# athaddius/RAFT_STIR

Hardware: AMD Instinct MI355X
Metric: train image-pairs/sec (node) + Sintel-res inference FPS, RAFT 12 iters (higher is better)
Workload: dtype bf16; 1 GPU; model=RAFT (raft-things config, 5.26M params), global_batch=8, per_gpu_batch=8, seq_len=12, iters=12, parallelism=dp1, ops=hip-kernels, corr_pyramid=bf16, correlation=all-pairs, train_step=eager, deterministic=True, grad_allreduce=none

## Files before the change

raft_stir_amd/csrc/conv.hip:

```cpp
#include "conv_common.h"

namespace rs {
namespace conv {

template <int CPR>
__device__ __forceinline__ int swz(int r, int c) {
  return CPR == 4 ? r * 4 + (c ^ ((r >> 2) & 3)) : r * 8 + (c ^ ((r >> 1) & 7));
}

template <int BM, int BN, int WAVES_M, int WAVES_N, int BK, bool GEO = false, bool F32 = false, int KG = 1>
__global__ __launch_bounds__(256 * KG) void conv_lds_kernel(Args a) {
  static_assert(WAVES_M * WAVES_N == 4, "4 waves");
  static_assert(KG == 1 || KG == 2 || KG == 4, "KG");
  static_assert(BK == 32 || BK == 64, "BK");
  static_assert(!F32 || BK == 64, "F32: 64-wide staged rows ([hi 32 | lo 32])");
  constexpr int CPR = BK / 8;
  constexpr int WM = BM / WAVES_M / 16, WN = BN / WAVES_N / 16;
  constexpr int NA = BM * CPR / 256, NB = F32 ? BN * 4 / 256 : BN * CPR / 256;
  static_assert(NA >= 1 && NB >= 1, "BM, BN must be multiples of 64");
  __shared__ uint4 lds_[KG * 2][(BM + BN) * CPR];

  const int kg = KG == 1 ? 0 : __builtin_amdgcn_readfirstlane((int)threadIdx.x >> 8);
  uint4 (*lds)[(BM + BN) * CPR] = lds_ + kg * 2;
  const int t = threadIdx.x & 255, lane = t & 63, wave = t >> 6;
// ... 478 lines not shown
#pragma unroll
      for (int nt = 0; nt < WN; ++nt)
        asm volatile("ds_read_b128 %0, %1 offset:%2" : "=v"(fb[kk][nt]) : "v"(bbase[kk] + so), "i"(nt * 16 * RB)
                     : "memory");
    }
    if (step + STAGES - 1 < nst) RS_BISSUE(buf == 0 ? STAGES - 1 : buf - 1);
    asm volatile("s_waitcnt lgkmcnt(0)" ::: "memory");
#pragma unroll
    for (int kk = 0; kk < 2; ++kk) {
#pragma unroll
      for (int mt = 0; mt < WM; ++mt) asm volatile("" : "+v"(fa[kk][mt]));
#pragma unroll
      for (int nt = 0; nt < WN; ++nt) asm volatile("" : "+v"(fb[kk][nt]));
    }
#pragma unroll
    for (int kk = 0; kk < 2; ++kk)
#pragma unroll
      for (int mt = 0; mt < WM; ++mt)
#pragma unroll
        for (int nt = 0; nt < WN; ++nt)
          acc[mt][nt] = __builtin_amdgcn_mfma_f32_16x16x32_bf16(__builtin_bit_cast(bf16x8_t, fa[kk][mt]),
                                                                __builtin_bit_cast(bf16x8_t, fb[kk][nt]),
                                                                acc[mt][nt], 0, 0, 0);
    buf = buf == STAGES - 1 ? 0 : buf + 1;
  }

#undef RS_BISSUE
#undef RS_BADV
  if constexpr (KG > 1) {
    constexpr int NE = WM * WN * 4;
    static_assert((KG - 1) * NE * NT * 4 <= STAGES * KG * GSLOT * 16, "split-K reduction buffer");
    float* red = reinterpret_cast<float*>(&lds[0][0]);
    __syncthreads();
    if (kg > 0) {
#pragma unroll
      for (int mt = 0; mt < WM; ++mt)
#pragma unroll
        for (int nt = 0; nt < WN; ++nt)
#pragma unroll
          for (int j = 0; j < 4; ++j)
            red[((size_t)((kg - 1) * NE + (mt * WN + nt) * 4 + j) * NT) + t] = acc[mt][nt][j];
    }
    __syncthreads();
    if (kg > 0) return;
#pragma unroll
    for (int g = 0; g < KG - 1; ++g)
#pragma unroll
      for (int mt = 0; mt < WM; ++mt)
#pragma unroll
        for (int nt = 0; nt < WN; ++nt)
#pragma unroll
          for (int j = 0; j < 4; ++j) acc[mt][nt][j] += red[((size_t)(g * NE + (mt * WN + nt) * 4 + j) * NT) + t];
  }

  int pb[WN], py[WN], px[WN];
#pragma unroll
  for (int nt = 0; nt < WN; ++nt) {
    const int p = n0 + nt * 16 + lr;
    if (p < a.P) {
      pb[nt] = p / HW;
      const int q = p - pb[nt] * HW;
      py[nt] = q / W;
      px[nt] = q - py[nt] * W;
    } else {
      pb[nt] = -1;
      py[nt] = px[nt] = 0;
    }
  }
  epilogue<WM, WN>(a, acc, m0, n0, lane, pb, py, px);
}

template <int BM, int TH, int HCAP>
__global__ __launch_bounds__(256) void conv_halo_kernel(Args a) {
  constexpr int TW = 16, BN = TH * TW;
  constexpr int WM = BM / 2 / 16, WN = BN / 2 / 16;
  constexpr int NA = BM * 8 / 256, NH = HCAP * 8 / 256;
  constexpr int AST = BM * 8, HST = HCAP * 8;
  constexpr int kFar = 0x7ffffff0;
  __shared__ uint4 lds[2 * AST + 2 * HST];

  const int t = threadIdx.x, lane = t & 63, wave = t >> 6;
  const int wm = wave & 1, wn = wave >> 1;
  const int H = a.H, W = a.W, KW = a.KW, Ktot = a.Ktot;
  const int taps = a.KH * KW;
  const int hw = TW + KW - 1;
  const int hrows = (TH + a.KH - 1) * hw;
  const int ntx = cdiv(W, TW), npb = cdiv(H, TH) * ntx;
  const int nct = cdiv(a.Cout, BM);
  const int lid = a.xcd_remap ? xcd_remap(blockIdx.x, gridDim.x) : (int)blockIdx.x;
  const int bm0 = (lid % nct) * BM;
  const int pt = lid / nct;
  const int img = pt / npb, pq = pt - img * npb;
  const int pty = pq / ntx;
  const int y0 = pty * TH, x0 = (pq - pty * ntx) * TW;
  const int m0 = bm0 + wm * WM * 16;

  const __amdgpu_buffer_rsrc_t rw = __builtin_amdgcn_make_buffer_rsrc((void*)a.w, (short)0, a.w_bytes, 0x00020000);
  const Seg s0 = a.seg[0], s1 = a.seg[1], s2 = a.seg[2];
  const __amdgpu_buffer_rsrc_t rs0 =
      __builtin_amdgcn_make_buffer_rsrc((void*)s0.ptr, (short)0, a.seg_bytes[0], 0x00020000);
  const __amdgpu_buffer_rsrc_t rs1 =
      __builtin_amdgcn_make_buffer_rsrc((void*)s1.ptr, (short)0, a.seg_bytes[1], 0x00020000);
  const __amdgpu_buffer_rsrc_t rs2 =
      __builtin_amdgcn_make_buffer_rsrc((void*)s2.ptr, (short)0, a.seg_bytes[2], 0x00020000);

  int aoff[NA];
#pragma unroll
  for (int i = 0; i < NA; ++i) {
    const int id = t + 256 * i, r = id >> 3;
    aoff[i] = ((bm0 + r) * taps * Ktot + (((id & 7) ^ ((r >> 1) & 7)) * 8)) * 2;
  }
  int hpix[NH], hch[NH];
#pragma unroll
  for (int i = 0; i < NH; ++i) {
    const int id = t + 256 * i, r = id >> 3;
    hch[i] = ((id & 7) ^ ((r >> 1) & 7)) * 8;
    hpix[i] = -1;
    if (r < hrows) {
      const int hy = r / hw, hx = r - hy * hw;
      const int y = y0 + hy - a.PH, x = x0 + hx - a.PW;
      if (y >= 0 && y < H && x >= 0 && x < W) hpix[i] = (img * H + y) * W + x;
    }
  }
  const int wbase = wave * 64;
  const int nsteps =
      taps * ((s0.C >> 6) + (a.nseg > 1 ? (s1.C >> 6) : 0) + (a.nseg > 2 ? (s2.C >> 6) : 0));

  int si = 0, c0 = 0, kseg = 0, itap = 0, ichunk = 0, istep = 0;
#define RS_HISSUE()                                                                                 \
  do {                                                                                              \
    const int sC = si == 0 ? s0.C : (si == 1 ? s1.C : s2.C);                                        \
    if (itap == 0) {                                                                                \
      const int sst = si == 0 ? s0.stride : (si == 1 ? s1.stride : s2.stride);                      \
      const __amdgpu_buffer_rsrc_t rb = si == 0 ? rs0 : (si == 1 ? rs1 : rs2);                      \
      uint4* hd = lds + 2 * AST + (ichunk & 1) * HST;                                               \
      _Pragma("unroll") for (int i = 0; i < NH; ++i) {                                              \
        const int v = hpix[i] >= 0 ? (hpix[i] * sst + c0 + hch[i]) * 2 : kFar;                      \
        bdma16(rb, hd + wbase + 256 * i, v, 0);                                                     \
      }                                                                                             \
    }                                                                                               \
    uint4* ad = lds + (istep & 1) * AST;                                                            \
    const int asoff = (itap * Ktot + kseg + c0) * 2;                                                \
    _Pragma("unroll") for (int i = 0; i < NA; ++i) bdma16(rw, ad + wbase + 256 * i, aoff[i], asoff); \
    ++istep;                                                                                        \
    if (++itap == taps) {                                                                           \
      itap = 0;                                                                                     \
      ++ichunk;                                                                                     \
      c0 += 64;                                                                                     \
      if (c0 == sC) { c0 = 0; kseg += sC; ++si; }                                                   \
    }                                                                                               \
  } while (0)

  f32x4_t acc[WM][WN];
#pragma unroll
  for (int i = 0; i < WM; ++i)
#pragma unroll
    for (int j = 0; j < WN; ++j) acc[i][j] = f32x4_t{0.f, 0.f, 0.f, 0.f};

  const int lr = lane & 15, lc = lane >> 4;
  const uint32_t lds0 = (uint32_t)(size_t)(__attribute__((address_space(3))) uint4*)&lds[0];
  uint32_t abase[2];
#pragma unroll
  for (int kk = 0; kk < 2; ++kk)
    abase[kk] = lds0 + (uint32_t)((wm * WM * 16 + lr) * 128 + (((kk * 4 + lc) ^ ((lr >> 1) & 7)) * 16));
  int rbn[WN];
#pragma unroll
  for (int nt = 0; nt < WN; ++nt) rbn[nt] = (wn * WN + nt) * hw + lr;

  RS_HISSUE();
  int ctap = 0, cty = 0, ctx = 0, cchunk = 0;
  for (int step = 0; step < nsteps; ++step) {
    wait_vmcnt<0>();
    asm volatile("s_barrier" ::: "memory");
    const uint32_t so = (step & 1) * AST * 16;
    const uint32_t hb = lds0 + (uint32_t)((2 * AST + (cchunk & 1) * HST) * 16);
    const int toff = cty * hw + ctx;
    uint32_t brow[WN], bsw[WN];
#pragma unroll
    for (int nt = 0; nt < WN; ++nt) {
      const int row = rbn[nt] + toff;
      brow[nt] = hb + (uint32_t)(row * 128);
      bsw[nt] = (uint32_t)((row >> 1) & 7);
    }
    u32x4_t fa[2][WM], fb[2][WN];
#pragma unroll
    for (int kk = 0; kk < 2; ++kk) {
#pragma unroll
      for (int mt = 0; mt < WM; ++mt)
        asm volatile("ds_read_b128 %0, %1 offset:%2" : "=v"(fa[kk][mt]) : "v"(abase[kk] + so), "i"(mt * 16 * 128)
                     : "memory");
#pragma unroll
      for (int nt = 0; nt < WN; ++nt)
        asm volatile("ds_read_b128 %0, %1" : "=v"(fb[kk][nt])
                     : "v"(brow[nt] + ((((uint32_t)(kk * 4 + lc)) ^ bsw[nt]) << 4)) : "memory");
    }
    if (step + 1 < nsteps) RS_HISSUE();
    asm volatile("s_waitcnt lgkmcnt(0)" ::: "memory");
#pragma unroll
    for (int kk = 0; kk < 2; ++kk) {
#pragma unroll
      for (int mt = 0; mt < WM; ++mt) asm volatile("" : "+v"(fa[kk][mt]));
#pragma unroll
      for (int nt = 0; nt < WN; ++nt) asm volatile("" : "+v"(fb[kk][nt]));
    }
#pragma unroll
    for (int kk = 0; kk < 2; ++kk)
#pragma unroll
      for (int mt = 0; mt < WM; ++mt)
#pragma unroll
        for (int nt = 0; nt < WN; ++nt)
          acc[mt][nt] = __builtin_amdgcn_mfma_f32_16x16x32_bf16(__builtin_bit_cast(bf16x8_t, fa[kk][mt]),
                                                                __builtin_bit_cast(bf16x8_t, fb[kk][nt]),
                                                                acc[mt][nt], 0, 0, 0);
    if (++ctx == KW) { ctx = 0; ++cty; }
    if (++ctap == taps) { ctap = 0; cty = 0; ctx = 0; ++cchunk; }
  }
#undef RS_HISSUE

  int pp[WN], pb[WN], py[WN], px[WN];
#pragma unroll
  for (int nt = 0; nt < WN; ++nt) {
    const int y = y0 + wn * WN + nt, x = x0 + lr;
    if (y < H && x < W) {
      pb[nt] = img;
      py[nt] = y;
      px[nt] = x;
      pp[nt] = (img * H + y) * W + x;
    } else {
      pb[nt] = -1;
      py[nt] = px[nt] = pp[nt] = 0;
    }
  }
  epilogue_pix<WM, WN>(a, acc, m0, lane, pp, pb, py, px);
}

__global__ __launch_bounds__(256) void conv_smalln_kernel(Args a) {
  __shared__ f32x4_t red[4][64];
  const int t = threadIdx.x, lane = t & 63, wave = t >> 6;
  const int n0 = blockIdx.x * 16;
  const int H = a.H, W = a.W, KW = a.KW, PH = a.PH, PW = a.PW, Ktot = a.Ktot;
  const int taps = a.KH * KW;
  const int HW = H * W;
  const int lr = lane & 15, lk = (lane >> 4) * 8;
  int pb[1], py[1], px[1];
  {
    const int p = n0 + lr;
    if (p < a.P) {
      pb[0] = p / HW;
      const int q = p - pb[0] * HW;
      py[0] = q / W;
      px[0] = q - py[0] * W;
    } else {
      pb[0] = -1;
      py[0] = px[0] = 0;
    }
  }
  const bf16_t* wrow = a.w + (size_t)lr * taps * Ktot + lk;
  const Seg s0 = a.seg[0], s1 = a.seg[1], s2 = a.seg[2];
  const int e1 = taps * (s0.C >> 5);
  const int e2 = e1 + (a.nseg > 1 ? taps * (s1.C >> 5) : 0);
  const int nsteps = e2 + (a.nseg > 2 ? taps * (s2.C >> 5) : 0);
  const uint4 zero = make_uint4(0, 0, 0, 0);
  f32x4_t acc[1][1];
  acc[0][0] = f32x4_t{0.f, 0.f, 0.f, 0.f};
  for (int step = wave; step < nsteps; step += 4) {
    const int si = (step >= e1) + (step >= e2);
    const bf16_t* sp = si == 0 ? s0.ptr : (si == 1 ? s1.ptr : s2.ptr);
    const int sC = si == 0 ? s0.C : (si == 1 ? s1.C : s2.C);
    const int sst = si == 0 ? s0.stride : (si == 1 ? s1.stride : s2.stride);
    const int kseg = si == 0 ? 0 : (si == 1 ? s0.C : s0.C + s1.C);
    const int local = step - (si == 0 ? 0 : (si == 1 ? e1 : e2));
    const int chunks = sC >> 5;
    const int tap = local / chunks;
    const int c0 = (local - tap * chunks) * 32;
    const int dy = tap / KW - PH, dx = tap % KW - PW;
    const uint4 fa = ld16(wrow + (size_t)tap * Ktot + kseg + c0);
    const int yy = py[0] + dy, xx = px[0] + dx;
    const bool ok = pb[0] >= 0 && yy >= 0 && yy < H && xx >= 0 && xx < W;
    const uint4 fb = ok ? ld16(sp + ((size_t)(pb[0] * H + yy) * W + xx) * sst + c0 + lk) : zero;
    acc[0][0] = __builtin_amdgcn_mfma_f32_16x16x32_bf16(__builtin_bit_cast(bf16x8_t, fa),
                                                        __builtin_bit_cast(bf16x8_t, fb), acc[0][0], 0, 0, 0);
  }
  red[wave][lane] = acc[0][0];
  __syncthreads();
  if (wave == 0) {
    acc[0][0] = red[0][lane] + red[1][lane] + red[2][lane] + red[3][lane];
    epilogue<1, 1>(a, acc, 0, n0, lane, pb, py, px);
  }
}

template <typename T>
__global__ __launch_bounds__(256) void gru_gate_bwd_kernel(float* __restrict__ dh, int dhstr, const T* __restrict__ z,
                                                           int zstr, const T* __restrict__ q, int qstr,
                                                           const T* __restrict__ h, int hstr, int hoff,
                                                           T* __restrict__ dq, int dqstr,
                                                           T* __restrict__ dzr, int dzrstr, long P, int hd) {
  const long total = P * hd;
  for (long i = (long)blockIdx.x * blockDim.x + threadIdx.x; i < total; i += (long)gridDim.x * blockDim.x) {
    const long p = i / hd;
    const int c = (int)(i - p * hd);
    const float g = dh[p * dhstr + c];
    const float zv = io<T>::ld(z + p * zstr + c), qv = io<T>::ld(q + p * qstr + c);
    const float hv = io<T>::ld(h + p * hstr + hoff + c);
    io<T>::st(dq + p * dqstr + c, g * zv * (1.f - qv * qv));
    io<T>::st(dzr + p * dzrstr + c, g * (qv - hv) * zv * (1.f - zv));
    dh[p * dhstr + c] = g * (1.f - zv);
  }
}

template <typename T>
__global__ __launch_bounds__(256) void relu_take_kernel(float* __restrict__ G, int gstr, int goff, int n, int nz,
                                                        const T* __restrict__ act, int astr, int aoff,
                                                        T* __restrict__ out, int ostr, long P) {
  const long total = P * ostr;
  for (long i = (long)blockIdx.x * blockDim.x + threadIdx.x; i < total; i += (long)gridDim.x * blockDim.x) {
    const long p = i / ostr;
    const int c = (int)(i - p * ostr);
    float v = 0.f;
    if (c < n) {
      const float g = G[p * gstr + goff + c];
      v = io<T>::ld(act + p * astr + aoff + c) > 0.f ? g : 0.f;
    }
    io<T>::st(out + i, v);
    if (c < nz) G[p * gstr + goff + c] = 0.f;
  }
}

}

bool conv_1x1_launch(const conv::Args& a, int tile, hipStream_t stream);

struct ConvLaunch {
  const void* seg_ptr[3];
  int seg_C[3], seg_stride[3];
  int nseg;
  const void* w;
  const float* bias;
  int B, H, W, KH, KW, PH, PW, Cout, Cout_pad, Ktot;
  int epi;
  float scale;
  int hd;
  void* out; int ostr, ooff;
  void* out2; int o2str, o2off;
  void* out3; int o3str, o3off;
  const void* aux1; int a1str, a1off;
  const void* aux2; int a2str, a2off;
  int tile;
  unsigned seg_bytes[3];
  unsigned w_bytes;
  int geo;
  int Hi, Wi, SY, SX, oH, oW, OSY, OSX, OOY, OOX;
  const float* chs;
  int f32;
};

bool conv_launch(const ConvLaunch& L, hipStream_t stream) {
  conv::Args a{};
  for (int s = 0; s < 3; ++s) {
    a.seg[s].ptr = static_cast<const bf16_t*>(L.seg_ptr[s]);
    a.seg[s].C = L.seg_C[s];
    a.seg[s].stride = L.seg_stride[s];
  }
  a.nseg = L.nseg;
  a.w = static_cast<const bf16_t*>(L.w);
  a.bias = L.bias;
  a.B = L.B; a.H = L.H; a.W = L.W; a.P = L.B * L.H * L.W;
  a.KH = L.KH; a.KW = L.KW; a.PH = L.PH; a.PW = L.PW;
  a.Cout = L.Cout; a.Ktot = L.Ktot;
  a.epi = L.epi; a.scale = L.scale; a.hd = L.hd;
  a.out = L.out; a.ostr = L.ostr; a.ooff = L.ooff;
  a.out2 = L.out2; a.o2str = L.o2str; a.o2off = L.o2off;
  a.out3 = L.out3; a.o3str = L.o3str; a.o3off = L.o3off;
  a.aux1 = static_cast<const bf16_t*>(L.aux1); a.a1str = L.a1str; a.a1off = L.a1off;
  a.aux2 = static_cast<const bf16_t*>(L.aux2); a.a2str = L.a2str; a.a2off = L.a2off;
  for (int s = 0; s < 3; ++s) a.seg_bytes[s] = L.seg_bytes[s];
  a.w_bytes = L.w_bytes;
  a.chs = L.chs;
  a.f32 = L.f32;
  a.xcd_remap = 1;
  if (L.geo) {
    a.Hi = L.Hi; a.Wi = L.Wi; a.SY = L.SY; a.SX = L.SX;
    a.oH = L.oH; a.oW = L.oW; a.OSY = L.OSY; a.OSX = L.OSX; a.OOY = L.OOY; a.OOX = L.OOX;
#define RS_GEO(BM_, BN_, WM_, WN_, BK_)                                                             \
  if (L.f32)                                                                                       \
    hipLaunchKernelGGL((conv::conv_lds_kernel<BM_, BN_, WM_, WN_, 64, true, true>),               \
                       dim3(cdiv(a.P, BN_), cdiv(L.Cout, BM_)), dim3(256), 0, stream, a);          \
  else                                                                                             \
    hipLaunchKernelGGL((conv::conv_lds_kernel<BM_, BN_, WM_, WN_, BK_, true>),                    \
                       dim3(cdiv(a.P, BN_), cdiv(L.Cout, BM_)), dim3(256), 0, stream, a)
    switch (L.tile) {
      case 2: RS_GEO(64, 128, 1, 4, 32); break;
      case 3: RS_GEO(64, 64, 2, 2, 32); break;
      case 6: RS_GEO(64, 64, 2, 2, 64); break;
      case 7: RS_GEO(128, 64, 2, 2, 64); break;
      case 8: RS_GEO(128, 128, 2, 2, 64); break;
      default: RS_GEO(128, 64, 2, 2, 32); break;
    }
#undef RS_GEO
    return true;
  }
  if (L.f32 && L.tile >= 81 && L.tile <= 85) {
    return conv_v3f_launch(a, L.tile, stream);
  }
  if (L.f32) {
#define RS_F32(BM_, BN_, KG_)                                                                       \
  hipLaunchKernelGGL((conv::conv_lds_kernel<BM_, BN_, 2, 2, 64, false, true, KG_>),                \
                     dim3(cdiv(a.P, BN_), cdiv(L.Cout, BM_)), dim3(256 * KG_), 0, stream, a)
    if (L.tile == 6) RS_F32(64, 64, 1);
    else if (L.tile == 8) RS_F32(128, 128, 1);
    else if (L.tile == 38) RS_F32(64, 64, 4);
    else if (L.tile == 39) RS_F32(128, 64, 2);
    else if (L.tile == 40) RS_F32(64, 64, 2);
    else RS_F32(128, 64, 1);
#undef RS_F32
    return true;
  }
  if (L.tile == 41) {
    dim3 grid(cdiv(a.P, 64), cdiv(L.Cout, 64));
    hipLaunchKernelGGL((conv::conv_lds_kernel<64, 64, 2, 2, 32, false, false, 4>), grid, dim3(1024), 0, stream, a);
    return true;
  }
  if (L.tile >= 24 && L.tile <= 26) {
    const int TH = L.tile == 26 ? 4 : 8, BM = L.tile == 25 ? 64 : 128;
    const dim3 grid(cdiv(L.Cout, BM) * L.B * cdiv(L.H, TH) * cdiv(L.W, 16));
    if (L.tile == 24) hipLaunchKernelGGL((conv::conv_halo_kernel<128, 8, 192>), grid, dim3(256), 0, stream, a);
    else if (L.tile == 25) hipLaunchKernelGGL((conv::conv_halo_kernel<64, 8, 192>), grid, dim3(256), 0, stream, a);
    else hipLaunchKernelGGL((conv::conv_halo_kernel<128, 4, 128>), grid, dim3(256), 0, stream, a);
    return true;
  }
  if (L.tile >= 42 && L.tile <= 54) {
    return conv_v2_launch(a, L.tile, stream);
  }
  if (L.tile == 70) {
    return conv_1x1_launch(a, L.tile, stream);
  }
  if (L.tile >= 56) {
    return conv_v3_launch(a, L.tile, stream);
  }
  if (L.tile == 5) {
    hipLaunchKernelGGL(conv::conv_smalln_kernel, dim3(cdiv(a.P, 16)), dim3(256), 0, stream, a);
  } else if (L.tile >= 2) {
    if (L.tile == 2) {
      dim3 grid(cdiv(a.P, 128), cdiv(L.Cout, 64));
      hipLaunchKernelGGL((conv::conv_lds_kernel<64, 128, 1, 4, 32>), grid, dim3(256), 0, stream, a);
    } else if (L.tile == 3) {
      dim3 grid(cdiv(a.P, 64), cdiv(L.Cout, 64));
      hipLaunchKernelGGL((conv::conv_lds_kernel<64, 64, 2, 2, 32>), grid, dim3(256), 0, stream, a);
    } else if (L.tile == 4) {
      dim3 grid(cdiv(a.P, 64), cdiv(L.Cout, 128));
      hipLaunchKernelGGL((conv::conv_lds_kernel<128, 64, 2, 2, 32>), grid, dim3(256), 0, stream, a);
    } else if (L.tile == 6) {
      dim3 grid(cdiv(a.P, 64), cdiv(L.Cout, 64));
      hipLaunchKernelGGL((conv::conv_lds_kernel<64, 64, 2, 2, 64>), grid, dim3(256), 0, stream, a);
    } else if (L.tile == 7) {
      dim3 grid(cdiv(a.P, 64), cdiv(L.Cout, 128));
      hipLaunchKernelGGL((conv::conv_lds_kernel<128, 64, 2, 2, 64>), grid, dim3(256), 0, stream, a);
    } else if (L.tile == 8) {
      dim3 grid(cdiv(a.P, 128), cdiv(L.Cout, 128));
      hipLaunchKernelGGL((conv::conv_lds_kernel<128, 128, 2, 2, 64>), grid, dim3(256), 0, stream, a);
    } else {
#define RS_GLDS(BM_, BN_, BK_, ST_)                                                                  \
  hipLaunchKernelGGL((conv::conv_glds_kernel<BM_, BN_, 2, 2, BK_, ST_>),                             \
                     dim3(cdiv(a.P, BN_) * cdiv(L.Cout, BM_)), dim3(256), 0, stream, a)
      switch (L.tile) {
        case 9: RS_GLDS(64, 64, 64, 3); break;
        case 10: RS_GLDS(128, 64, 64, 3); break;
        case 11: RS_GLDS(128, 64, 64, 2); break;
        case 12: RS_GLDS(128, 64, 32, 4); break;
        case 13: RS_GLDS(128, 64, 32, 3); break;
        case 14: RS_GLDS(64, 64, 32, 4); break;
        case 15: RS_GLDS(64, 64, 64, 2); break;
#define RS_BUF(BM_, BN_, ST_)                                                                        \
  hipLaunchKernelGGL((conv::conv_buf_kernel<BM_, BN_, 2, 2, ST_>), dim3(cdiv(a.P, BN_) * cdiv(L.Cout, BM_)), \
                     dim3(256), 0, stream, a)
        case 16: RS_BUF(128, 64, 2); break;
        case 17: RS_BUF(64, 64, 2); break;
        case 18: RS_BUF(128, 64, 3); break;
        case 19: RS_BUF(64, 64, 3); break;
        case 20: RS_BUF(128, 128, 2); break;
        case 21: RS_BUF(64, 128, 2); break;
        case 22: RS_BUF(128, 128, 3); break;
        case 23: RS_BUF(64, 64, 4); break;
#define RS_BUF8(BM_, BN_, ST_)                                                                       \
  hipLaunchKernelGGL((conv::conv_buf_kernel<BM_, BN_, 4, 2, ST_>), dim3(cdiv(a.P, BN_) * cdiv(L.Cout, BM_)), \
                     dim3(512), 0, stream, a)
        case 27: RS_BUF8(256, 96, 3); break;
        case 28: RS_BUF8(128, 96, 3); break;
        case 29: RS_BUF8(192, 96, 3); break;
        case 30: RS_BUF8(256, 96, 2); break;
        case 31: RS_BUF8(128, 96, 2); break;
        case 32: RS_BUF8(256, 192, 2); break;
        case 33: RS_BUF8(128, 192, 2); break;
#define RS_BUFK(BM_, BN_, ST_, KG_)                                                                  \
  hipLaunchKernelGGL((conv::conv_buf_kernel<BM_, BN_, 2, 2, ST_, KG_>),                                \
                     dim3(cdiv(a.P, BN_) * cdiv(L.Cout, BM_)), dim3(256 * KG_), 0, stream, a)
        case 34: RS_BUFK(64, 64, 2, 2); break;
        case 35: RS_BUFK(64, 64, 3, 2); break;
        case 36: RS_BUFK(128, 64, 2, 2); break;
        default: RS_BUFK(64, 64, 2, 4); break;
#undef RS_BUFK
#undef RS_BUF8
#undef RS_BUF
      }
#undef RS_GLDS
    }
  } else if (L.tile == 1) {
    constexpr int WM = 4, WN = 2, WAVES_M = 1, WAVES_N = 4;
    dim3 grid(cdiv(a.P, WN * 16 * WAVES_N), cdiv(L.Cout, WM * 16 * WAVES_M));
    hipLaunchKernelGGL((conv::conv_kernel<WM, WN, WAVES_M, WAVES_N>), grid, dim3(64 * WAVES_M * WAVES_N),
                       0, stream, a);
  } else {
    constexpr int WM = 2, WN = 2, WAVES_M = 1, WAVES_N = 4;
    dim3 grid(cdiv(a.P, WN * 16 * WAVES_N), cdiv(L.Cout, WM * 16 * WAVES_M));
    hipLaunchKernelGGL((conv::conv_kernel<WM, WN, WAVES_M, WAVES_N>), grid, dim3(64 * WAVES_M * WAVES_N),
                       0, stream, a);
  }
  return true;
}

static int egrid(long total) {
  const long g = (total + 255) / 256;
  return (int)(g < 16384 ? g : 16384);
}

void gru_gate_bwd_launch(float* dh, int dhstr, const void* z, int zstr, const void* q, int qstr, const void* h,
                         int hstr, int hoff, void* dq, int dqstr, void* dzr, int dzrstr, long P, int hd, bool f32,
                         hipStream_t stream) {
  if (f32)
    hipLaunchKernelGGL(conv::gru_gate_bwd_kernel<float>, dim3(egrid(P * hd)), dim3(256), 0, stream, dh, dhstr,
                       static_cast<const float*>(z), zstr, static_cast<const float*>(q), qstr,
                       static_cast<const float*>(h), hstr, hoff, static_cast<float*>(dq), dqstr,
                       static_cast<float*>(dzr), dzrstr, P, hd);
  else
    hipLaunchKernelGGL(conv::gru_gate_bwd_kernel<bf16_t>, dim3(egrid(P * hd)), dim3(256), 0, stream, dh, dhstr,
                       static_cast<const bf16_t*>(z), zstr, static_cast<const bf16_t*>(q), qstr,
                       static_cast<const bf16_t*>(h), hstr, hoff, static_cast<bf16_t*>(dq), dqstr,
                       static_cast<bf16_t*>(dzr), dzrstr, P, hd);
}

void relu_take_launch(float* G, int gstr, int goff, int n, int nz, const void* act, int astr, int aoff, void* out,
                      int ostr, long P, bool f32, hipStream_t stream) {
  if (f32)
    hipLaunchKernelGGL(conv::relu_take_kernel<float>, dim3(egrid(P * ostr)), dim3(256), 0, stream, G, gstr, goff, n,
                       nz, static_cast<const float*>(act), astr, aoff, static_cast<float*>(out), ostr, P);
  else
    hipLaunchKernelGGL(conv::relu_take_kernel<bf16_t>, dim3(egrid(P * ostr)), dim3(256), 0, stream, G, gstr, goff, n,
                       nz, static_cast<const bf16_t*>(act), astr, aoff, static_cast<bf16_t*>(out), ostr, P);
}


}
```

raft_stir_amd/csrc/conv_common.h:

```cpp
#pragma once
#include "common.h"

#include <stdlib.h>

namespace rs {
namespace conv {

enum Epi : int {
  EPI_BIAS = 0,
  EPI_RELU = 1,
  EPI_SCALE = 2,
  EPI_GRU_ZR = 3,
  EPI_GRU_Q = 4,
  EPI_FLOW = 5,
  EPI_RELU_BWD = 6,
  EPI_ACC_F32 = 7,
  EPI_GRU_QBWD = 8,
  EPI_NORM = 9,
};

struct Seg {
  const bf16_t* ptr;
  int C;
  int stride;
};

struct Args {
  Seg seg[3];
  int nseg;
  const bf16_t* w;
  const float* bias;
  int B, H, W, P;
  int KH, KW, PH, PW;
  int Cout, Ktot;
  int epi;
  float scale;
  int hd;
  void* out;
  int ostr, ooff;
  void* out2;
  int o2str, o2off;
  void* out3;
  int o3str, o3off;
  const bf16_t* aux1;
  int a1str, a1off;
  const bf16_t* aux2;
  int a2str, a2off;
  int xcd_remap;
  unsigned seg_bytes[3];
  unsigned w_bytes;
  int Hi, Wi, SY, SX;
  int oH, oW, OSY, OSX, OOY, OOX;
  const float* chs;
  int f32;
};

typedef float f32x2v_t __attribute__((ext_vector_type(2)));
typedef __bf16 bf16x2v_t __attribute__((ext_vector_type(2)));
__device__ __forceinline__ void split8(const float4& a, const float4& b, uint4& hi, uint4& lo) {
  const float x[8] = {a.x, a.y, a.z, a.w, b.x, b.y, b.z, b.w};
  uint32_t h[4], l[4];
#pragma unroll
  for (int i = 0; i < 4; ++i) {
    const f32x2v_t v = {x[2 * i], x[2 * i + 1]};
    const uint32_t hu = __builtin_bit_cast(uint32_t, __builtin_convertvector(v, bf16x2v_t));
    const f32x2v_t hf = {__uint_as_float(hu << 16), __uint_as_float(hu & 0xffff0000u)};
    h[i] = hu;
    l[i] = __builtin_bit_cast(uint32_t, __builtin_convertvector(v - hf, bf16x2v_t));
  }
  hi = make_uint4(h[0], h[1], h[2], h[3]);
  lo = make_uint4(l[0], l[1], l[2], l[3]);
}

__device__ __forceinline__ uint4 ld16(const bf16_t* p) { return *reinterpret_cast<const uint4*>(p); }

__device__ __forceinline__ void ld4(const bf16_t* p, float (&f)[4]) {
  const uint2 u = *reinterpret_cast<const uint2*>(p);
  f[0] = bf2f((bf16_t)(u.x & 0xffffu));
  f[1] = bf2f((bf16_t)(u.x >> 16));
  f[2] = bf2f((bf16_t)(u.y & 0xffffu));
  f[3] = bf2f((bf16_t)(u.y >> 16));
}
__device__ __forceinline__ void st4(bf16_t* p, const float (&f)[4]) {
  typedef float f2_t __attribute__((ext_vector_type(2)));
  typedef __bf16 b2_t __attribute__((ext_vector_type(2)));
  uint2 pk;
  pk.x = __builtin_bit_cast(uint32_t, __builtin_convertvector((f2_t{f[0], f[1]}), b2_t));
  pk.y = __builtin_bit_cast(uint32_t, __builtin_convertvector((f2_t{f[2], f[3]}), b2_t));
  *reinterpret_cast<uint2*>(p) = pk;
}
__device__ __forceinline__ void acc4(float* p, const float (&f)[4]) {
  float4 o = *reinterpret_cast<float4*>(p);
  o.x += f[0];
  o.y += f[1];
  o.z += f[2];
  o.w += f[3];
  *reinterpret_cast<float4*>(p) = o;
}

template <int E>
__device__ __forceinline__ void epi_frag(const Args& a, float (&v)[4], int cb, int p, int pb, int py, int px,
                                         int HW, bool vec) {
  const bool full = cb + 3 < a.Cout;
  if constexpr (E == EPI_FLOW) {
    float* crd = static_cast<float*>(a.out);
    const float* src = a.out2 ? static_cast<const float*>(a.out2) : crd;
#pragma unroll
    for (int j = 0; j < 4; ++j) {
      const int co = cb + j;
      if (co < a.Cout && co < 2) {
        const size_t o = ((size_t)pb * 2 + co) * HW + (size_t)py * a.W + px;
        crd[o] = src[o] + v[j];
      }
    }
  } else if constexpr (E == EPI_GRU_ZR) {
    if (cb < a.hd) {
      bf16_t* z = static_cast<bf16_t*>(a.out) + (size_t)p * a.ostr + a.ooff + cb;
      float zv[4];
#pragma unroll
      for (int j = 0; j < 4; ++j) zv[j] = sigmoidf_(v[j]);
      if (vec) {
        st4(z, zv);
      } else {
#pragma unroll
        for (int j = 0; j < 4; ++j) z[j] = f2bf(zv[j]);
      }
    } else {
      const int c = cb - a.hd;
      const bf16_t* h = a.aux1 + (size_t)p * a.a1str + a.a1off + c;
      bf16_t* rh = static_cast<bf16_t*>(a.out2) + (size_t)p * a.o2str + a.o2off + c;
      bf16_t* rs_ = a.out3 ? static_cast<bf16_t*>(a.out3) + (size_t)p * a.o3str + a.o3off + c : nullptr;
      float hv[4], rv[4], rhv[4];
      if (vec) {
        ld4(h, hv);
      } else {
#pragma unroll
        for (int j = 0; j < 4; ++j) hv[j] = bf2f(h[j]);
      }
#pragma unroll
      for (int j = 0; j < 4; ++j) {
        rv[j] = sigmoidf_(v[j]);
        rhv[j] = rv[j] * hv[j];
      }
      if (vec) {
        st4(rh, rhv);
        if (rs_) st4(rs_, rv);
      } else {
#pragma unroll
        for (int j = 0; j < 4; ++j) {
          rh[j] = f2bf(rhv[j]);
          if (rs_) rs_[j] = f2bf(rv[j]);
        }
      }
    }
  } else if constexpr (E == EPI_GRU_Q) {
    const bf16_t* h = a.aux1 + (size_t)p * a.a1str + a.a1off + cb;
    const bf16_t* z = a.aux2 + (size_t)p * a.a2str + a.a2off + cb;
    bf16_t* hn = static_cast<bf16_t*>(a.out) + (size_t)p * a.ostr + a.ooff + cb;
    bf16_t* qs = a.out2 ? static_cast<bf16_t*>(a.out2) + (size_t)p * a.o2str + a.o2off + cb : nullptr;
    float hv[4], zv[4], qv[4], nv[4];
    if (vec) {
      ld4(h, hv);
      ld4(z, zv);
    } else {
#pragma unroll
      for (int j = 0; j < 4; ++j) {
        hv[j] = bf2f(h[j]);
        zv[j] = bf2f(z[j]);
      }
    }
#pragma unroll
    for (int j = 0; j < 4; ++j) {
      qv[j] = tanhf_(v[j]);
      nv[j] = (1.f - zv[j]) * hv[j] + zv[j] * qv[j];
    }
    if (vec) {
      st4(hn, nv);
      if (qs) st4(qs, qv);
    } else {
#pragma unroll
      for (int j = 0; j < 4; ++j) {
        hn[j] = f2bf(nv[j]);
        if (qs) qs[j] = f2bf(qv[j]);
      }
    }
  } else if constexpr (E == EPI_RELU_BWD) {
    const bf16_t* act = a.aux1 + (size_t)p * a.a1str + a.a1off + cb;
    bf16_t* o = static_cast<bf16_t*>(a.out) + (size_t)p * a.ostr + a.ooff + cb;
    if (vec && full) {
      float av[4], ov[4];
      ld4(act, av);
#pragma unroll
      for (int j = 0; j < 4; ++j) ov[j] = av[j] > 0.f ? v[j] : 0.f;
      st4(o, ov);
    } else {
#pragma unroll
      for (int j = 0; j < 4; ++j)
        if (cb + j < a.Cout) o[j] = f2bf(bf2f(act[j]) > 0.f ? v[j] : 0.f);
    }
  } else if constexpr (E == EPI_ACC_F32) {
    float* o = static_cast<float*>(a.out) + (size_t)p * a.ostr + a.ooff + cb;
    if (vec && full) {
      acc4(o, v);
    } else {
#pragma unroll
      for (int j = 0; j < 4; ++j)
        if (cb + j < a.Cout) o[j] += v[j];
    }
  } else if constexpr (E == EPI_GRU_QBWD) {
    float* o = static_cast<float*>(a.out) + (size_t)p * a.ostr + a.ooff + cb;
    if (cb < a.hd) {
      const bf16_t* h = a.aux1 + (size_t)p * a.a1str + a.a1off + cb;
      const bf16_t* r = a.aux2 + (size_t)p * a.a2str + a.a2off + cb;
      bf16_t* drp = static_cast<bf16_t*>(a.out2) + (size_t)p * a.o2str + a.o2off + cb;
      float hv[4], rv[4], dv[4], gv[4];
      if (vec) {
        ld4(h, hv);
        ld4(r, rv);
      } else {
#pragma unroll
        for (int j = 0; j < 4; ++j) {
          hv[j] = bf2f(h[j]);
          rv[j] = bf2f(r[j]);
        }
      }
#pragma unroll
      for (int j = 0; j < 4; ++j) {
        dv[j] = v[j] * hv[j] * rv[j] * (1.f - rv[j]);
        gv[j] = v[j] * rv[j];
      }
      if (vec) {
        st4(drp, dv);
        acc4(o, gv);
      } else {
#pragma unroll
        for (int j = 0; j < 4; ++j) {
          drp[j] = f2bf(dv[j]);
          o[j] += gv[j];
        }
      }
    } else {
      if (vec && full) {
        acc4(o, v);
      } else {
#pragma unroll
        for (int j = 0; j < 4; ++j)
          if (cb + j < a.Cout) o[j] += v[j];
      }
    }
  } else if constexpr (E == EPI_NORM) {
    if (a.hd) {
#pragma unroll
      for (int j = 0; j < 4; ++j) v[j] = fmaxf(v[j], 0.f);
    }
    bf16_t* o = static_cast<bf16_t*>(a.out) + (size_t)p * a.ostr + a.ooff + cb;
    const bf16_t* r = a.aux1 ? a.aux1 + (size_t)p * a.a1str + a.a1off + cb : nullptr;
    if (vec && full) {
      if (r) {
        float rv[4];
        ld4(r, rv);
#pragma unroll
        for (int j = 0; j < 4; ++j) v[j] = fmaxf(v[j] + rv[j], 0.f);
      }
      st4(o, v);
    } else {
#pragma unroll
      for (int j = 0; j < 4; ++j)
        if (cb + j < a.Cout) o[j] = f2bf(r ? fmaxf(v[j] + bf2f(r[j]), 0.f) : v[j]);
    }
  } else {
#pragma unroll
    for (int j = 0; j < 4; ++j) {
      if constexpr (E == EPI_RELU) v[j] = fmaxf(v[j], 0.f);
      if constexpr (E == EPI_SCALE) v[j] *= a.scale;
    }
    bf16_t* o = static_cast<bf16_t*>(a.out) + (size_t)p * a.ostr + a.ooff + cb;
    if (vec && full) {
      st4(o, v);
    } else {
#pragma unroll
      for (int j = 0; j < 4; ++j)
        if (cb + j < a.Cout) o[j] = f2bf(v[j]);
    }
  }
}

template <int WM, int WN, int E>
__device__ __forceinline__ void epi_loop(const Args& a, const f32x4_t (&acc)[WM][WN], int m0, int lane,
                                         const int (&pp)[WN], const int (&pb)[WN], const int (&py)[WN],
                                         const int (&px)[WN]) {
  const int HW = a.H * a.W;
  const int cq = (lane >> 4) * 4;
  const bool vec =
      ((a.ooff | a.ostr | a.o2off | a.o2str | a.o3off | a.o3str | a.a1off | a.a1str | a.a2off | a.a2str) & 3) == 0 &&
      (((uintptr_t)a.out | (uintptr_t)a.out2 | (uintptr_t)a.out3 | (uintptr_t)a.aux1 | (uintptr_t)a.aux2) & 15) == 0;
  const bool bvec = a.bias && (((uintptr_t)a.bias) & 15) == 0;
#pragma unroll
  for (int nt = 0; nt < WN; ++nt) {
    if (pb[nt] < 0) continue;
#pragma unroll
    for (int mt = 0; mt < WM; ++mt) {
      const int cb = m0 + mt * 16 + cq;
      if (cb >= a.Cout) continue;
      float v[4];
      if constexpr (E == EPI_NORM) {
        const float4 sv = *reinterpret_cast<const float4*>(a.chs + cb);
        const float4 bv = *reinterpret_cast<const float4*>(a.bias + cb);
        v[0] = acc[mt][nt][0] * sv.x + bv.x;
        v[1] = acc[mt][nt][1] * sv.y + bv.y;
        v[2] = acc[mt][nt][2] * sv.z + bv.z;
        v[3] = acc[mt][nt][3] * sv.w + bv.w;
      } else if (bvec && cb + 3 < a.Cout) {
        const float4 bv = *reinterpret_cast<const float4*>(a.bias + cb);
        v[0] = acc[mt][nt][0] + bv.x;
        v[1] = acc[mt][nt][1] + bv.y;
        v[2] = acc[mt][nt][2] + bv.z;
        v[3] = acc[mt][nt][3] + bv.w;
      } else {
#pragma unroll
        for (int j = 0; j < 4; ++j) v[j] = acc[mt][nt][j] + (cb + j < a.Cout && a.bias ? a.bias[cb + j] : 0.f);
      }
      epi_frag<E>(a, v, cb, pp[nt], pb[nt], py[nt], px[nt], HW, vec);
    }
  }
}

template <int WM, int WN>
__device__ __forceinline__ void epilogue_pix(const Args& a, const f32x4_t (&acc)[WM][WN], int m0, int lane,
                                             const int (&pp)[WN], const int (&pb)[WN], const int (&py)[WN],
                                             const int (&px)[WN]) {
  switch (a.epi) {
#define RS_EPI(E) \
  case E: epi_loop<WM, WN, E>(a, acc, m0, lane, pp, pb, py, px); break
    RS_EPI(EPI_FLOW);
    RS_EPI(EPI_GRU_ZR);
    RS_EPI(EPI_GRU_Q);
    RS_EPI(EPI_RELU_BWD);
    RS_EPI(EPI_ACC_F32);
    RS_EPI(EPI_GRU_QBWD);
    RS_EPI(EPI_RELU);
    RS_EPI(EPI_SCALE);
    RS_EPI(EPI_NORM);
#undef RS_EPI
    default: epi_loop<WM, WN, EPI_BIAS>(a, acc, m0, lane, pp, pb, py, px); break;
  }
}

__device__ __forceinline__ void ld4f(const bf16_t* p, float (&f)[4]) {
  const float4 v = *reinterpret_cast<const float4*>(p);
  f[0] = v.x; f[1] = v.y; f[2] = v.z; f[3] = v.w;
}
__device__ __forceinline__ void st4f(void* p, const float (&f)[4]) {
  *reinterpret_cast<float4*>(p) = make_float4(f[0], f[1], f[2], f[3]);
}

template <int E>
__device__ __forceinline__ void epi_frag_f32(const Args& a, float (&v)[4], int cb, int p, bool vec) {
  const bool full = cb + 3 < a.Cout;
  auto fo = [](void* b, int str, int off, int p_, int c) { return static_cast<float*>(b) + (size_t)p_ * str + off + c; };
  auto fi = [](const bf16_t* b, int str, int off, int p_, int c) {
    return reinterpret_cast<const float*>(b) + (size_t)p_ * str + off + c;
  };
  if constexpr (E == EPI_GRU_ZR) {
    if (cb < a.hd) {
      float* z = fo(a.out, a.ostr, a.ooff, p, cb);
#pragma unroll
      for (int j = 0; j < 4; ++j) z[j] = sigmoidf_(v[j]);
    } else {
      const int c = cb - a.hd;
      const float* h = fi(a.aux1, a.a1str, a.a1off, p, c);
      float* rh = fo(a.out2, a.o2str, a.o2off, p, c);
      float* r = a.out3 ? fo(a.out3, a.o3str, a.o3off, p, c) : nullptr;
#pragma unroll
      for (int j = 0; j < 4; ++j) {
        const float rv = sigmoidf_(v[j]);
        rh[j] = rv * h[j];
        if (r) r[j] = rv;
      }
    }
  } else if constexpr (E == EPI_GRU_Q) {
    const float* h = fi(a.aux1, a.a1str, a.a1off, p, cb);
    const float* z = fi(a.aux2, a.a2str, a.a2off, p, cb);
    float* hn = fo(a.out, a.ostr, a.ooff, p, cb);
    float* qs = a.out2 ? fo(a.out2, a.o2str, a.o2off, p, cb) : nullptr;
#pragma unroll
    for (int j = 0; j < 4; ++j) {
      const float q = tanhf(v[j]);
      hn[j] = (1.f - z[j]) * h[j] + z[j] * q;
      if (qs) qs[j] = q;
    }
  } else if constexpr (E == EPI_RELU_BWD) {
    const float* act = fi(a.aux1, a.a1str, a.a1off, p, cb);
    float* o = fo(a.out, a.ostr, a.ooff, p, cb);
    if (vec && full) {
      const float4 av = *reinterpret_cast<const float4*>(act);
      *reinterpret_cast<float4*>(o) = make_float4(av.x > 0.f ? v[0] : 0.f, av.y > 0.f ? v[1] : 0.f,
                                                  av.z > 0.f ? v[2] : 0.f, av.w > 0.f ? v[3] : 0.f);
    } else {
#pragma unroll
      for (int j = 0; j < 4; ++j)
        if (cb + j < a.Cout) o[j] = act[j] > 0.f ? v[j] : 0.f;
    }
  } else if constexpr (E == EPI_ACC_F32) {
    float* o = fo(a.out, a.ostr, a.ooff, p, cb);
    if (vec && full) {
      acc4(o, v);
    } else {
#pragma unroll
      for (int j = 0; j < 4; ++j)
        if (cb + j < a.Cout) o[j] += v[j];
    }
  } else if constexpr (E == EPI_GRU_QBWD) {
    float* o = fo(a.out, a.ostr, a.ooff, p, cb);
    if (cb < a.hd) {
      const float* h = fi(a.aux1, a.a1str, a.a1off, p, cb);
      const float* r = fi(a.aux2, a.a2str, a.a2off, p, cb);
      float* drp = fo(a.out2, a.o2str, a.o2off, p, cb);
      float gv[4];
#pragma unroll
      for (int j = 0; j < 4; ++j) {
        drp[j] = v[j] * h[j] * r[j] * (1.f - r[j]);
        gv[j] = v[j] * r[j];
      }
      if (vec) {
        acc4(o, gv);
      } else {
#pragma unroll
        for (int j = 0; j < 4; ++j) o[j] += gv[j];
      }
    } else if (vec && full) {
      acc4(o, v);
    } else {
#pragma unroll
      for (int j = 0; j < 4; ++j)
        if (cb + j < a.Cout) o[j] += v[j];
    }
  } else {
#pragma unroll
    for (int j = 0; j < 4; ++j) {
      if constexpr (E == EPI_RELU) v[j] = fmaxf(v[j], 0.f);
      if constexpr (E == EPI_SCALE) v[j] *= a.scale;
      if constexpr (E == EPI_NORM)
        if (a.hd) v[j] = fmaxf(v[j], 0.f);
    }
    float* o = fo(a.out, a.ostr, a.ooff, p, cb);
    const float* r = (E == EPI_NORM && a.aux1) ? fi(a.aux1, a.a1str, a.a1off, p, cb) : nullptr;
    if (vec && full) {
      if (r) {
        float rv[4];
        ld4f(reinterpret_cast<const bf16_t*>(r), rv);
#pragma unroll
        for (int j = 0; j < 4; ++j) v[j] = fmaxf(v[j] + rv[j], 0.f);
      }
      st4f(o, v);
    } else {
#pragma unroll
      for (int j = 0; j < 4; ++j)
        if (cb + j < a.Cout) o[j] = r ? fmaxf(v[j] + r[j], 0.f) : v[j];
    }
  }
}

template <int WM, int WN, int E>
__device__ __forceinline__ void epi_loop_f32(const Args& a, const f32x4_t (&acc)[WM][WN], int m0, int lane,
                                             const int (&pp)[WN], const int (&pb)[WN]) {
  const int cq = (lane >> 4) * 4;
  const bool vec =
      ((a.ooff | a.ostr | a.o2off | a.o2str | a.o3off | a.o3str | a.a1off | a.a1str | a.a2off | a.a2str) & 3) == 0 &&
      (((uintptr_t)a.out | (uintptr_t)a.out2 | (uintptr_t)a.out3 | (uintptr_t)a.aux1 | (uintptr_t)a.aux2) & 15) == 0;
#pragma unroll
  for (int nt = 0; nt < WN; ++nt) {
    if (pb[nt] < 0) continue;
#pragma unroll
    for (int mt = 0; mt < WM; ++mt) {
      const int cb = m0 + mt * 16 + cq;
      if (cb >= a.Cout) continue;
      float v[4];
#pragma unroll
      for (int j = 0; j < 4; ++j) {
        const int c = cb + j;
        const bool in = c < a.Cout;
        const float sc = (E == EPI_NORM && in) ? a.chs[c] : 1.f;
        v[j] = acc[mt][nt][j] * sc + (in && a.bias ? a.bias[c] : 0.f);
      }
      epi_frag_f32<E>(a, v, cb, pp[nt], vec);
    }
  }
}

template <int WM, int WN>
__device__ __forceinline__ void epilogue_pix_f32(const Args& a, const f32x4_t (&acc)[WM][WN], int m0, int lane,
                                                 const int (&pp)[WN], const int (&pb)[WN]) {
  switch (a.epi) {
#define RS_EPI32(E) \
  case E: epi_loop_f32<WM, WN, E>(a, acc, m0, lane, pp, pb); break
    RS_EPI32(EPI_GRU_ZR);
    RS_EPI32(EPI_GRU_Q);
    RS_EPI32(EPI_RELU_BWD);
    RS_EPI32(EPI_ACC_F32);
    RS_EPI32(EPI_GRU_QBWD);
    RS_EPI32(EPI_RELU);
    RS_EPI32(EPI_SCALE);
    RS_EPI32(EPI_NORM);
#undef RS_EPI32
    default: epi_loop_f32<WM, WN, EPI_BIAS>(a, acc, m0, lane, pp, pb); break;
  }
}

template <int WM, int WN>
__device__ __forceinline__ void epilogue(const Args& a, const f32x4_t (&acc)[WM][WN], int m0, int n0,
                                         int lane, const int (&pb)[WN], const int (&py)[WN],
                                         const int (&px)[WN]) {
  int pp[WN];
#pragma unroll
  for (int nt = 0; nt < WN; ++nt) pp[nt] = n0 + nt * 16 + (lane & 15);
  epilogue_pix<WM, WN>(a, acc, m0, lane, pp, pb, py, px);
}

template <int WM, int WN, int WAVES_M, int WAVES_N>
__global__ __launch_bounds__(64 * WAVES_M * WAVES_N) void conv_kernel(Args a) {
  const int lane = threadIdx.x & 63;
  const int wave = threadIdx.x >> 6;
  const int wm = wave % WAVES_M, wn = wave / WAVES_M;
  const int m0 = (blockIdx.y * WAVES_M + wm) * WM * 16;
  const int n0 = (blockIdx.x * WAVES_N + wn) * WN * 16;
  const int lr = lane & 15, lk = (lane >> 4) * 8;
  const int taps = a.KH * a.KW;
  const int HW = a.H * a.W;

  int pb[WN], py[WN], px[WN];
#pragma unroll
  for (int nt = 0; nt < WN; ++nt) {
    const int p = n0 + nt * 16 + lr;
    if (p < a.P) {
      pb[nt] = p / HW;
      const int q = p - pb[nt] * HW;
      py[nt] = q / a.W;
      px[nt] = q - py[nt] * a.W;
    } else {
      pb[nt] = -1;
      py[nt] = px[nt] = 0;
    }
  }
  const bf16_t* wrow[WM];
#pragma unroll
  for (int mt = 0; mt < WM; ++mt)
    wrow[mt] = a.w + (size_t)(m0 + mt * 16 + lr) * taps * a.Ktot + lk;

  f32x4_t acc[WM][WN];
#pragma unroll
  for (int i = 0; i < WM; ++i)
#pragma unroll
    for (int j = 0; j < WN; ++j) acc[i][j] = f32x4_t{0.f, 0.f, 0.f, 0.f};

  const Seg s0 = a.seg[0], s1 = a.seg[1], s2 = a.seg[2];
  const int e1 = taps * (s0.C >> 5);
  const int e2 = e1 + (a.nseg > 1 ? taps * (s1.C >> 5) : 0);
  const int nsteps = e2 + (a.nseg > 2 ? taps * (s2.C >> 5) : 0);

  const int H = a.H, W = a.W, KW = a.KW, PH = a.PH, PW = a.PW, Ktot = a.Ktot;
  const uint4 zero = make_uint4(0, 0, 0, 0);
#define RS_CONV_LOAD(STEP, FA, FB)                                                           \
  do {                                                                                       \
    const int step_ = (STEP);                                                                \
    const int si = (step_ >= e1) + (step_ >= e2);                                            \
    const bf16_t* sp = si == 0 ? s0.ptr : (si == 1 ? s1.ptr : s2.ptr);                       \
    const int sC = si == 0 ? s0.C : (si == 1 ? s1.C : s2.C);                                 \
    const int sst = si == 0 ? s0.stride : (si == 1 ? s1.stride : s2.stride);                 \
    const int kseg = si == 0 ? 0 : (si == 1 ? s0.C : s0.C + s1.C);                           \
    const int local = step_ - (si == 0 ? 0 : (si == 1 ? e1 : e2));                          \
    const int chunks = sC >> 5;                                                              \
    const int tap = local / chunks;                                                          \
    const int c0 = (local - tap * chunks) * 32;                                              \
    const int dy = tap / KW - PH, dx = tap % KW - PW;                                        \
    _Pragma("unroll") for (int mt = 0; mt < WM; ++mt)                                        \
      FA[mt] = ld16(wrow[mt] + (size_t)tap * Ktot + kseg + c0);                              \
    _Pragma("unroll") for (int nt = 0; nt < WN; ++nt) {                                      \
      const int yy = py[nt] + dy, xx = px[nt] + dx;                                          \
      const bool ok = pb[nt] >= 0 && yy >= 0 && yy < H && xx >= 0 && xx < W;                 \
      FB[nt] = ok ? ld16(sp + ((size_t)(pb[nt] * H + yy) * W + xx) * sst + c0 + lk) : zero;  \
    }                                                                                        \
  } while (0)

#define RS_CONV_MMA(FA, FB)                                                                       \
  _Pragma("unroll") for (int mt = 0; mt < WM; ++mt)                                               \
    _Pragma("unroll") for (int nt = 0; nt < WN; ++nt)                                             \
      acc[mt][nt] = __builtin_amdgcn_mfma_f32_16x16x32_bf16(                                      \
          __builtin_bit_cast(bf16x8_t, FA[mt]), __builtin_bit_cast(bf16x8_t, FB[nt]), acc[mt][nt], \
          0, 0, 0)

  uint4 fa0[WM], fb0[WN], fa1[WM], fb1[WN];
  RS_CONV_LOAD(0, fa0, fb0);
  int step = 0;
  for (; step + 2 <= nsteps; step += 2) {
    RS_CONV_LOAD(step + 1, fa1, fb1);
    RS_CONV_MMA(fa0, fb0);
    if (step + 2 < nsteps) RS_CONV_LOAD(step + 2, fa0, fb0);
    RS_CONV_MMA(fa1, fb1);
  }
  if (step < nsteps) {
    RS_CONV_MMA(fa0, fb0);
  }
#undef RS_CONV_LOAD
#undef RS_CONV_MMA

  epilogue<WM, WN>(a, acc, m0, n0, lane, pb, py, px);
}

typedef unsigned int u32x4_t __attribute__((ext_vector_type(4)));

__device__ __forceinline__ int xcd_remap(int bid, int nwg) {
  const int q = nwg >> 3, r = nwg & 7, x = bid & 7;
  return (x < r ? x * (q + 1) : r * (q + 1) + (x - r) * q) + (bid >> 3);
}

__device__ __forceinline__ void glds16(const void* src, uint4* lds_base) {
  __builtin_amdgcn_global_load_lds(
      (const __attribute__((address_space(1))) void*)src, (__attribute__((address_space(3))) void*)lds_base, 16,
      0, 0);
}

template <int N>
__device__ __forceinline__ void wait_vmcnt() {
  asm volatile("s_waitcnt vmcnt(%0)" ::"n"(N) : "memory");
}

__device__ __forceinline__ void bdma16(__amdgpu_buffer_rsrc_t r, uint4* lds_base, int voff, int soff) {
  __builtin_amdgcn_raw_ptr_buffer_load_lds(r, (__attribute__((address_space(3))) void*)lds_base, 16, voff, soff,
                                           0, 0);
}

template <int N>
__device__ __forceinline__ void wait_lgkm() {
  asm volatile("s_waitcnt lgkmcnt(%0)" ::"n"(N) : "memory");
}

template <int E>
__device__ __forceinline__ void epi32(const Args& a, const f32x16_t& acc, int m0, int lane, int p, int pb, int py,
                                      int px, bool vec) {
  if (pb < 0) return;
  const int HW = a.H * a.W;
#pragma unroll
  for (int g = 0; g < 4; ++g) {
    const int cb = m0 + 8 * g + 4 * (lane >> 5);
    if (cb >= a.Cout) continue;
    float v[4];
#pragma unroll
    for (int j = 0; j < 4; ++j) v[j] = acc[4 * g + j] + (cb + j < a.Cout && a.bias ? a.bias[cb + j] : 0.f);
    epi_frag<E>(a, v, cb, p, pb, py, px, HW, vec);
  }
}

template <int NB, int E>
__device__ __forceinline__ void epi32_batch(const Args& a, const f32x16_t (&acc)[NB], int m0, int lane,
                                            const int (&pp)[NB], const int (&pb)[NB]) {
  const int h4 = 4 * (lane >> 5);
  float bz[16];
#pragma unroll
  for (int i = 0; i < 16; ++i) bz[i] = a.bias ? a.bias[m0 + 8 * (i >> 2) + h4 + (i & 3)] : 0.f;
  const bool lo = m0 < a.hd;
  constexpr int NBC = NB > 3 ? 3 : NB;
#pragma unroll
  for (int n0 = 0; n0 < NB; n0 += NBC) {
    uint2 l1[NBC][4], l2[NBC][4];
    float4 lf[NBC][4];
#pragma unroll
    for (int k = 0; k < NBC; ++k) {
      if (n0 + k >= NB) break;
      const size_t p = (size_t)(pb[n0 + k] >= 0 ? pp[n0 + k] : 0);
#pragma unroll
      for (int g = 0; g < 4; ++g) {
        const int cb = m0 + 8 * g + h4;
        if constexpr (E == EPI_GRU_ZR) {
          if (!lo) l1[k][g] = *reinterpret_cast<const uint2*>(a.aux1 + p * a.a1str + a.a1off + cb - a.hd);
        } else if constexpr (E == EPI_GRU_Q) {
          l1[k][g] = *reinterpret_cast<const uint2*>(a.aux1 + p * a.a1str + a.a1off + cb);
          l2[k][g] = *reinterpret_cast<const uint2*>(a.aux2 + p * a.a2str + a.a2off + cb);
        } else if constexpr (E == EPI_RELU_BWD) {
          l1[k][g] = *reinterpret_cast<const uint2*>(a.aux1 + p * a.a1str + a.a1off + cb);
        } else if constexpr (E == EPI_ACC_F32) {
          lf[k][g] = *reinterpret_cast<const float4*>(static_cast<const float*>(a.out) + p * a.ostr + a.ooff + cb);
        } else if constexpr (E == EPI_GRU_QBWD) {
          lf[k][g] = *reinterpret_cast<const float4*>(static_cast<const float*>(a.out) + p * a.ostr + a.ooff + cb);
          if (lo) {
            l1[k][g] = *reinterpret_cast<const uint2*>(a.aux1 + p * a.a1str + a.a1off + cb);
            l2[k][g] = *reinterpret_cast<const uint2*>(a.aux2 + p * a.a2str + a.a2off + cb);
          }
        }
      }
    }
#pragma unroll
    for (int k = 0; k < NBC; ++k) {
      if (n0 + k >= NB) break;
      if (pb[n0 + k] < 0) continue;
      const size_t p = (size_t)pp[n0 + k];
#pragma unroll
      for (int g = 0; g < 4; ++g) {
        const int cb = m0 + 8 * g + h4;
        float v[4];
#pragma unroll
        for (int j = 0; j < 4; ++j) v[j] = acc[n0 + k][4 * g + j] + bz[4 * g + j];
        auto unpack = [](uint2 u, float (&f)[4]) {
          f[0] = bf2f((bf16_t)(u.x & 0xffffu));
          f[1] = bf2f((bf16_t)(u.x >> 16));
          f[2] = bf2f((bf16_t)(u.y & 0xffffu));
          f[3] = bf2f((bf16_t)(u.y >> 16));
        };
        if constexpr (E == EPI_GRU_ZR) {
          float r[4];
#pragma unroll
          for (int j = 0; j < 4; ++j) r[j] = sigmoidf_(v[j]);
          if (lo) {
            st4(static_cast<bf16_t*>(a.out) + p * a.ostr + a.ooff + cb, r);
          } else {
            const int c = cb - a.hd;
            float hv[4], rh[4];
            unpack(l1[k][g], hv);
#pragma unroll
            for (int j = 0; j < 4; ++j) rh[j] = r[j] * hv[j];
            st4(static_cast<bf16_t*>(a.out2) + p * a.o2str + a.o2off + c, rh);
            if (a.out3) st4(static_cast<bf16_t*>(a.out3) + p * a.o3str + a.o3off + c, r);
          }
        } else if constexpr (E == EPI_GRU_Q) {
          float hv[4], zv[4], q[4], nv[4];
          unpack(l1[k][g], hv);
          unpack(l2[k][g], zv);
#pragma unroll
          for (int j = 0; j < 4; ++j) {
            q[j] = tanhf_(v[j]);
            nv[j] = (1.f - zv[j]) * hv[j] + zv[j] * q[j];
          }
          st4(static_cast<bf16_t*>(a.out) + p * a.ostr + a.ooff + cb, nv);
          if (a.out2) st4(static_cast<bf16_t*>(a.out2) + p * a.o2str + a.o2off + cb, q);
        } else if constexpr (E == EPI_RELU_BWD) {
          float av[4];
          unpack(l1[k][g], av);
#pragma unroll
          for (int j = 0; j < 4; ++j) v[j] = av[j] > 0.f ? v[j] : 0.f;
          st4(static_cast<bf16_t*>(a.out) + p * a.ostr + a.ooff + cb, v);
        } else if constexpr (E == EPI_ACC_F32) {
          const float4 o = lf[k][g];
          *reinterpret_cast<float4*>(static_cast<float*>(a.out) + p * a.ostr + a.ooff + cb) =
              make_float4(o.x + v[0], o.y + v[1], o.z + v[2], o.w + v[3]);
        } else if constexpr (E == EPI_GRU_QBWD) {
          const float4 o = lf[k][g];
          float* op = static_cast<float*>(a.out) + p * a.ostr + a.ooff + cb;
          if (lo) {
            float hv[4], rv[4], dv[4];
            unpack(l1[k][g], hv);
            unpack(l2[k][g], rv);
#pragma unroll
            for (int j = 0; j < 4; ++j) dv[j] = v[j] * hv[j] * rv[j] * (1.f - rv[j]);
            st4(static_cast<bf16_t*>(a.out2) + p * a.o2str + a.o2off + cb, dv);
            *reinterpret_cast<float4*>(op) =
                make_float4(o.x + v[0] * rv[0], o.y + v[1] * rv[1], o.z + v[2] * rv[2], o.w + v[3] * rv[3]);
          } else {
            *reinterpret_cast<float4*>(op) = make_float4(o.x + v[0], o.y + v[1], o.z + v[2], o.w + v[3]);
          }
        } else {
#pragma unroll
          for (int j = 0; j < 4; ++j) {
            if constexpr (E == EPI_RELU) v[j] = fmaxf(v[j], 0.f);
            if constexpr (E == EPI_SCALE) v[j] *= a.scale;
          }
          st4(static_cast<bf16_t*>(a.out) + p * a.ostr + a.ooff + cb, v);
        }
      }
    }
  }
}

template <int NB>
__device__ __forceinline__ void epilogue32(const Args& a, const f32x16_t (&acc)[NB], int m0, int lane,
                                           const int (&pp)[NB], const int (&pb)[NB], const int (&py)[NB],
                                           const int (&px)[NB]) {
  const bool vec =
      ((a.ooff | a.ostr | a.o2off | a.o2str | a.o3off | a.o3str | a.a1off | a.a1str | a.a2off | a.a2str) & 3) == 0 &&
      (((uintptr_t)a.out | (uintptr_t)a.out2 | (uintptr_t)a.out3 | (uintptr_t)a.aux1 | (uintptr_t)a.aux2) & 15) == 0;
  const bool fast = vec && m0 + 32 <= a.Cout && (a.hd & 31) == 0;
  if (fast) {
    switch (a.epi) {
#define RS_EB(E) \
  case E: epi32_batch<NB, E>(a, acc, m0, lane, pp, pb); return
      RS_EB(EPI_GRU_ZR);
      RS_EB(EPI_GRU_Q);
      RS_EB(EPI_RELU_BWD);
      RS_EB(EPI_ACC_F32);
      RS_EB(EPI_GRU_QBWD);
      RS_EB(EPI_RELU);
      RS_EB(EPI_SCALE);
      RS_EB(EPI_BIAS);
#undef RS_EB
      default: break;
    }
  }
  switch (a.epi) {
#define RS_E2(E)                                                                      \
  case E:                                                                             \
    _Pragma("unroll") for (int nb = 0; nb < NB; ++nb)                                 \
      epi32<E>(a, acc[nb], m0, lane, pp[nb], pb[nb], py[nb], px[nb], vec);            \
    break
    RS_E2(EPI_FLOW);
    RS_E2(EPI_GRU_ZR);
    RS_E2(EPI_GRU_Q);
    RS_E2(EPI_RELU_BWD);
    RS_E2(EPI_ACC_F32);
    RS_E2(EPI_GRU_QBWD);
    RS_E2(EPI_RELU);
    RS_E2(EPI_SCALE);
#undef RS_E2
    default:
#pragma unroll
      for (int nb = 0; nb < NB; ++nb) epi32<EPI_BIAS>(a, acc[nb], m0, lane, pp[nb], pb[nb], py[nb], px[nb], vec);
      break;
  }
}

}

bool conv_v2_launch(const conv::Args& a, int tile, hipStream_t stream);
bool conv_v3_launch(const conv::Args& a, int tile, hipStream_t stream);
bool conv_v3f_launch(const conv::Args& a, int tile, hipStream_t stream);
}
```

raft_stir_amd/csrc/ops_conv.cpp:

```cpp
#include <ATen/ATen.h>
#include "host_common.h"
#include "enc_epi.h"
#include <c10/core/DeviceGuard.h>
#include <torch/library.h>

#include <hip/hip_runtime.h>
#include <stdlib.h>

#include <algorithm>
#include <initializer_list>

namespace rs {
struct ConvLaunch {
  const void* seg_ptr[3];
  int seg_C[3], seg_stride[3];
  int nseg;
  const void* w;
  const float* bias;
  int B, H, W, KH, KW, PH, PW, Cout, Cout_pad, Ktot;
  int epi;
  float scale;
  int hd;
  void* out; int ostr, ooff;
  void* out2; int o2str, o2off;
  void* out3; int o3str, o3off;
  const void* aux1; int a1str, a1off;
  const void* aux2; int a2str, a2off;
  int tile;
  unsigned seg_bytes[3];
  unsigned w_bytes;
  int geo;
  int Hi, Wi, SY, SX, oH, oW, OSY, OSX, OOY, OOX;
  const float* chs;
  int f32;
};
bool conv_launch(const ConvLaunch& L, hipStream_t stream);
struct SconvLaunch {
  const void* x;
  int xstr, Cin, B, Hi, Wi;
  const float* w;
  const float* bias;
  void* y;
  int ystr, yoff, Cout, Ho, Wo, KH, KW, S, P, relu;
  const void* res;
  int rstr;
  bool f32;
};
int sconv_max_weights();
struct SconvWgradLaunch {
  const void* x;
  const void* dy;
  int xstr, ystr, Cin, Cout, B, Hi, Wi, Ho, Wo, KH, KW, S, P;
  bool f32;
  float* dw;
  float* part;
};
int sconv_wgrad_blocks(int B, int Ho, int OUT, int* rows_per_block);
void sconv_wgrad_launch(const SconvWgradLaunch& L, int nblk, int rows_per_block, hipStream_t stream);
void sconv_launch(const SconvLaunch& L, hipStream_t stream);
struct EncWgradLaunch {
  const void* x;
  const void* dy;
  int xstr, ystr;
  long x_bytes, dy_bytes;
  int B, H, W, Cin, Cout;
  float* part;
  float* dw;
  int nsplit, tpb;
};
int enc_wgrad_splits(int B, int H, int W, int Cin, int Cout, int* tpb);
void enc_wgrad_launch(const EncWgradLaunch& L, hipStream_t stream);
void flow_enc_launch(const float* coords, int B, int H, int W, const float* w, const float* bias,
                     int Cout, void* out, int ostr, int ooff, void* fout, int fstr, int foff, bool f32,
                     hipStream_t stream);
void flowhead_fwd_launch(const void* x, int xstr, int xoff, int cin, const float* w, const float* bias, int B,
                         int H, int W, float* crd, const float* src, bool x_f32, hipStream_t s);
void flowhead_dgrad_launch(const float* dflow, const float* w, int cin, int B, int H, int W, const void* act,
                           int astr, int aoff, void* out, int ostr, int ooff, bool f32, hipStream_t s);
void gru_gate_bwd_launch(float* dh, int dhstr, const void* z, int zstr, const void* q, int qstr, const void* h,
                         int hstr, int hoff, void* dq, int dqstr, void* dzr, int dzrstr, long P, int hd, bool f32,
                         hipStream_t stream);
void relu_take_launch(float* G, int gstr, int goff, int n, int nz, const void* act, int astr, int aoff, void* out,
                      int ostr, long P, bool f32, hipStream_t stream);
struct WgradLaunch {
  const void* dy;
  int ystr, yoff, Cout;
  const void* seg_ptr[3];
  int seg_C[3], seg_stride[3], seg_period[3];
  int nseg;
  int Bp, H, W, KH, KW, Ktot;
  float* dw;
  float* db;
  int bn128;  unsigned dy_bytes, seg_bytes[3];
  int dma;
  float* part;
  int Hi, Wi, SY, SX;
};
void wgrad_launch(const WgradLaunch& L, hipStream_t stream);
int wgrad_splits(const WgradLaunch& L);
int colsum_blocks(int P);
void colsum_launch(const void* dy, int ystr, int yoff, int C, int P, float* db, float* part, hipStream_t stream);
int flow_wgrad_blocks(int Bp, int H);
size_t flow_wgrad_lds(int W);
void flow_wgrad_launch(const float* coords, int Bp, int H, int W, const void* df, int fstr, int Cout, float* dw,
                       float* db, float* part, bool f32, hipStream_t stream);
bool deterministic();
bool enc_halo_launch(const uint16_t* x, int xstr, const uint16_t* w, int Ktot, uint16_t* y, int ystr, int B, int H,
                     int W, int cin, int cout, int num_cus, const EncEpi& e, hipStream_t stream);
bool enc_halo_supported(int cin, int cout);
struct StemLaunch {
  const void* x;
  int x_bf16, B, Hi, Wi, Ho, Wo;
  const void* w;
  const float* bias;
  int Cout, epi, relu;
  void* out;
  int ostr, ooff;
  const void* res;
  int rstr;
  const float* chs;
  int f32;
};
void stem_launch(const StemLaunch& L, hipStream_t stream);
int stem_wgrad_blocks(int B, int Ho, int Wo, int* chunks_per_block);
void stem_wgrad_launch(const void* x, bool x_bf16, int B, int Hi, int Wi, int Ho, int Wo, const uint16_t* dy, int ystr,
                       int Cout, float* part, int nblk, int px_per_block, float* dw, hipStream_t stream);
}

namespace {
using at::Tensor;

constexpr int EPI_GRU_ZR = 3, EPI_GRU_Q = 4, EPI_FLOW = 5, EPI_RELU_BWD = 6, EPI_ACC_F32 = 7, EPI_GRU_QBWD = 8,
              EPI_NORM = 9;

hipStream_t stream() { return rs::current_stream(); }

void check_nhwc(const Tensor& t, int B, int H, int W, const char* n, at::ScalarType dt = at::kBFloat16) {
  TORCH_CHECK(t.is_cuda() && t.is_contiguous() && t.dim() == 4, n, ": contiguous NHWC GPU tensor required");
  TORCH_CHECK(t.size(0) == B && t.size(1) == H && t.size(2) == W, n, ": spatial shape mismatch");
  TORCH_CHECK(t.scalar_type() == dt, n, ": ", dt, " required");
}

void check_one_device(const char* op, const Tensor& first, std::initializer_list<const Tensor*> rest) {
  for (const Tensor* t : rest)
    TORCH_CHECK(t == nullptr || !t->defined() || t->device() == first.device(), op,
                ": all tensors must be on one device, got ", first.device(), " and ", t->device());
}
const Tensor* opt_ptr(const c10::optional<Tensor>& t) { return t ? &*t : nullptr; }

struct NormX {
  const float* chs = nullptr;
};
void check_vec4(const c10::optional<Tensor>& t, int Cout, const char* op, const char* n) {
  TORCH_CHECK(t && t->is_cuda() && t->is_contiguous() && t->scalar_type() == at::kFloat &&
                  t->numel() >= (Cout + 3) / 4 * 4 && (uintptr_t)t->data_ptr() % 16 == 0,
              op, ": ", n, " must be 16-B aligned fp32 with round_up(Cout, 4) values");
}
NormX norm_extras(const c10::optional<Tensor>& nscale, const c10::optional<Tensor>& bias, int epi, int Cout,
                  const char* op) {
  NormX x;
  TORCH_CHECK(bool(nscale) == (epi == EPI_NORM), op, ": nscale is the EPI_NORM scale (and only that)");
  if (nscale) {
    check_vec4(nscale, Cout, op, "nscale");
    check_vec4(bias, Cout, op, "bias (the EPI_NORM shift)");
    x.chs = nscale->data_ptr<float>();
  }
  return x;
}

void conv_impl(const std::vector<Tensor>& segs, at::IntArrayRef seg_off, at::IntArrayRef seg_C,
               const Tensor& w, const c10::optional<Tensor>& bias, int64_t KH, int64_t KW, int64_t Cout,
               int64_t epi, double scale, int64_t hd, const Tensor& out, int64_t ooff,
               const c10::optional<Tensor>& out2, int64_t o2off, const c10::optional<Tensor>& out3,
               int64_t o3off, const c10::optional<Tensor>& aux1, int64_t a1off,
               const c10::optional<Tensor>& aux2, int64_t a2off, int64_t tile,
               const NormX& nx = NormX()) {
  TORCH_CHECK(!segs.empty() && segs.size() <= 3, "conv_fused: 1..3 input segments");
  TORCH_CHECK(seg_off.size() == segs.size() && seg_C.size() == segs.size(), "conv_fused: segment spec");
  const int B = segs[0].size(0), H = segs[0].size(1), W = segs[0].size(2);
  const c10::DeviceGuard guard(segs[0].device());
  rs::ConvLaunch L{};
  const bool f32 = segs[0].scalar_type() == at::kFloat;
  const at::ScalarType adt = f32 ? at::kFloat : at::kBFloat16;
  const bool v3f = f32 && tile >= 81 && tile <= 85;
  if (f32) {
    TORCH_CHECK(tile == 6 || tile == 7 || tile == 8 || (tile >= 38 && tile <= 40) || v3f,
                "conv_fused: fp32 activations run on tiles 6, 7, 8, 38-40, 81-85 only");
    TORCH_CHECK(epi != EPI_FLOW, "conv_fused: fp32 activations: no flow epilogue (csrc/flowhead.hip serves it)");
  }
  L.f32 = f32 ? 1 : 0;
  int Ktot = 0;
  for (size_t s = 0; s < 3; ++s) {
    if (s < segs.size()) {
      check_nhwc(segs[s], B, H, W, "segment", adt);
      const int C = seg_C[s], off = seg_off[s], Cb = segs[s].size(3);
      TORCH_CHECK(C > 0 && C % 32 == 0, "conv_fused: segment channels must be a positive multiple of 32");
      TORCH_CHECK(off >= 0 && off % 8 == 0 && Cb % 8 == 0 && off + C <= Cb,
                  "conv_fused: segment window out of bounds or misaligned");
      L.seg_ptr[s] = static_cast<const char*>(segs[s].data_ptr()) + (size_t)off * segs[s].element_size();
      L.seg_C[s] = C;
      L.seg_stride[s] = Cb;
      TORCH_CHECK(segs[s].numel() * segs[s].element_size() < (int64_t(1) << 31),
                  "conv_fused: segment tensor must be < 2 GiB");
      L.seg_bytes[s] = (unsigned)((segs[s].numel() - off) * segs[s].element_size());
      Ktot += C;
    } else {
      L.seg_ptr[s] = L.seg_ptr[0];
      L.seg_C[s] = 32;
      L.seg_stride[s] = L.seg_stride[0];
      L.seg_bytes[s] = L.seg_bytes[0];
    }
  }
  L.nseg = segs.size();
  TORCH_CHECK(KH >= 1 && KW >= 1 && KH % 2 == 1 && KW % 2 == 1, "conv_fused: odd kernel sizes only");
  TORCH_CHECK((tile >= 0 && tile <= 54) || tile == 56 || tile == 57 || tile == 61 || tile == 65 || tile == 66 ||
                  tile == 68 || tile == 70 || v3f,
              "conv_fused: tile must be in [0,54], 56, 57, 61, 65, 66, 68 or 70");
  if (tile == 70) {
    TORCH_CHECK(KH == 1 && KW == 1 && !f32, "conv_fused: tile 70 is the bf16 1x1 GEMM");
    for (size_t s = 0; s < segs.size(); ++s)
      TORCH_CHECK(seg_C[s] % 64 == 0, "conv_fused: tile 70 needs segment channels % 64 == 0");
  }
  const bool v3 = tile >= 56 && tile <= 68;
  if (v3f) {
    for (size_t s = 0; s < segs.size(); ++s)
      TORCH_CHECK(seg_C[s] % 64 == 0, "conv_fused: tiles 81-85 need segment channels % 64 == 0");
    TORCH_CHECK(tile != 85 || Ktot == 64, "conv_fused: tile 85 (one halo buffer) needs exactly one 64-channel K chunk");
  }
  if ((tile >= 42 && tile <= 54) || v3 || v3f)
    TORCH_CHECK((KH == 3 && KW == 3) || (KH == 1 && KW == 5) || (KH == 5 && KW == 1),
                "conv_fused: tiles 42-68 are instantiated for 3x3, 1x5 and 5x1 kernels only");
  TORCH_CHECK(tile < 16 || KH * KW <= 32, "conv_fused: buffer-DMA tiles (16-37) support at most 32 taps");
  TORCH_CHECK(!(tile >= 38 && tile <= 40) || f32, "conv_fused: tiles 38-40 are the fp32 split-K tiles");
  TORCH_CHECK(tile != 5 || Cout <= 16, "conv_fused: tile 5 (small-N) needs Cout <= 16");
  if (tile >= 24 && tile <= 26) {
    const int TH = tile == 26 ? 4 : 8, HCAP = tile == 26 ? 128 : 192;
    TORCH_CHECK((TH + KH - 1) * (16 + KW - 1) <= HCAP, "conv_fused: kernel too large for halo tile ", tile);
  }
  const bool bm128 = tile == 4 || tile == 7 || tile == 8 || (tile >= 10 && tile <= 13) || tile == 16 ||
                     tile == 18 || tile == 20 || tile == 22 || tile == 24 || tile == 26 || tile == 36 ||
                     tile == 39;
  const bool bm128w = tile == 28 || tile == 31 || tile == 33;
  const int tileM = (tile == 48 || tile == 49 || tile == 53 || tile == 70) ? 128
                    : (tile == 50 || tile == 51 || tile == 52) ? 256
                    : tile == 54 ? 192
                    : (tile == 42 || tile >= 45) ? 64 : tile == 43 ? 32 : tile == 44 ? 128
                    : tile == 0 ? 32
                    : (tile == 27 || tile == 30 || tile == 32) ? 256
                    : tile == 29 ? 192
                    : (bm128 || bm128w) ? 128 : (tile == 5 ? 16 : 64);
  if (tile >= 6 && tile != 12 && tile != 13 && tile != 14 && tile != 41 && !f32)
    for (size_t s = 0; s < segs.size(); ++s)
      TORCH_CHECK(seg_C[s] % 64 == 0, "conv_fused: 64-deep-K tiles need segment channels % 64 == 0");
  TORCH_CHECK(w.is_cuda() && w.is_contiguous() && w.scalar_type() == at::kBFloat16 && w.dim() == 3,
              "conv_fused: packed weight must be contiguous bf16 (Cout_pad, taps, Ktot)");
  TORCH_CHECK(w.size(1) == KH * KW && w.size(2) == (f32 && !v3f ? 2 : 1) * Ktot,
              "conv_fused: packed weight K mismatch", f32 && !v3f ? " (fp32: split [wh | wl] weights, 2 x Ktot)" : "");
  if (v3f) {
    TORCH_CHECK(w.size(0) % 64 == 0 && w.size(0) / 2 >= (Cout + 31) / 32 * 32 && w.numel() * 2 < (int64_t(1) << 31),
                "conv_fused: tiles 81-85 need split fragment-major weights [frag(wh); frag(wl)] (ops/conv.py "
                "frag_weight_split)");
  } else if (v3) {
    TORCH_CHECK(w.size(0) % 32 == 0 && w.size(0) >= (Cout + 31) / 32 * 32 && w.numel() * 2 < (int64_t(1) << 31),
                "conv_fused: tiles 56-68 need fragment-major weights with round_up(Cout, 32) rows (< 2 GiB)");
  } else {
    TORCH_CHECK(w.size(0) >= (Cout + tileM - 1) / tileM * tileM,
                "conv_fused: packed weight needs >= round_up(Cout, ", tileM, ") rows");
  }
  if (bias) {
    TORCH_CHECK(bias->is_cuda() && bias->scalar_type() == at::kFloat && bias->numel() >= Cout &&
                    bias->is_contiguous(),
                "conv_fused: bias must be fp32 (Cout,)");
  }
  L.w = w.data_ptr();
  L.w_bytes = (unsigned)(w.numel() * 2);
  L.bias = bias ? bias->data_ptr<float>() : nullptr;
  L.B = B; L.H = H; L.W = W; L.KH = KH; L.KW = KW; L.PH = KH / 2; L.PW = KW / 2;
  L.Cout = Cout; L.Cout_pad = w.size(0); L.Ktot = w.size(2);
  L.epi = epi; L.scale = scale; L.hd = hd; L.tile = tile;
  if (epi == EPI_FLOW) {
    TORCH_CHECK(out.is_cuda() && out.is_contiguous() && out.scalar_type() == at::kFloat && out.dim() == 4 &&
                    out.size(0) == B && out.size(1) == 2 && out.size(2) == H && out.size(3) == W,
                "conv_fused(flow): out must be fp32 coords (B,2,H,W)");
    TORCH_CHECK(Cout == 2, "conv_fused(flow): Cout must be 2");
    L.out = out.data_ptr(); L.ostr = 0; L.ooff = 0;
    if (out2) {
      TORCH_CHECK(out2->is_cuda() && out2->is_contiguous() && out2->scalar_type() == at::kFloat &&
                      out2->sizes() == out.sizes(),
                  "conv_fused(flow): out2 (source coords) must match out");
      L.out2 = out2->data_ptr();
    }
  } else {
    const bool f32out = f32 || epi == EPI_ACC_F32 || epi == EPI_GRU_QBWD;
    check_nhwc(out, B, H, W, "out", f32out ? at::kFloat : at::kBFloat16);
    const int cw = epi == EPI_GRU_ZR ? hd : Cout;
    TORCH_CHECK(ooff >= 0 && ooff + cw <= out.size(3), "conv_fused: output window out of bounds");
    L.out = out.data_ptr(); L.ostr = out.size(3); L.ooff = ooff;
  }
  auto opt_nhwc = [&](const c10::optional<Tensor>& t, int64_t off, int width, const char* n, void** p,
                      int* str, int* o) {
    if (!t) { *p = nullptr; *str = 0; *o = 0; return; }
    check_nhwc(*t, B, H, W, n, adt);
    TORCH_CHECK(off >= 0 && off + width <= t->size(3), "conv_fused: ", n, " window out of bounds");
    *p = t->data_ptr(); *str = t->size(3); *o = off;
  };
  void* p;
  if (epi == EPI_GRU_ZR) {
    TORCH_CHECK(Cout == 2 * hd && hd % 4 == 0 && out2 && aux1, "conv_fused(gru_zr): needs Cout=2*hd, out2 (r*h), aux1 (h)");
    opt_nhwc(out2, o2off, hd, "out2", &L.out2, &L.o2str, &L.o2off);
    opt_nhwc(out3, o3off, hd, "out3", &L.out3, &L.o3str, &L.o3off);
    opt_nhwc(aux1, a1off, hd, "aux1", &p, &L.a1str, &L.a1off); L.aux1 = p;
  } else if (epi == EPI_GRU_Q) {
    TORCH_CHECK(Cout % 4 == 0 && aux1 && aux2, "conv_fused(gru_q): needs aux1 (h) and aux2 (z)");
    opt_nhwc(out2, o2off, Cout, "out2", &L.out2, &L.o2str, &L.o2off);
    opt_nhwc(aux1, a1off, Cout, "aux1", &p, &L.a1str, &L.a1off); L.aux1 = p;
    opt_nhwc(aux2, a2off, Cout, "aux2", &p, &L.a2str, &L.a2off); L.aux2 = p;
  } else if (epi == EPI_RELU_BWD) {
    TORCH_CHECK(aux1, "conv_fused(relu_bwd): needs aux1 (the ReLU output)");
    opt_nhwc(aux1, a1off, Cout, "aux1", &p, &L.a1str, &L.a1off); L.aux1 = p;
  } else if (epi == EPI_NORM) {
    if (aux1) { opt_nhwc(aux1, a1off, Cout, "aux1", &p, &L.a1str, &L.a1off); L.aux1 = p; }
  } else if (epi == EPI_GRU_QBWD) {
    TORCH_CHECK(hd % 4 == 0 && hd <= Cout && out2 && aux1 && aux2,
                "conv_fused(gru_qbwd): needs out2 (dr_pre), aux1 (h), aux2 (r)");
    opt_nhwc(out2, o2off, hd, "out2", &L.out2, &L.o2str, &L.o2off);
    opt_nhwc(aux1, a1off, hd, "aux1", &p, &L.a1str, &L.a1off); L.aux1 = p;
    opt_nhwc(aux2, a2off, hd, "aux2", &p, &L.a2str, &L.a2off); L.aux2 = p;
  }
  TORCH_CHECK(epi >= 0 && epi <= EPI_NORM, "conv_fused: unknown epilogue kind");
  if (nx.chs)
    TORCH_CHECK(!(tile >= 42 && tile <= 54) && !v3 && tile != 70 && (!(tile >= 81 && tile <= 85) || f32),
                "conv_fused: EPI_NORM needs a tile with the shared epilogue (not 42-70)");
  L.chs = nx.chs;
  TORCH_CHECK(rs::conv_launch(L, stream()), "conv_fused: tile ", L.tile, " is not instantiated for a ", KH, "x", KW,
              " kernel");
  RS_CHECK_LAUNCH();
}

void conv_fused(const std::vector<Tensor>& segs, at::IntArrayRef seg_off, at::IntArrayRef seg_C,
                const Tensor& w, const c10::optional<Tensor>& bias, int64_t KH, int64_t KW, int64_t Cout,
                int64_t epi, double scale, int64_t hd, const Tensor& out, int64_t ooff,
                const c10::optional<Tensor>& out2, int64_t o2off, const c10::optional<Tensor>& out3,
                int64_t o3off, const c10::optional<Tensor>& aux1, int64_t a1off,
                const c10::optional<Tensor>& aux2, int64_t a2off, int64_t tile, const c10::optional<Tensor>& nscale) {
  const NormX nx = norm_extras(nscale, bias, epi, Cout, "conv_fused");
  conv_impl(segs, seg_off, seg_C, w, bias, KH, KW, Cout, epi, scale, hd, out, ooff, out2, o2off, out3, o3off,
            aux1, a1off, aux2, a2off, tile, nx);
}

void conv_geo(const std::vector<Tensor>& segs, at::IntArrayRef seg_off, at::IntArrayRef seg_C, const Tensor& w,
              const c10::optional<Tensor>& bias, int64_t KH, int64_t KW, int64_t PH, int64_t PW, int64_t SY,
              int64_t SX, int64_t Ho, int64_t Wo, int64_t Cout, const Tensor& out, int64_t ooff, int64_t OSY,
              int64_t OSX, int64_t OOY, int64_t OOX, int64_t tile, const c10::optional<Tensor>& nscale, bool relu) {
  TORCH_CHECK(!segs.empty() && segs.size() <= 3 && seg_off.size() == segs.size() && seg_C.size() == segs.size(),
              "conv_geo: 1..3 input segments");
  TORCH_CHECK(tile == 2 || tile == 3 || tile == 4 || tile == 6 || tile == 7 || tile == 8,
              "conv_geo: tile must be one of the register-staged variants 2, 3, 4, 6, 7, 8");
  const bool f32 = segs[0].scalar_type() == at::kFloat;
  const at::ScalarType adt = f32 ? at::kFloat : at::kBFloat16;
  const int bk = (tile >= 6 && !f32) ? 64 : 32;
  const int tileM = (tile == 2 || tile == 3 || tile == 6) ? 64 : 128;
  const int B = segs[0].size(0), Hi = segs[0].size(1), Wi = segs[0].size(2);
  const c10::DeviceGuard guard(segs[0].device());
  rs::ConvLaunch L{};
  int Ktot = 0;
  for (size_t s = 0; s < 3; ++s) {
    if (s < segs.size()) {
      check_nhwc(segs[s], B, Hi, Wi, "conv_geo segment", adt);
      const int C = seg_C[s], off = seg_off[s], Cb = segs[s].size(3);
      TORCH_CHECK(C > 0 && C % bk == 0, "conv_geo: segment channels must be a multiple of ", bk, " for tile ", tile);
      TORCH_CHECK(off >= 0 && off % 8 == 0 && Cb % 8 == 0 && off + C <= Cb, "conv_geo: segment window");
      L.seg_ptr[s] = static_cast<const char*>(segs[s].data_ptr()) + (size_t)off * segs[s].element_size();
      L.seg_C[s] = C;
      L.seg_stride[s] = Cb;
      Ktot += C;
    } else {
      L.seg_ptr[s] = L.seg_ptr[0];
      L.seg_C[s] = bk;
      L.seg_stride[s] = L.seg_stride[0];
    }
  }
  L.nseg = segs.size();
  TORCH_CHECK(KH >= 1 && KW >= 1 && SY >= 1 && SX >= 1 && Ho >= 1 && Wo >= 1 && Cout >= 1, "conv_geo: geometry");
  TORCH_CHECK(w.is_cuda() && w.is_contiguous() && w.scalar_type() == at::kBFloat16 && w.dim() == 3 &&
                  w.size(1) == KH * KW && w.size(2) == (f32 ? 2 : 1) * Ktot &&
                  w.size(0) >= (Cout + tileM - 1) / tileM * tileM,
              "conv_geo: packed weight must be bf16 [>= round_up(Cout, ", tileM, ")][KH*KW][Ktot]");
  if (bias)
    TORCH_CHECK(bias->is_cuda() && bias->scalar_type() == at::kFloat && bias->is_contiguous() &&
                    bias->numel() >= Cout,
                "conv_geo: bias fp32 (Cout,)");
  TORCH_CHECK(out.is_cuda() && out.is_contiguous() && out.dim() == 4 && out.scalar_type() == adt &&
                  out.size(0) == B && ooff >= 0 && ooff + Cout <= out.size(3),
              "conv_geo: out must be contiguous NHWC (the input dtype) with room for the channel window");
  const int oH = out.size(1), oW = out.size(2);
  TORCH_CHECK(OSY >= 1 && OSX >= 1 && OOY >= 0 && OOX >= 0 && (Ho - 1) * OSY + OOY < oH &&
                  (Wo - 1) * OSX + OOX < oW,
              "conv_geo: output pixel map out of bounds");
  TORCH_CHECK(int64_t(B) * Ho * Wo < (int64_t(1) << 31) && out.numel() < (int64_t(1) << 31), "conv_geo: size");
  L.w = w.data_ptr();
  L.bias = bias ? bias->data_ptr<float>() : nullptr;
  L.B = B; L.H = Ho; L.W = Wo; L.KH = KH; L.KW = KW; L.PH = PH; L.PW = PW;
  L.Cout = Cout; L.Cout_pad = w.size(0); L.Ktot = w.size(2);
  L.f32 = f32 ? 1 : 0;
  const int epi = nscale ? EPI_NORM : 0;
  const NormX nx = norm_extras(nscale, bias, epi, Cout, "conv_geo");
  TORCH_CHECK(!relu || nscale, "conv_geo: relu goes with the EPI_NORM epilogue");
  L.epi = epi; L.scale = 1.f; L.hd = relu ? 1 : 0;
  L.chs = nx.chs;
  L.out = out.data_ptr(); L.ostr = out.size(3); L.ooff = ooff;
  L.tile = tile;
  L.geo = 1;
  L.Hi = Hi; L.Wi = Wi; L.SY = SY; L.SX = SX;
  L.oH = oH; L.oW = oW; L.OSY = OSY; L.OSX = OSX; L.OOY = OOY; L.OOX = OOX;
  TORCH_CHECK(rs::conv_launch(L, stream()), "conv_fused: tile ", L.tile, " is not instantiated for a ", KH, "x", KW,
              " kernel");
  RS_CHECK_LAUNCH();
}

void flow_encode(const Tensor& coords, const Tensor& w, const Tensor& bias, const Tensor& out, int64_t ooff,
                 const c10::optional<Tensor>& fout, int64_t foff) {
  TORCH_CHECK(coords.is_cuda() && coords.is_contiguous() && coords.scalar_type() == at::kFloat &&
                  coords.dim() == 4 && coords.size(1) == 2,
              "flow_encode: coords must be fp32 (B,2,H,W)");
  const int B = coords.size(0), H = coords.size(2), W = coords.size(3);
  const int Cout = bias.numel();
  TORCH_CHECK(Cout % 16 == 0, "flow_encode: Cout must be a multiple of 16");
  TORCH_CHECK(w.is_cuda() && w.is_contiguous() && w.scalar_type() == at::kFloat && w.numel() == 98 * Cout,
              "flow_encode: w must be fp32 [49][2][Cout]");
  TORCH_CHECK(bias.is_cuda() && bias.scalar_type() == at::kFloat && bias.is_contiguous(), "flow_encode: bias fp32");
  const bool f32 = out.scalar_type() == at::kFloat;
  check_nhwc(out, B, H, W, "out", f32 ? at::kFloat : at::kBFloat16);
  TORCH_CHECK(ooff % 8 == 0 && out.size(3) % 8 == 0 && ooff + Cout <= out.size(3), "flow_encode: out window");
  void* fp = nullptr;
  int fstr = 0;
  if (fout) {
    check_nhwc(*fout, B, H, W, "fout", f32 ? at::kFloat : at::kBFloat16);
    TORCH_CHECK(foff >= 0 && foff + 2 <= fout->size(3), "flow_encode: fout window");
    fp = fout->data_ptr();
    fstr = fout->size(3);
  }
  const c10::DeviceGuard guard(coords.device());
  rs::flow_enc_launch(coords.data_ptr<float>(), B, H, W, w.data_ptr<float>(), bias.data_ptr<float>(), Cout,
                      out.data_ptr(), out.size(3), ooff, fp, fstr, foff, f32, stream());
  RS_CHECK_LAUNCH();
}

void flow_head(const Tensor& x, int64_t xoff, int64_t cin, const Tensor& w, const Tensor& bias, const Tensor& crd,
               const c10::optional<Tensor>& src) {
  TORCH_CHECK(cin == 128 || cin == 256, "flow_head: Cin must be 128 or 256");
  TORCH_CHECK(crd.is_cuda() && crd.is_contiguous() && crd.scalar_type() == at::kFloat && crd.dim() == 4 &&
                  crd.size(1) == 2,
              "flow_head: coords must be contiguous fp32 (B,2,H,W)");
  const int B = crd.size(0), H = crd.size(2), W = crd.size(3);
  const bool xf = x.scalar_type() == at::kFloat;
  check_nhwc(x, B, H, W, "x", xf ? at::kFloat : at::kBFloat16);
  const int vn = cin == 256 ? 4 : 2;
  TORCH_CHECK(xoff >= 0 && xoff + cin <= x.size(3) && xoff % vn == 0 && x.size(3) % vn == 0,
              "flow_head: x channel window");
  TORCH_CHECK(w.is_cuda() && w.is_contiguous() && w.scalar_type() == at::kFloat && w.numel() == 18 * cin,
              "flow_head: w must be fp32 [2][3][3][Cin]");
  TORCH_CHECK(bias.is_cuda() && bias.scalar_type() == at::kFloat && bias.numel() == 2, "flow_head: bias fp32 (2,)");
  if (src) TORCH_CHECK(src->sizes() == crd.sizes() && src->is_contiguous() && src->scalar_type() == at::kFloat,
                       "flow_head: src must match coords");
  const c10::DeviceGuard guard(crd.device());
  rs::flowhead_fwd_launch(x.data_ptr(), x.size(3), xoff, cin, w.data_ptr<float>(), bias.data_ptr<float>(), B, H, W,
                          crd.data_ptr<float>(), src ? src->data_ptr<float>() : crd.data_ptr<float>(), xf, stream());
  RS_CHECK_LAUNCH();
}

void flow_head_dgrad(const Tensor& dflow, const Tensor& w, int64_t cin, const Tensor& act, int64_t aoff,
                     const Tensor& out, int64_t ooff) {
  TORCH_CHECK(cin == 128 || cin == 256, "flow_head_dgrad: Cin must be 128 or 256");
  TORCH_CHECK(dflow.is_cuda() && dflow.is_contiguous() && dflow.scalar_type() == at::kFloat && dflow.dim() == 4 &&
                  dflow.size(1) == 2,
              "flow_head_dgrad: dflow must be contiguous fp32 (B,2,H,W)");
  const int B = dflow.size(0), H = dflow.size(2), W = dflow.size(3);
  const bool f32 = out.scalar_type() == at::kFloat;
  check_nhwc(act, B, H, W, "act", f32 ? at::kFloat : at::kBFloat16);
  check_nhwc(out, B, H, W, "out", f32 ? at::kFloat : at::kBFloat16);
  const int vn = cin == 256 ? 4 : 2;
  TORCH_CHECK(aoff >= 0 && aoff + cin <= act.size(3) && aoff % vn == 0 && act.size(3) % vn == 0,
              "flow_head_dgrad: act channel window");
  TORCH_CHECK(ooff >= 0 && ooff + cin <= out.size(3) && ooff % vn == 0 && out.size(3) % vn == 0,
              "flow_head_dgrad: out channel window");
  TORCH_CHECK(w.is_cuda() && w.is_contiguous() && w.scalar_type() == at::kFloat && w.numel() == 18 * cin,
              "flow_head_dgrad: w must be fp32 [2][3][3][Cin]");
  const c10::DeviceGuard guard(dflow.device());
  rs::flowhead_dgrad_launch(dflow.data_ptr<float>(), w.data_ptr<float>(), cin, B, H, W, act.data_ptr(), act.size(3),
                            aoff, out.data_ptr(), out.size(3), ooff, f32, stream());
  RS_CHECK_LAUNCH();
}

void conv_wgrad_impl(const Tensor& dy, int64_t yoff, int64_t Cout, const std::vector<Tensor>& segs,
                     at::IntArrayRef seg_off, at::IntArrayRef seg_C, at::IntArrayRef seg_period, int64_t KH,
                     int64_t KW, const Tensor& dw, const c10::optional<Tensor>& db, int64_t bn128, int64_t SY,
                     int64_t SX) {
  check_one_device("conv_wgrad", dy, {&dw, opt_ptr(db)});
  for (const auto& t : segs) check_one_device("conv_wgrad", dy, {&t});
  TORCH_CHECK(dy.is_cuda() && dy.is_contiguous() && dy.dim() == 4 && dy.scalar_type() == at::kBFloat16,
              "conv_wgrad: dy must be contiguous bf16 NHWC");
  const int Bp = dy.size(0), H = dy.size(1), W = dy.size(2);
  const bool strided = SY != 1 || SX != 1;
  TORCH_CHECK(SY >= 1 && SX >= 1, "conv_wgrad: stride >= 1");
  const int Hi = strided ? segs.at(0).size(1) : H, Wi = strided ? segs.at(0).size(2) : W;
  static const int dma_env = [] {
    const char* e = getenv("RS_WGRAD_DMA");
    return e ? atoi(e) : 1;
  }();
  const int bm = Cout > 64 ? 128 : 64;
  TORCH_CHECK(yoff >= 0 && yoff % 8 == 0 && yoff + (dma_env ? Cout : (Cout + bm - 1) / bm * bm) <= dy.size(3),
              "conv_wgrad: dy channel window out of bounds");
  TORCH_CHECK(bn128 >= 0 && bn128 <= 5, "conv_wgrad: tile variant 0..5");
  if (db) TORCH_CHECK(db->is_cuda() && db->scalar_type() == at::kFloat && db->numel() >= Cout, "conv_wgrad: db fp32");
  TORCH_CHECK(!segs.empty() && segs.size() <= 3 && seg_off.size() == segs.size() && seg_C.size() == segs.size() &&
                  seg_period.size() == segs.size(),
              "conv_wgrad: segment spec");
  rs::WgradLaunch L{};
  int Ktot = 0;
  for (size_t s = 0; s < 3; ++s) {
    if (s < segs.size()) {
      const Tensor& t = segs[s];
      TORCH_CHECK(t.is_cuda() && t.is_contiguous() && t.dim() == 4 && t.scalar_type() == at::kBFloat16 &&
                      t.size(1) == Hi && t.size(2) == Wi,
                  "conv_wgrad: segment must be contiguous bf16 NHWC with dy's spatial size (the input grid "
                  "when strided)");
      const int per = seg_period[s];
      TORCH_CHECK(per == t.size(0) * Hi * Wi && Bp % t.size(0) == 0,
                  "conv_wgrad: segment period must be its pixel count and its images divide dy's");
      const int C = seg_C[s], off = seg_off[s];
      TORCH_CHECK(C % 64 == 0 && off % 8 == 0 && off + C <= t.size(3), "conv_wgrad: segment window (C % 64)");
      L.seg_ptr[s] = static_cast<const at::BFloat16*>(t.data_ptr()) + off;
      L.seg_C[s] = C;
      L.seg_stride[s] = t.size(3);
      L.seg_period[s] = per;
      TORCH_CHECK(t.numel() * 2 < (int64_t(1) << 31), "conv_wgrad: segment tensor must be < 2 GiB");
      L.seg_bytes[s] = (unsigned)((t.numel() - off) * 2);
      Ktot += C;
    } else {
      L.seg_ptr[s] = L.seg_ptr[0];
      L.seg_C[s] = 64;
      L.seg_stride[s] = L.seg_stride[0];
      L.seg_period[s] = L.seg_period[0];
      L.seg_bytes[s] = L.seg_bytes[0];
    }
  }
  TORCH_CHECK(dw.is_cuda() && dw.is_contiguous() && dw.scalar_type() == at::kFloat && dw.dim() == 3 &&
                  dw.size(0) >= Cout && dw.size(1) == KH * KW && dw.size(2) == Ktot,
              "conv_wgrad: dw must be fp32 (>=Cout, taps, Ktot)");
  const c10::DeviceGuard guard(dy.device());
  L.dy = dy.data_ptr(); L.ystr = dy.size(3); L.yoff = yoff; L.Cout = Cout;
  TORCH_CHECK(dy.numel() * 2 < (int64_t(1) << 31), "conv_wgrad: dY tensor must be < 2 GiB");
  L.dy_bytes = (unsigned)(dy.numel() * 2);
  L.dma = dma_env;
  TORCH_CHECK(!strided || L.dma, "conv_wgrad: strided weight gradients need the buffer-DMA kernels");
  L.Hi = Hi; L.Wi = Wi; L.SY = SY; L.SX = SX;
  L.nseg = segs.size();
  L.Bp = Bp; L.H = H; L.W = W; L.KH = KH; L.KW = KW; L.Ktot = Ktot;
  L.dw = dw.data_ptr<float>();
  L.db = db ? db->data_ptr<float>() : nullptr;
  L.bn128 = bn128;
  L.part = nullptr;
  Tensor part;
  if (rs::deterministic()) {
    TORCH_CHECK(L.dma, "conv_wgrad: deterministic mode needs the buffer-DMA kernels (RS_WGRAD_DMA=1)");
    const int64_t n = int64_t(rs::wgrad_splits(L)) * (int64_t(Cout) * KH * KW * Ktot + Cout);
    part = at::empty({n}, dy.options().dtype(at::kFloat));
    L.part = part.data_ptr<float>();
  }
  rs::wgrad_launch(L, stream());
  RS_CHECK_LAUNCH();
}

void conv_wgrad(const Tensor& dy, int64_t yoff, int64_t Cout, const std::vector<Tensor>& segs,
                at::IntArrayRef seg_off, at::IntArrayRef seg_C, at::IntArrayRef seg_period, int64_t KH, int64_t KW,
                const Tensor& dw, const c10::optional<Tensor>& db, int64_t bn128) {
  conv_wgrad_impl(dy, yoff, Cout, segs, seg_off, seg_C, seg_period, KH, KW, dw, db, bn128, 1, 1);
}

void conv_wgrad_strided(const Tensor& dy, int64_t Cout, const std::vector<Tensor>& segs, at::IntArrayRef seg_off,
                        at::IntArrayRef seg_C, int64_t KH, int64_t KW, int64_t SY, int64_t SX, const Tensor& dw,
                        const c10::optional<Tensor>& db) {
  TORCH_CHECK(dy.dim() == 4 && !segs.empty() && segs[0].dim() == 4 && KH >= 1 && KW >= 1 && SY >= 1 && SX >= 1,
              "conv_wgrad_strided: dy and the segments must be NHWC");
  const int64_t Hi = segs[0].size(1), Wi = segs[0].size(2);
  TORCH_CHECK(dy.size(1) == (Hi + 2 * (KH / 2) - KH) / SY + 1 && dy.size(2) == (Wi + 2 * (KW / 2) - KW) / SX + 1,
              "conv_wgrad_strided: dy grid ", dy.size(1), "x", dy.size(2), " does not match the conv geometry (input ",
              Hi, "x", Wi, ", kernel ", KH, "x", KW, ", stride ", SY, "x", SX, ")");
  std::vector<int64_t> per;
  for (const auto& t : segs) per.push_back(t.size(0) * t.size(1) * t.size(2));
  conv_wgrad_impl(dy, 0, Cout, segs, seg_off, seg_C, per, KH, KW, dw, db, 0, SY, SX);
}

static void check_nhwc_view(const Tensor& t, const char* n) {
  TORCH_CHECK(t.is_cuda() && t.dim() == 4 && t.scalar_type() == at::kBFloat16, n, ": bf16 NHWC GPU tensor");
  TORCH_CHECK(t.stride(3) == 1 && t.stride(2) >= t.size(3) && t.stride(2) % 8 == 0 &&
                  t.stride(1) == t.size(2) * t.stride(2) && t.stride(0) == t.size(1) * t.stride(1),
              n, ": dense NHWC pixels with a channel stride % 8 == 0");
  TORCH_CHECK(reinterpret_cast<uintptr_t>(t.data_ptr()) % 16 == 0, n, ": 16-B aligned base");
  TORCH_CHECK(t.numel() / t.size(3) * t.stride(2) * 2 < (int64_t(1) << 31), n, ": too large for 32-bit offsets");
}

void sconv(const Tensor& x, const Tensor& w, const c10::optional<Tensor>& bias, int64_t stride, int64_t pad,
           bool relu, const Tensor& out, int64_t yoff, const c10::optional<Tensor>& res) {
  check_one_device("sconv", x, {&w, opt_ptr(bias), &out, opt_ptr(res)});
  TORCH_CHECK(x.is_cuda() && x.dim() == 4 && (x.scalar_type() == at::kBFloat16 || x.scalar_type() == at::kFloat),
              "sconv: x bf16 / fp32 NHWC");
  const int B = x.size(0), Hi = x.size(1), Wi = x.size(2), Cin = x.size(3);
  TORCH_CHECK(x.stride(3) == 1 && x.stride(2) % 8 == 0 && x.stride(1) == Wi * x.stride(2) &&
                  x.stride(0) == Hi * x.stride(1) && reinterpret_cast<uintptr_t>(x.data_ptr()) % 16 == 0,
              "sconv: x must be dense NHWC pixels with a channel stride % 8 == 0, 16-B aligned");
  TORCH_CHECK(w.is_cuda() && w.is_contiguous() && w.scalar_type() == at::kFloat && w.dim() == 4 && w.size(3) == Cin,
              "sconv: w fp32 [Cout, KH, KW, Cin]");
  const int Cout = w.size(0), KH = w.size(1), KW = w.size(2);
  TORCH_CHECK(Cin % 8 == 0 && Cout % 8 == 0, "sconv: channel counts must be multiples of 8");
  TORCH_CHECK(std::min(4, Cout / 8) * 8 * KH * KW * Cin <= rs::sconv_max_weights(), "sconv: weight tile too large");
  TORCH_CHECK(stride >= 1 && pad >= 0, "sconv: geometry");
  const int Ho = (Hi + 2 * pad - KH) / stride + 1, Wo = (Wi + 2 * pad - KW) / stride + 1;
  TORCH_CHECK(out.is_cuda() && out.is_contiguous() && out.dim() == 4 && out.scalar_type() == x.scalar_type() &&
                  out.size(0) == B && out.size(1) == Ho && out.size(2) == Wo && yoff >= 0 && yoff % 8 == 0 &&
                  yoff + Cout <= out.size(3) && out.size(3) % 8 == 0,
              "sconv: out must be contiguous [B, Ho, Wo, C] with the window [yoff, yoff + Cout)");
  if (bias) TORCH_CHECK(bias->is_cuda() && bias->scalar_type() == at::kFloat && bias->numel() == Cout, "sconv: bias");
  if (res)
    TORCH_CHECK(res->is_cuda() && res->is_contiguous() && res->scalar_type() == x.scalar_type() && res->dim() == 4 &&
                    res->size(0) == B && res->size(1) == Ho && res->size(2) == Wo && res->size(3) == Cout,
                "sconv: residual must be contiguous [B, Ho, Wo, Cout]");
  const c10::DeviceGuard guard(x.device());
  rs::SconvLaunch L{};
  L.x = x.data_ptr(); L.xstr = x.stride(2); L.Cin = Cin; L.B = B; L.Hi = Hi; L.Wi = Wi;
  L.w = w.data_ptr<float>(); L.bias = bias ? bias->data_ptr<float>() : nullptr;
  L.y = out.data_ptr(); L.ystr = out.size(3); L.yoff = yoff; L.Cout = Cout;
  L.Ho = Ho; L.Wo = Wo; L.KH = KH; L.KW = KW; L.S = stride; L.P = pad; L.relu = relu ? 1 : 0;
  L.res = res ? res->data_ptr() : nullptr; L.rstr = Cout;
  L.f32 = x.scalar_type() == at::kFloat;
  rs::sconv_launch(L, stream());
  RS_CHECK_LAUNCH();
}

void sconv_wgrad(const Tensor& dy, const Tensor& x, int64_t KH, int64_t KW, int64_t stride, int64_t pad,
                 const Tensor& dw) {
  check_one_device("sconv_wgrad", x, {&dy, &dw});
  TORCH_CHECK(x.is_cuda() && x.dim() == 4 && (x.scalar_type() == at::kBFloat16 || x.scalar_type() == at::kFloat),
              "sconv_wgrad: x bf16 / fp32 NHWC");
  TORCH_CHECK(dy.is_cuda() && dy.dim() == 4 && dy.scalar_type() == x.scalar_type(), "sconv_wgrad: dy dtype");
  const int B = x.size(0), Hi = x.size(1), Wi = x.size(2), Cin = x.size(3);
  const int Ho = dy.size(1), Wo = dy.size(2), Cout = dy.size(3);
  TORCH_CHECK(x.stride(3) == 1 && x.stride(2) % 8 == 0 && x.stride(1) == Wi * x.stride(2) &&
                  x.stride(0) == Hi * x.stride(1) && reinterpret_cast<uintptr_t>(x.data_ptr()) % 16 == 0,
              "sconv_wgrad: x must be dense NHWC pixels with a channel stride % 8 == 0, 16-B aligned");
  TORCH_CHECK(dy.stride(3) == 1 && dy.stride(1) == Wo * dy.stride(2) && dy.stride(0) == Ho * dy.stride(1) &&
                  dy.stride(2) % 4 == 0 && reinterpret_cast<uintptr_t>(dy.data_ptr()) % 16 == 0 && Cout % 4 == 0,
              "sconv_wgrad: dy must be dense 16-B aligned NHWC pixels, channel stride % 4 == 0, Cout % 4 == 0");
  TORCH_CHECK(Cin % 8 == 0 && dy.size(0) == B && stride >= 1 && pad >= 0 && KH >= 1 && KW >= 1,
              "sconv_wgrad: shapes");
  TORCH_CHECK(Ho == (Hi + 2 * pad - KH) / stride + 1 && Wo == (Wi + 2 * pad - KW) / stride + 1,
              "sconv_wgrad: dy grid does not match the conv geometry");
  TORCH_CHECK(dw.is_cuda() && dw.is_contiguous() && dw.scalar_type() == at::kFloat &&
                  dw.numel() == (int64_t)Cout * KH * KW * Cin,
              "sconv_wgrad: dw fp32 [Cout, KH, KW, Cin]");
  const int OUT = Cout * KH * KW * Cin;
  int rows = 0;
  const int nblk = rs::sconv_wgrad_blocks(B, Ho, OUT, &rows);
  const c10::DeviceGuard guard(x.device());
  Tensor part = at::empty({(int64_t)nblk * OUT}, dw.options());
  rs::SconvWgradLaunch L{};
  L.x = x.data_ptr(); L.dy = dy.data_ptr(); L.xstr = x.stride(2); L.ystr = dy.stride(2);
  L.Cin = Cin; L.Cout = Cout; L.B = B; L.Hi = Hi; L.Wi = Wi; L.Ho = Ho; L.Wo = Wo;
  L.KH = KH; L.KW = KW; L.S = stride; L.P = pad; L.f32 = x.scalar_type() == at::kFloat;
  L.dw = dw.data_ptr<float>(); L.part = part.data_ptr<float>();
  rs::sconv_wgrad_launch(L, nblk, rows, stream());
  RS_CHECK_LAUNCH();
}

Tensor enc_wgrad(const Tensor& dy, const Tensor& x) {
  check_one_device("enc_wgrad", x, {&dy});
  check_nhwc_view(dy, "enc_wgrad dy");
  check_nhwc_view(x, "enc_wgrad x");
  const int B = x.size(0), H = x.size(1), W = x.size(2), Cin = x.size(3), Cout = dy.size(3);
  TORCH_CHECK(dy.size(0) == B && dy.size(1) == H && dy.size(2) == W, "enc_wgrad: dy / x shapes");
  TORCH_CHECK(Cin % 32 == 0 && Cout % 32 == 0 && Cin >= 64 && Cout >= 64 && Cin <= 512 && Cout <= 512,
              "enc_wgrad: channel counts must be multiples of 32, >= 64");
  const c10::DeviceGuard guard(x.device());
  rs::EncWgradLaunch L{};
  L.x = x.data_ptr();
  L.dy = dy.data_ptr();
  L.xstr = x.stride(2);
  L.ystr = dy.stride(2);
  L.x_bytes = (long)B * H * W * L.xstr * 2;
  L.dy_bytes = (long)B * H * W * L.ystr * 2;
  L.B = B; L.H = H; L.W = W; L.Cin = Cin; L.Cout = Cout;
  L.nsplit = rs::enc_wgrad_splits(B, H, W, Cin, Cout, &L.tpb);
  const int64_t nblk = int64_t(L.nsplit) * ((Cout + 63) / 64) * ((Cin + 63) / 64);
  Tensor part = at::empty({nblk * 64 * 9 * 64}, x.options().dtype(at::kFloat));
  Tensor dw = at::empty({Cout, Cin, 3, 3}, x.options().dtype(at::kFloat).memory_format(at::MemoryFormat::ChannelsLast));
  L.part = part.data_ptr<float>();
  L.dw = dw.data_ptr<float>();
  rs::enc_wgrad_launch(L, stream());
  RS_CHECK_LAUNCH();
  return dw;
}

void colsum(const Tensor& dy, int64_t yoff, int64_t C, const Tensor& db) {
  TORCH_CHECK(dy.is_cuda() && dy.is_contiguous() && dy.scalar_type() == at::kBFloat16, "colsum: bf16 dy");
  TORCH_CHECK(yoff >= 0 && yoff + C <= dy.size(-1), "colsum: channel window");
  TORCH_CHECK(db.is_cuda() && db.scalar_type() == at::kFloat && db.numel() >= C, "colsum: fp32 db");
  const c10::DeviceGuard guard(dy.device());
  const int P = dy.numel() / dy.size(-1);
  Tensor part;
  if (rs::deterministic()) part = at::empty({int64_t(rs::colsum_blocks(P)) * C}, dy.options().dtype(at::kFloat));
  rs::colsum_launch(dy.data_ptr(), dy.size(-1), yoff, C, P, db.data_ptr<float>(),
                    part.defined() ? part.data_ptr<float>() : nullptr, stream());
  RS_CHECK_LAUNCH();
}

void flow_wgrad(const Tensor& coords, const Tensor& df, const Tensor& dw, const Tensor& db) {
  TORCH_CHECK(coords.is_cuda() && coords.is_contiguous() && coords.scalar_type() == at::kFloat && coords.dim() == 4 &&
                  coords.size(1) == 2,
              "flow_wgrad: coords fp32 (B',2,H,W)");
  const int Bp = coords.size(0), H = coords.size(2), W = coords.size(3);
  const bool f32 = df.scalar_type() == at::kFloat;
  TORCH_CHECK(df.is_cuda() && df.is_contiguous() && (f32 || df.scalar_type() == at::kBFloat16) && df.dim() == 4 &&
                  df.size(0) == Bp && df.size(1) == H && df.size(2) == W,
              "flow_wgrad: df bf16 / fp32 (B',H,W,C)");
  const int Cout = db.numel();
  TORCH_CHECK(Cout <= df.size(3) && Cout <= 128 && dw.numel() == 98 * Cout && dw.scalar_type() == at::kFloat &&
                  db.scalar_type() == at::kFloat,
              "flow_wgrad: dw fp32 [49][2][Cout], db fp32 [Cout]");
  TORCH_CHECK(rs::flow_wgrad_lds(W) <= 65536, "flow_wgrad: row width ", W, " exceeds the LDS staging (",
              rs::flow_wgrad_lds(W), " > 65536 bytes)");
  TORCH_CHECK(dw.is_contiguous() && db.is_contiguous(), "flow_wgrad: dw, db contiguous");
  const c10::DeviceGuard guard(coords.device());
  Tensor part;
  if (rs::deterministic())
    part = at::empty({int64_t(rs::flow_wgrad_blocks(Bp, H)) * 99 * Cout}, coords.options());
  rs::flow_wgrad_launch(coords.data_ptr<float>(), Bp, H, W, df.data_ptr(), df.size(3), Cout, dw.data_ptr<float>(),
                        db.data_ptr<float>(), part.defined() ? part.data_ptr<float>() : nullptr, f32, stream());
  RS_CHECK_LAUNCH();
}

void gru_gate_bwd(const Tensor& dh, const Tensor& z, const Tensor& q, const Tensor& h, int64_t hoff, const Tensor& dq,
                  const Tensor& dzr) {
  const int hd = z.size(-1);
  const int64_t P = z.numel() / hd;
  auto chk = [&](const Tensor& t, at::ScalarType dt, int minc, const char* n) {
    TORCH_CHECK(t.is_cuda() && t.is_contiguous() && t.scalar_type() == dt && t.numel() / t.size(-1) == P &&
                    t.size(-1) >= minc,
                "gru_gate_bwd: ", n);
  };
  const bool f32 = z.scalar_type() == at::kFloat;
  const at::ScalarType adt = f32 ? at::kFloat : at::kBFloat16;
  chk(dh, at::kFloat, hd, "dh (fp32)");
  chk(z, adt, hd, "z");
  chk(q, adt, hd, "q");
  chk(h, adt, hoff + hd, "h");
  chk(dq, adt, hd, "dq");
  chk(dzr, adt, hd, "dzr");
  const c10::DeviceGuard guard(z.device());
  rs::gru_gate_bwd_launch(dh.data_ptr<float>(), dh.size(-1), z.data_ptr(), hd, q.data_ptr(), q.size(-1), h.data_ptr(),
                          h.size(-1), hoff, dq.data_ptr(), dq.size(-1), dzr.data_ptr(), dzr.size(-1), P, hd, f32,
                          stream());
  RS_CHECK_LAUNCH();
}

void relu_take(const Tensor& G, int64_t goff, int64_t n, int64_t nz, const Tensor& act, int64_t aoff, const Tensor& out) {
  const int64_t P = out.numel() / out.size(-1);
  TORCH_CHECK(G.is_cuda() && G.is_contiguous() && G.scalar_type() == at::kFloat && G.numel() / G.size(-1) == P &&
                  goff + std::max(n, nz) <= G.size(-1),
              "relu_take: G");
  const bool f32 = out.scalar_type() == at::kFloat;
  const at::ScalarType adt = f32 ? at::kFloat : at::kBFloat16;
  TORCH_CHECK(act.is_contiguous() && act.scalar_type() == adt && act.numel() / act.size(-1) == P &&
                  aoff + n <= act.size(-1),
              "relu_take: act (the out dtype)");
  TORCH_CHECK(out.is_contiguous() && out.scalar_type() == adt && n <= out.size(-1), "relu_take: out");
  const c10::DeviceGuard guard(out.device());
  rs::relu_take_launch(G.data_ptr<float>(), G.size(-1), goff, n, nz, act.data_ptr(), act.size(-1), aoff, out.data_ptr(),
                       out.size(-1), P, f32, stream());
  RS_CHECK_LAUNCH();
}

int num_cus(int dev) {
  static int n[64] = {0};
  if (dev < 0 || dev >= 64) return 256;
  if (n[dev] == 0) {
    int v = 0;
    if (hipDeviceGetAttribute(&v, hipDeviceAttributeMultiprocessorCount, dev) != hipSuccess || v <= 0) v = 256;
    n[dev] = v;
  }
  return n[dev];
}

void conv3x3_halo(const Tensor& x, const Tensor& w, const Tensor& y, int64_t cin, int64_t cout,
                  const c10::optional<Tensor>& nscale,
                  const c10::optional<Tensor>& nshift, const c10::optional<Tensor>& res, bool relu,
                  bool accumulate) {
  check_one_device("conv3x3_halo", x, {&w, &y, opt_ptr(nscale), opt_ptr(nshift), opt_ptr(res)});
  TORCH_CHECK(x.dim() == 4, "conv3x3_halo: x must be NHWC");
  const int B = x.size(0), H = x.size(1), W = x.size(2);
  check_nhwc(x, B, H, W, "conv3x3_halo: x");
  check_nhwc(y, B, H, W, "conv3x3_halo: y");
  TORCH_CHECK(rs::enc_halo_supported(cin, cout), "conv3x3_halo: unsupported channels ", cin, "->", cout);
  TORCH_CHECK(cin <= x.size(3) && x.size(3) % 8 == 0, "conv3x3_halo: x channels");
  TORCH_CHECK(cout <= y.size(3) && y.size(3) % 4 == 0, "conv3x3_halo: y channels");
  TORCH_CHECK(w.is_cuda() && w.is_contiguous() && w.scalar_type() == at::kBFloat16 && w.dim() == 3 &&
                  w.size(0) >= cout && w.size(1) == 9 && w.size(2) >= cin && w.size(2) % 8 == 0,
              "conv3x3_halo: w must be packed [Cout_pad>=cout][9][Ktot>=cin] bf16");
  TORCH_CHECK(((uintptr_t)x.data_ptr() | (uintptr_t)w.data_ptr()) % 16 == 0 && (uintptr_t)y.data_ptr() % 8 == 0,
              "conv3x3_halo: alignment");
  TORCH_CHECK(x.numel() < (int64_t(1) << 31) && y.numel() < (int64_t(1) << 31), "conv3x3_halo: tensor too large");
  rs::EncEpi e;
  const NormX nx = norm_extras(nscale, nshift, nscale ? EPI_NORM : 0, cout, "conv3x3_halo");
  e.chs = nx.chs;
  e.shift = nscale ? nshift->data_ptr<float>() : nullptr;
  TORCH_CHECK(!relu || nscale, "conv3x3_halo: relu goes with nscale / nshift");
  TORCH_CHECK(!res || nscale, "conv3x3_halo: the residual goes with nscale / nshift");
  e.relu = relu ? 1 : 0;
  if (res) {
    check_nhwc(*res, B, H, W, "conv3x3_halo: res");
    TORCH_CHECK(cout <= res->size(3) && res->size(3) % 4 == 0 && (uintptr_t)res->data_ptr() % 8 == 0,
                "conv3x3_halo: res channels / alignment");
    e.res = static_cast<const uint16_t*>(res->data_ptr());
    e.rstr = res->size(3);
  }
  if (accumulate) {
    TORCH_CHECK(!res && !nscale, "conv3x3_halo: accumulate excludes res / nscale");
    e.res = static_cast<const uint16_t*>(y.data_ptr());
    e.rstr = y.size(3);
    e.res_relu = 0;
  }
  const c10::DeviceGuard guard(x.device());
  rs::enc_halo_launch(static_cast<const uint16_t*>(x.data_ptr()), x.size(3), static_cast<const uint16_t*>(w.data_ptr()),
                      w.size(2), static_cast<uint16_t*>(y.data_ptr()), y.size(3), B, H, W, cin, cout,
                      num_cus(x.get_device()), e, stream());
  RS_CHECK_LAUNCH();
}

void stem_conv(const Tensor& x, const Tensor& w, const c10::optional<Tensor>& bias, const Tensor& out, int64_t Cout,
               int64_t epi, const c10::optional<Tensor>& nscale, bool relu) {
  check_one_device("stem_conv", x, {&w, opt_ptr(bias), &out, opt_ptr(nscale)});
  TORCH_CHECK(x.is_cuda() && x.is_contiguous() && x.dim() == 4 && x.size(3) == 3 &&
                  (x.scalar_type() == at::kFloat || x.scalar_type() == at::kBFloat16),
              "stem_conv: x must be a contiguous NHWC [B,H,W,3] fp32 / bf16 image");
  const int B = x.size(0), Hi = x.size(1), Wi = x.size(2);
  const int Ho = (Hi + 6 - 7) / 2 + 1, Wo = (Wi + 6 - 7) / 2 + 1;
  const bool f32 = out.scalar_type() == at::kFloat;
  check_nhwc(out, B, Ho, Wo, "stem_conv: out", f32 ? at::kFloat : at::kBFloat16);
  TORCH_CHECK(Cout >= 1 && Cout <= 64 && Cout % 4 == 0 && out.size(3) >= Cout && out.size(3) % 4 == 0,
              "stem_conv: Cout must be a multiple of 4 in [4, 64]");
  TORCH_CHECK(w.is_cuda() && w.is_contiguous() && w.scalar_type() == at::kBFloat16 && w.dim() == 3 &&
                  w.size(0) == 64 && w.size(1) == 7 && w.size(2) == (f32 ? 64 : 32),
              "stem_conv: packed weight must be bf16 [64][7][", f32 ? 64 : 32, "]");
  TORCH_CHECK(epi == 0 || epi == EPI_NORM, "stem_conv: epilogue 0 (bias) or EPI_NORM");
  if (bias)
    TORCH_CHECK(bias->is_cuda() && bias->scalar_type() == at::kFloat && bias->is_contiguous() &&
                    bias->numel() >= Cout, "stem_conv: bias fp32 (Cout,)");
  const NormX nx = norm_extras(nscale, bias, epi, Cout, "stem_conv");
  TORCH_CHECK(!relu || epi == EPI_NORM, "stem_conv: relu goes with EPI_NORM");
  TORCH_CHECK((uintptr_t)out.data_ptr() % 16 == 0, "stem_conv: out alignment");
  TORCH_CHECK(out.numel() < (int64_t(1) << 31) && x.numel() < (int64_t(1) << 31), "stem_conv: size");
  rs::StemLaunch L{};
  L.x = x.data_ptr(); L.x_bf16 = x.scalar_type() == at::kBFloat16;
  L.B = B; L.Hi = Hi; L.Wi = Wi; L.Ho = Ho; L.Wo = Wo;
  L.w = w.data_ptr(); L.bias = bias ? bias->data_ptr<float>() : nullptr;
  L.Cout = Cout; L.epi = epi; L.relu = relu ? 1 : 0;
  L.out = out.data_ptr(); L.ostr = out.size(3); L.ooff = 0;
  L.chs = nx.chs; L.f32 = f32 ? 1 : 0;
  const c10::DeviceGuard guard(x.device());
  rs::stem_launch(L, stream());
  RS_CHECK_LAUNCH();
}

void stem_wgrad(const Tensor& x, const Tensor& dy, int64_t Cout, const Tensor& dw) {
  check_one_device("stem_wgrad", x, {&dy, &dw});
  TORCH_CHECK(x.is_cuda() && x.is_contiguous() && x.dim() == 4 && x.size(3) == 3 &&
                  (x.scalar_type() == at::kFloat || x.scalar_type() == at::kBFloat16),
              "stem_wgrad: x must be a contiguous NHWC [B,H,W,3] image");
  const int B = x.size(0), Hi = x.size(1), Wi = x.size(2);
  const int Ho = (Hi + 6 - 7) / 2 + 1, Wo = (Wi + 6 - 7) / 2 + 1;
  check_nhwc(dy, B, Ho, Wo, "stem_wgrad: dy");
  TORCH_CHECK(Cout >= 1 && Cout <= 64 && dy.size(3) >= Cout && dy.size(3) % 8 == 0 &&
                  (uintptr_t)dy.data_ptr() % 16 == 0, "stem_wgrad: dy channels / alignment");
  TORCH_CHECK(dw.is_cuda() && dw.is_contiguous() && dw.scalar_type() == at::kFloat && dw.numel() == Cout * 147,
              "stem_wgrad: dw must be fp32 [Cout][3][7][7]");
  int per = 0;
  const int nblk = rs::stem_wgrad_blocks(B, Ho, Wo, &per);
  const c10::DeviceGuard guard(x.device());
  Tensor part = at::empty({(int64_t)nblk * 64 * 224}, dw.options());
  rs::stem_wgrad_launch(x.data_ptr(), x.scalar_type() == at::kBFloat16, B, Hi, Wi, Ho, Wo,
                        static_cast<const uint16_t*>(dy.data_ptr()), dy.size(3), Cout, part.data_ptr<float>(), nblk,
                        per, dw.data_ptr<float>(), stream());
  RS_CHECK_LAUNCH();
}

}

TORCH_LIBRARY_FRAGMENT(raft_stir, m) {
  m.def("stem_conv(Tensor x, Tensor w, Tensor? bias, Tensor(a!) out, int Cout, int epi, Tensor? nscale=None, "
        "bool relu=False) -> ()");
  m.def("stem_wgrad(Tensor x, Tensor dy, int Cout, Tensor(a!) dw) -> ()");
  m.def("conv3x3_halo(Tensor x, Tensor w, Tensor(a!) y, int cin, int cout, "
        "Tensor? nscale=None, Tensor? nshift=None, Tensor? res=None, "
        "bool relu=False, bool accumulate=False) -> ()");
  m.def("conv_wgrad(Tensor dy, int yoff, int Cout, Tensor[] segs, int[] seg_off, int[] seg_C, int[] seg_period, "
        "int KH, int KW, Tensor(a!) dw, Tensor(b!)? db=None, int bn128=0) -> ()");
  m.def("flow_head(Tensor x, int xoff, int cin, Tensor w, Tensor bias, Tensor(a!) crd, Tensor? src) -> ()");
  m.def("flow_head_dgrad(Tensor dflow, Tensor w, int cin, Tensor act, int aoff, Tensor(a!) out, int ooff) -> ()");
  m.def("colsum(Tensor dy, int yoff, int C, Tensor(a!) db) -> ()");
  m.def("flow_wgrad(Tensor coords, Tensor df, Tensor(a!) dw, Tensor(b!) db) -> ()");
  m.def("conv_wgrad_strided(Tensor dy, int Cout, Tensor[] segs, int[] seg_off, int[] seg_C, int KH, int KW, "
        "int SY, int SX, Tensor(a!) dw, Tensor(b!)? db) -> ()");
  m.def("gru_gate_bwd(Tensor(a!) dh, Tensor z, Tensor q, Tensor h, int hoff, Tensor(b!) dq, Tensor(c!) dzr) -> ()");
  m.def("relu_take(Tensor(a!) G, int goff, int n, int nz, Tensor act, int aoff, Tensor(b!) out) -> ()");
  m.def("conv_fused(Tensor[] segs, int[] seg_off, int[] seg_C, Tensor w, Tensor? bias, int KH, int KW, "
        "int Cout, int epi, float scale, int hd, Tensor(a!) out, int ooff, Tensor(b!)? out2, int o2off, "
        "Tensor(c!)? out3, int o3off, Tensor? aux1, int a1off, Tensor? aux2, int a2off, int tile, "
        "Tensor? nscale=None) -> ()");
  m.def("enc_wgrad(Tensor dy, Tensor x) -> Tensor");
  m.def("sconv_wgrad(Tensor dy, Tensor x, int KH, int KW, int stride, int pad, Tensor(a!) dw) -> ()");
  m.def("sconv(Tensor x, Tensor w, Tensor? bias, int stride, int pad, bool relu, Tensor(a!) out, int yoff, "
        "Tensor? res) -> ()");
  m.def("conv_geo(Tensor[] segs, int[] seg_off, int[] seg_C, Tensor w, Tensor? bias, int KH, int KW, int PH, "
        "int PW, int SY, int SX, int Ho, int Wo, int Cout, Tensor(a!) out, int ooff, int OSY, int OSX, int OOY, "
        "int OOX, int tile, Tensor? nscale=None, bool relu=False) -> ()");
  m.def("flow_encode(Tensor coords, Tensor w, Tensor bias, Tensor(a!) out, int ooff, Tensor(b!)? fout, "
        "int foff) -> ()");
}

TORCH_LIBRARY_IMPL(raft_stir, CUDA, m) {
  m.impl("conv_fused", &conv_fused);
  m.impl("conv3x3_halo", &conv3x3_halo);
  m.impl("enc_wgrad", &enc_wgrad);
  m.impl("sconv_wgrad", &sconv_wgrad);
  m.impl("sconv", &sconv);
  m.impl("stem_conv", &stem_conv);
  m.impl("stem_wgrad", &stem_wgrad);
  m.impl("conv_geo", &conv_geo);
  m.impl("flow_encode", &flow_encode);
  m.impl("flow_head", &flow_head);
  m.impl("flow_head_dgrad", &flow_head_dgrad);
  m.impl("conv_wgrad", &conv_wgrad);
  m.impl("colsum", &colsum);
  m.impl("flow_wgrad", &flow_wgrad);
  m.impl("conv_wgrad_strided", &conv_wgrad_strided);
  m.impl("gru_gate_bwd", &gru_gate_bwd);
  m.impl("relu_take", &relu_take);
}
```

raft_stir_amd/models/fused_train.py:

```python
from __future__ import annotations

import contextlib
import os


import torch

from ..ops import _ext
from ..ops.conv import (EPI_ACC_F32, EPI_BIAS, EPI_FLOW, EPI_GRU_Q, EPI_GRU_QBWD, EPI_GRU_ZR, EPI_RELU,
                        EPI_RELU_BWD, EPI_SCALE, conv_fused, frag32_eligible, frag_eligible, frag_weight,
                        frag_weight_split, pack_bias, pack_weight, pad_to)

R = torch.ops.raft_stir
HD = 128
CORR_C = 324
CORR_PAD = 384
SHD = 96
SCORR_C = 196
SCORR_PAD = 256
_SMALL_KPAD = os.environ.get("RS_SMALL_KPAD", "1") != "0"
_EARLY_CORR_BWD = os.environ.get("RS_EARLY_CORR_BWD", "1") != "0"
_V3F_TRAIN = True


class _PConv:

    def __init__(self, convs, segs, scale=1.0, wsegs=None, fsegs=None, dk=None):
        self.convs = convs if isinstance(convs, (list, tuple)) else [convs]
        self.segs = segs
        self.fsegs = fsegs if fsegs is not None else segs
        self.dk = dk
        self.wsegs = wsegs if wsegs is not None else segs
        self.scale = scale
        w0 = self.convs[0].weight
        self.kh, self.kw = w0.shape[2], w0.shape[3]
        self.cout = sum(c.weight.shape[0] for c in self.convs)
        self.cin = w0.shape[1]
        self.ktot = sum(c for c, _ in segs)
        self.wktot = sum(c for c, _ in self.wsegs)

    def index_maps(self, pidx, fill, frag=False):
        weight = torch.cat([pidx[id(c.weight)] for c in self.convs], 0)
        bias = torch.cat([pidx[id(c.bias)] for c in self.convs], 0)
        cout, cin, kh, kw = weight.shape
        taps = kh * kw
        wt = weight.permute(0, 2, 3, 1).reshape(cout, taps, cin)

        def packed(segs):
            w = torch.full((pad_to(cout, 128), taps, sum(c for c, _ in segs)), fill, dtype=torch.long)
            kb = 0
            for c, pieces in segs:
                for w0, n, s0 in pieces:
                    w[:cout, :, kb + s0:kb + s0 + n] = wt[:, :, w0:w0 + n]
                kb += c
            return w
        ws = packed(self.segs)
        w = ws if self.fsegs is self.segs else packed(self.fsegs)
        cy = self.dk or pad_to(cout, 32)
        wd = torch.full((pad_to(self.ktot, 128), taps, cy), fill, dtype=torch.long)
        wd[:self.ktot] = ws[:cy].flip(1).permute(2, 1, 0)
        self.cy = cy
        wf = frag_weight(w) if frag and frag_eligible(w, kh, kw) else None
        wdf = frag_weight(wd) if frag and frag_eligible(wd, kh, kw) else None
        return w, bias, wd, wf, wdf

    def grad_maps(self, gidx):
        dwi, dbi = gidx
        taps = self.kh * self.kw
        gw = torch.empty(self.cout, taps, self.cin, dtype=torch.long)
        kb = 0
        for c, pieces in self.wsegs:
            for w0, n, s0 in pieces:
                gw[:, :, w0:w0 + n] = dwi[:self.cout, :, kb + s0:kb + s0 + n]
            kb += c
        gw = gw.reshape(self.cout, self.kh, self.kw, self.cin).permute(0, 3, 1, 2)
        out, r0 = [], 0
        for c in self.convs:
            n = c.weight.shape[0]
            out.append((gw[r0:r0 + n].contiguous(), dbi[r0:r0 + n].contiguous()))
            r0 += n
        return out


class FusedTrainEngine:
    def __init__(self, model):
        self.model = model
        ub = model.update_block
        enc, g = ub.encoder, ub.gru
        full = lambda c: [(c, [(0, c, 0)])]
        self.small = bool(model.cfg.small)
        self.f32 = not bool(model.cfg.mixed_precision)
        self.spad = self.small and not self.f32 and _SMALL_KPAD
        if self.small:
            self.hd, self.hx_c, self.corr_c, self.corr_pad = SHD, 256, SCORR_C, SCORR_PAD
            dk = 128 if self.spad else None
            self.c1 = _PConv(enc.convc1, [(SCORR_PAD, [(0, SCORR_C, 0)])], dk=dk)
            self.f2 = _PConv(enc.convf2, full(64))
            self.cv = _PConv(enc.conv, full(128), dk=dk)
            self.zr = [_PConv([g.convz, g.convr], [(256, [(0, SHD + 146, 0)])])]
            qw = [(128, [(0, SHD, 0)]), (192, [(SHD, 146, 32)])]
            self.q = [_PConv(g.convq, [(SHD, [(0, SHD, 0)]), (160, [(SHD, 146, 0)])], wsegs=qw,
                             fsegs=qw if self.spad else None, dk=dk)]
            hw = [(128, [(0, SHD, 0)])]
            self.head = _PConv(ub.flow_head.conv1, full(SHD), wsegs=hw, fsegs=hw if self.spad else None)
            self.flow = _PConv(ub.flow_head.conv2, full(128))
            self.mask2 = None
            self.c2 = None
            self.convs = [self.c1, self.f2, self.cv, *self.zr, *self.q, self.head, self.flow]
        else:
            self.hd, self.hx_c, self.corr_c, self.corr_pad = HD, 256, CORR_C, CORR_PAD
            gru_segs = [(HD, [(0, HD, 0)]), (128, [(HD, 128, 0)]), (128, [(HD + 128, 128, 0)])]
            self.c1 = _PConv(enc.convc1, [(CORR_PAD, [(0, CORR_C, 0)])])
            self.c2 = _PConv(enc.convc2, full(256))
            self.f2 = _PConv(enc.convf2, full(128))
            self.cv = _PConv(enc.conv, full(256))
            self.zr = [_PConv([g.convz1, g.convr1], gru_segs), _PConv([g.convz2, g.convr2], gru_segs)]
            self.q = [_PConv(g.convq1, gru_segs), _PConv(g.convq2, gru_segs)]
            self.head = _PConv([ub.flow_head.conv1, ub.mask[0]], full(HD))
            self.flow = _PConv(ub.flow_head.conv2, full(256))
            self.mask2 = _PConv(ub.mask[2], full(256), scale=0.25)
            self.convs = [self.c1, self.c2, self.f2, self.cv, *self.zr, *self.q, self.head, self.flow, self.mask2]
        self.f1 = enc.convf1
        self.f1c = self.f1.weight.shape[0]
        self.adt = torch.float32 if self.f32 else torch.bfloat16
        self.params = []
        for pc in self.convs:
            for c in pc.convs:
                self.params += [c.weight, c.bias]
        self.params += [self.f1.weight, self.f1.bias]
        self._bufs = {}
        self._maps = None
        self.grad_group = None
        self.trace = None

    def attach_grad_group(self, group, world_size: int):
        self.grad_group = (group, int(world_size))

    def reduce_packed(self, gbuf):
        import torch.distributed as dist
        group, ws = self.grad_group
        if ws > 1:
            gbuf.mul_(1.0 / ws)
        work = dist.all_reduce(gbuf, group=group, async_op=True)
        if self.trace is not None:
            self.trace.append(("packed_allreduce", gbuf.numel()))
        work.wait()

    def _build_maps(self, dev):
        sizes = [p.numel() for p in self.params]
        nsrc = sum(sizes)
        fill = nsrc
        ids = torch.arange(nsrc)
        pidx, off = {}, 0
        for p in self.params:
            pidx[id(p)] = ids[off:off + p.numel()].view(p.shape)
            off += p.numel()
        bf_maps, f32_maps, layout = [], [], []
        nbf = 0
        for pc in self.convs:
            w, b, wd, wf, wdf = pc.index_maps(pidx, fill, frag=not self.f32)
            layout.append((pc, w.shape, wd.shape, b.shape, wf is not None, wdf is not None))
            bf_maps += [w.reshape(-1), wd.reshape(-1)]
            bf_maps += [x.reshape(-1) for x in (wf, wdf) if x is not None]
            f32_maps.append(b.reshape(-1))
        f1w = pidx[id(self.f1.weight)].permute(2, 3, 1, 0).contiguous()
        f32_maps += [f1w.reshape(-1), pidx[id(self.f1.bias)].reshape(-1)]
        fcw = self.model.update_block.flow_head.conv2.weight
        f32_maps.append(pidx[id(fcw)].permute(0, 2, 3, 1).reshape(-1))
        nbf = sum(m.numel() for m in bf_maps)
        gather = torch.cat(bf_maps + f32_maps)
        o, scaled = 0, []
        for pc, ws, wds, bs, hf, hdf in layout:
            o += ws.numel()
            if pc.scale != 1.0:
                scaled.append((o, o + wds.numel(), pc.scale))
            o += wds.numel()
            o += ws.numel() if hf else 0
            if hdf and pc.scale != 1.0:
                scaled.append((o, o + wds.numel(), pc.scale))
            o += wds.numel() if hdf else 0
        glayout, go = [], 0
        for pc in self.convs:
            dws = (pad_to(pc.cout, 128), pc.kh * pc.kw, pc.wktot)
            n = dws[0] * dws[1] * dws[2]
            glayout.append((go, dws, go + n, pc.cout))
            go += n + pc.cout
        fc = self.f1c
        gf1 = (go, go + 49 * 2 * fc)
        gtotal = gf1[1] + fc
        gids = torch.arange(gtotal)
        gmaps, gscaled, o = [], [], 0
        for pc, (dwo, dws, dbo, nb) in zip(self.convs, glayout):
            dwi = gids[dwo:dwo + dws[0] * dws[1] * dws[2]].view(dws)
            dbi = gids[dbo:dbo + nb]
            for gw, gb in pc.grad_maps((dwi, dbi)):
                gmaps += [gw.reshape(-1), gb.reshape(-1)]
                if pc.scale != 1.0:
                    scaled_range = (o, o + gw.numel() + gb.numel(), pc.scale)
                    gscaled.append(scaled_range)
                o += gw.numel() + gb.numel()
        f1g = gids[gf1[0]:gf1[1]].view(7, 7, 2, fc).permute(3, 2, 0, 1).contiguous()
        gmaps += [f1g.reshape(-1), gids[gf1[1]:gf1[1] + fc]]
        starts = torch.tensor([0] + sizes[:-1]).cumsum(0)
        row = torch.searchsorted(starts, gather, right=True) - 1
        code = torch.where(gather == fill, torch.full_like(gather, -1),
                           ((row.clamp_min(0) << 24) | (gather - starts[row.clamp_min(0)])))
        assert len(self.params) <= 63 and max(sizes) < (1 << 24)
        code = code.to(torch.int32).to(dev)
        self._maps = dict(dev=dev, gather=gather.to(dev), nbf=nbf, layout=layout, scaled=scaled,
                          code_bf=code[:nbf], code_f32=code[nbf:], tab=None, tab_key=None,
                          out_bf=torch.empty(nbf, dtype=torch.float32 if self.f32 else torch.bfloat16, device=dev),
                          out_f32=torch.empty(gather.numel() - nbf, dtype=torch.float32, device=dev),
                          glayout=glayout, gf1=gf1, gtotal=gtotal, ggather=torch.cat(gmaps).to(dev),
                          gscaled=gscaled, zero=torch.zeros(1, device=dev))

    def _src_table(self):
        M = self._maps
        key = tuple((p.data_ptr(), p.dtype, p.stride()) for p in self.params)
        if key != M["tab_key"]:
            rows = []
            for p in self.params:
                pad = 4 - p.dim()
                rows.append([p.data_ptr(), int(p.dtype == torch.bfloat16)] + [1] * pad + list(p.shape)
                            + [0] * pad + list(p.stride()))
            M["tab"] = torch.tensor(rows, dtype=torch.int64).to(M["dev"])
            M["tab_key"] = key
        return M["tab"]

    @torch.no_grad()
    def pack(self, dev):
        if self._maps is None or self._maps["dev"] != dev:
            self._build_maps(dev)
        M = self._maps
        nbf = M["nbf"]
        if all(p.dtype in (torch.float32, torch.bfloat16) and p.dim() <= 4 for p in self.params):
            tab = self._src_table()
            sc = M["scaled"]
            R.wpack_gather(M["code_bf"], tab, M["out_bf"], [a for a, _, _ in sc], [b for _, b, _ in sc],
                           [float(x) for _, _, x in sc])
            R.wpack_gather(M["code_f32"], tab, M["out_f32"], [], [], [])
            bf = M["out_bf"]
            vals = _Offset(M["out_f32"], nbf)
        else:
            src = torch.cat([p.detach().reshape(-1).float() for p in self.params] + [M["zero"]])
            v = src.index_select(0, M["gather"])
            for a, b, s in M["scaled"]:
                v[a:b].mul_(s)
            bf = v[:nbf] if self.f32 else v[:nbf].to(torch.bfloat16)
            vals = _Offset(v[nbf:], nbf)
        k = 1
        if self.f32:
            v32 = bf.view(-1, 1, 32)
            hi = v32.to(torch.bfloat16)
            bf = torch.cat([hi, (v32 - hi.float()).to(torch.bfloat16)], 1).view(-1)
            k = 2
        ob, of = 0, nbf
        for pc, ws, wds, bs, hf, hdf in M["layout"]:
            n = ws.numel()
            pc.w = bf[k * ob:k * (ob + n)].view(ws[0], ws[1], k * ws[2])
            ob += n
            n = wds.numel()
            pc.wd = bf[k * ob:k * (ob + n)].view(wds[0], wds[1], k * wds[2])
            ob += n
            if self.f32 and _V3F_TRAIN:
                for t in (pc.w, pc.wd):
                    if frag32_eligible(t, pc.kh, pc.kw):
                        t._rs_frag32 = frag_weight_split(t)
            pc.wf = pc.wdf = None
            if hf:
                pc.wf = bf[ob:ob + ws.numel()].view(ws)
                ob += ws.numel()
                pc.w._rs_frag = pc.wf
            if hdf:
                pc.wdf = bf[ob:ob + wds.numel()].view(wds)
                ob += wds.numel()
                pc.wd._rs_frag = pc.wdf
            pc.b = vals[of:of + bs.numel()]
            of += bs.numel()
        fc = self.f1c
        self.f1w = vals[of:of + 49 * 2 * fc].view(7, 7, 2, fc)
        of += 49 * 2 * fc
        self.f1b = vals[of:of + fc]
        of += fc
        fcw = self.model.update_block.flow_head.conv2.weight
        self.flow_w32 = vals[of:of + fcw.numel()].view(fcw.shape[0], fcw.shape[2], fcw.shape[3], fcw.shape[1])

    def side_stream(self, dev, slot: int = 0, flow: bool = False):
        from .raft import OVERLAP
        if not self.model.cfg.overlap_encoders or (flow and not OVERLAP["flow"]):
            return None
        return self.model._side_stream(dev, slot)

    def grad_buffers(self, dev):
        M = self._maps
        g = torch.zeros(M["gtotal"], device=dev)
        for pc, (dwo, dws, dbo, nb) in zip(self.convs, M["glayout"]):
            pc.dw = g[dwo:dwo + dws[0] * dws[1] * dws[2]].view(dws)
            pc.db = g[dbo:dbo + nb]
        a, b = M["gf1"]
        return g, g[a:b].view(49, 2, self.f1c), g[b:b + self.f1c]

    def unpack_grads(self, g):
        M = self._maps
        flat = g.index_select(0, M["ggather"])
        for a, b, s in M["gscaled"]:
            flat[a:b].mul_(s)
        out, o = [], 0
        for p in self.params:
            out.append(flat[o:o + p.numel()].view(p.shape))
            o += p.numel()
        return out

    @staticmethod
    def config_capable(cfg) -> bool:
        return bool(cfg.fused_gru) and getattr(cfg, "fused_train", True)

    @staticmethod
    def eligible(model, image, corr_fn) -> bool:
        corr_ok = getattr(corr_fn, "state", None) is not None or (
            getattr(corr_fn, "f2s", None) is not None and corr_fn.radius == (3 if model.cfg.small else 4)
            and len(corr_fn.f2s) == 4 and corr_fn.f1.dtype == torch.bfloat16 and model.cfg.mixed_precision)
        return (image.device.type == "cuda" and torch.is_grad_enabled() and model.training
                and FusedTrainEngine.config_capable(model.cfg)
                and getattr(corr_fn, "hip", False) and corr_ok
                and _ext.use_hip(image))

    @staticmethod
    def corr_inputs(corr_fn):
        if getattr(corr_fn, "state", None) is not None:
            return corr_fn.state, corr_fn.token, ()
        return None, None, (corr_fn.f1, *corr_fn.f2s)

    def buffers(self, B, H, W, iters, dev):
        key = (B, H, W, iters, dev)
        S = self._bufs.get(key)
        adt = self.adt
        if S is None and self.small:
            n = iters * B
            e = lambda b, c: torch.empty(b, H, W, c, device=dev, dtype=adt)
            z = lambda b, c: torch.zeros(b, H, W, c, device=dev, dtype=adt)
            S = dict(
                corr=e(n, SCORR_PAD), f1=e(n, 64), mot=e(n, 128),
                hx=z(n + B, 256),
                z=[e(n, SHD)], r=[e(n, SHD)], q=[e(n, SHD)],
                rh=[z(n, 128)],
                head=e(n, 128), inp=e(B, 64),
                C=torch.empty(n + B, 2, H, W, device=dev),
                d_flow=torch.zeros(n, H, W, 64, device=dev, dtype=adt),
                d_head=e(n, 128), d_zr=[e(n, 2 * SHD)], d_q=[z(n, 128) if self.spad else e(n, SHD)],
                d_conv=e(n, 128 if self.spad else 96), d_mot=e(n, 128),
                d_f1=e(n, 64), d_corr=e(n, SCORR_PAD),
                G=torch.empty(B, H, W, 256, device=dev),
            )
            self._bufs = {key: S}
        elif S is None:
            n = iters * B
            e = lambda b, c: torch.empty(b, H, W, c, device=dev, dtype=adt)
            S = dict(
                corr=e(n, CORR_PAD), c1=e(n, 256), f1=e(n, 128), mot=e(n, 256), hx=e(n + B, 256), h1=e(n, HD),
                z=[e(n, HD), e(n, HD)], r=[e(n, HD), e(n, HD)], q=[e(n, HD), e(n, HD)], rh=[e(n, HD), e(n, HD)],
                head=e(n, 512), mask=e(n, 576), inp=e(B, 128),
                C=torch.empty(n + B, 2, H, W, device=dev),
                d_mask=torch.zeros(n, H, W, 640, device=dev, dtype=adt),
                d_flow=torch.zeros(n, H, W, 64, device=dev, dtype=adt),
                d_head=e(n, 512), d_zr=[e(n, 256), e(n, 256)], d_q=[e(n, HD), e(n, HD)], d_conv=e(n, 128),
                d_c2f2=e(n, 256), d_c1=e(n, 256), d_f1=e(n, 128), d_corr=e(n, CORR_PAD),
                G=torch.empty(B, H, W, 384, device=dev),
            )
            self._bufs = {key: S}
        return S


def _split_bf16(t: torch.Tensor):
    if t.is_cuda and t.is_contiguous() and t.data_ptr() % 16 == 0:
        hi, lo = R.split_bf16(t)
        return hi, lo
    hi = t.to(torch.bfloat16)
    return hi, (t - hi.float()).to(torch.bfloat16)


_WG3 = True


def _wgrad_fn(pc, segs, bn128):
    if (_WG3 and pc.kh * pc.kw in (5, 9) and pc.cout > 64 and all(int(s[2]) % 64 == 0 for s in segs)):
        bm = 128 if pc.cout >= 512 else 64
        return lambda *a: R.wgrad_v3(*a, bm)
    return lambda *a: R.conv_wgrad(*a, bn128)


def _conv_wgrad(eng, pc, dy, yoff, segs, H, W, bn128=0):
    per = [s[0].shape[0] * H * W for s in segs]
    wg = _wgrad_fn(pc, segs, bn128)
    if not eng.f32:
        wg(dy, yoff, pc.cout, [s[0] for s in segs], [s[1] for s in segs], [s[2] for s in segs],
           per, pc.kh, pc.kw, pc.dw, pc.db)
        return
    cache = eng.__dict__.setdefault("_split_cache", {})
    def split(t):
        key = (t.data_ptr(), tuple(t.shape))
        v = cache.get(key)
        if v is None:
            v = cache[key] = _split_bf16(t)
        return v
    dyh, dyl = split(dy)
    xs = [split(s[0]) for s in segs]
    offs, chans = [s[1] for s in segs], [s[2] for s in segs]
    wg(dyh, yoff, pc.cout, [x[0] for x in xs], offs, chans, per, pc.kh, pc.kw, pc.dw, pc.db)
    wg(dyl, yoff, pc.cout, [x[0] for x in xs], offs, chans, per, pc.kh, pc.kw, pc.dw, pc.db)
    wg(dyh, yoff, pc.cout, [x[1] for x in xs], offs, chans, per, pc.kh, pc.kw, pc.dw, None)


class DeferGrads(torch.autograd.Function):

    @staticmethod
    def forward(ctx, stream, *params):
        ctx.stream = stream
        return tuple(p.view_as(p) for p in params)

    @staticmethod
    def backward(ctx, *grads):
        dev = next(g.device for g in grads if g is not None)
        torch.cuda.current_stream(dev).wait_stream(ctx.stream)
        return (None, *grads)


class _Offset:
    __slots__ = ("t", "o")

    def __init__(self, t, o):
        self.t, self.o = t, o

    def __getitem__(self, s):
        return self.t[s.start - self.o:s.stop - self.o]


class FusedTrainLoop(torch.autograd.Function):

    @staticmethod
    def forward(ctx, eng, corr_state, token, net, inp, coords0, coords1, iters, defer, otf, *tensors):
        nt = 0 if otf is None else otf[2] + 1
        otf_t, params = tensors[:nt], tensors[nt:]
        if eng.small:
            return _small_forward(ctx, eng, corr_state, net, inp, coords0, coords1, iters, defer, otf, otf_t)
        B, _, H, W = coords1.shape
        dev = coords1.device
        eng.pack(dev)
        f1w, f1b = eng.f1w, eng.f1b
        S = eng.buffers(B, H, W, iters, dev)
        sl = lambda t, i: t[i * B:(i + 1) * B]
        if inp is None:
            cn = net.permute(0, 2, 3, 1).to(S["inp"].dtype).contiguous()
            R.context_act(cn, S["hx"][:B], S["inp"], HD)
        else:
            S["hx"][:B, ..., :HD].copy_(net.permute(0, 2, 3, 1))
            S["inp"].copy_(inp.permute(0, 2, 3, 1))
        C = S["C"]
        sl(C, 0).copy_(coords1.detach())
        c0 = coords0.detach().float().contiguous()
        inpb = S["inp"]
        if otf is not None:
            S["corr"][..., otf[2] * 81:].zero_()
        main, side = torch.cuda.current_stream(dev), eng.side_stream(dev, flow=True)
        for i in range(iters):
            hx, hx1 = sl(S["hx"], i), sl(S["hx"], i + 1)
            coords = sl(C, i)
            if side is not None:
                side.wait_stream(main)
            with torch.cuda.stream(side) if side is not None else contextlib.nullcontext():
                R.flow_encode(coords, f1w, f1b, sl(S["f1"], i), 0, hx, 254)
                conv_fused([(sl(S["f1"], i), 0, 128)], eng.f2.w, eng.f2.b, 3, 3, 64, EPI_RELU, sl(S["mot"], i), 192)
            if otf is None:
                R.corr_lookup_into(corr_state.pyr, coords, corr_state.radius, sl(S["corr"], i))
            else:
                cf = R.corr_otf(otf_t[0], list(otf_t[1:]), coords, otf[0], otf[1], True)
                sl(S["corr"], i)[..., :cf.shape[-1]].copy_(cf)
            conv_fused([(sl(S["corr"], i), 0, CORR_PAD)], eng.c1.w, eng.c1.b, 1, 1, 256, EPI_RELU, sl(S["c1"], i))
            conv_fused([(sl(S["c1"], i), 0, 256)], eng.c2.w, eng.c2.b, 3, 3, 192, EPI_RELU, sl(S["mot"], i), 0)
            if side is not None:
                main.wait_stream(side)
            conv_fused([(sl(S["mot"], i), 0, 256)], eng.cv.w, eng.cv.b, 3, 3, 126, EPI_RELU, hx, HD)
            h_in = [(hx, 0), (sl(S["h1"], i), 0)]
            h_out = [(sl(S["h1"], i), 0), (hx1, 0)]
            for p in range(2):
                hb, ho = h_in[p]
                z, r, q, rh = (sl(S[k][p], i) for k in ("z", "r", "q", "rh"))
                conv_fused([(hb, ho, HD), (inpb, 0, 128), (hx, HD, 128)], eng.zr[p].w, eng.zr[p].b, eng.zr[p].kh,
                           eng.zr[p].kw, 2 * HD, EPI_GRU_ZR, z, 0, hd=HD, out2=rh, out3=r, aux1=hb, a1off=ho)
                ob, oo = h_out[p]
                conv_fused([(rh, 0, HD), (inpb, 0, 128), (hx, HD, 128)], eng.q[p].w, eng.q[p].b, eng.q[p].kh,
                           eng.q[p].kw, HD, EPI_GRU_Q, ob, oo, out2=q, aux1=hb, a1off=ho, aux2=z)
            head = sl(S["head"], i)
            conv_fused([(hx1, 0, HD)], eng.head.w, eng.head.b, 3, 3, 512, EPI_RELU, head, 0)
            R.flow_head(head, 0, 256, eng.flow_w32, eng.flow.b, sl(C, i + 1), coords)
            conv_fused([(head, 256, 256)], eng.mask2.w, eng.mask2.b, 1, 1, 576, EPI_SCALE, sl(S["mask"], i), 0,
                       scale=0.25)
        n = iters * B
        flows = (C[B:].view(iters, B, 2, H, W) - c0).view(n, 2, H, W)
        up = R.convex_upsample(flows, S["mask"])
        ctx.eng, ctx.state, ctx.S, ctx.iters = eng, corr_state, S, iters
        ctx.otf = otf
        if otf is not None:
            ctx.save_for_backward(*otf_t)
        ctx.defer = bool(defer) and eng.side_stream(dev) is not None
        ctx.c0 = c0
        ctx.net_dtype = net.dtype
        ctx.inp_dtype = inp.dtype if inp is not None else None
        return up

    @staticmethod
    def backward(ctx, g_up):
        if ctx.eng.small:
            return _small_backward(ctx, g_up)
        eng, st, S, iters = ctx.eng, ctx.state, ctx.S, ctx.iters
        c0 = ctx.c0
        B, H, W = S["inp"].shape[:3]
        dev = c0.device
        n = iters * B
        sl = lambda t, i: t[i * B:(i + 1) * B]
        main = torch.cuda.current_stream(dev)
        side = eng.side_stream(dev, 1 if ctx.defer else 0, flow=not ctx.defer)
        lside = eng.side_stream(dev, 0) if ctx.defer else None
        otf = ctx.otf
        if otf is None:
            if st.gpyr is None:
                st.gpyr = st.zero_grads()
        else:
            otf_t = ctx.saved_tensors
            d_otf = None
        G = S["G"]
        G.zero_()
        inpb = S["inp"]
        C = S["C"]
        if g_up is None:
            g_up = torch.zeros(n, 2, 8 * H, 8 * W, device=dev)
        flows = (C[B:].view(iters, B, 2, H, W) - c0).view(n, 2, H, W)
        dflow, _ = R.convex_upsample_backward(flows, S["mask"], g_up.contiguous(), S["d_mask"])
        S["d_flow"][..., :2].copy_(dflow.permute(0, 2, 3, 1))
        for i in reversed(range(iters)):
            hx, hx1, head = sl(S["hx"], i), sl(S["hx"], i + 1), sl(S["head"], i)
            dm, df, dh = sl(S["d_mask"], i), sl(S["d_flow"], i), sl(S["d_head"], i)
            conv_fused([(dm, 0, 576)], eng.mask2.wd, None, 1, 1, 256, EPI_RELU_BWD, dh, 256, aux1=head, a1off=256)
            R.flow_head_dgrad(sl(dflow, i), eng.flow_w32, 256, head, 0, dh, 0)
            conv_fused([(dh, 0, 512)], eng.head.wd, None, 3, 3, HD, EPI_ACC_F32, G, 0)
            h_in = [(hx, 0), (sl(S["h1"], i), 0)]
            for p in (1, 0):
                hb, ho = h_in[p]
                z, r, q = sl(S["z"][p], i), sl(S["r"][p], i), sl(S["q"][p], i)
                dq, dzr = sl(S["d_q"][p], i), sl(S["d_zr"][p], i)
                R.gru_gate_bwd(G, z, q, hb, ho, dq, dzr)
                conv_fused([(dq, 0, HD)], eng.q[p].wd, None, eng.q[p].kh, eng.q[p].kw, 384, EPI_GRU_QBWD, G, 0,
                           hd=HD, out2=dzr, o2off=HD, aux1=hb, a1off=ho, aux2=r)
                conv_fused([(dzr, 0, 256)], eng.zr[p].wd, None, eng.zr[p].kh, eng.zr[p].kw, 384, EPI_ACC_F32, G, 0)
            dcv = sl(S["d_conv"], i)
            R.relu_take(G, 256, 126, 128, hx, HD, dcv)
            dc2f2 = sl(S["d_c2f2"], i)
            conv_fused([(dcv, 0, 128)], eng.cv.wd, None, 3, 3, 256, EPI_RELU_BWD, dc2f2, 0, aux1=sl(S["mot"], i))
            dc1 = sl(S["d_c1"], i)
            if side is not None:
                side.wait_stream(main)
            with torch.cuda.stream(side) if side is not None else contextlib.nullcontext():
                conv_fused([(dc2f2, 192, 64)], eng.f2.wd, None, 3, 3, 128, EPI_RELU_BWD, sl(S["d_f1"], i), 0,
                           aux1=sl(S["f1"], i))
            conv_fused([(dc2f2, 0, 192)], eng.c2.wd, None, 3, 3, 256, EPI_RELU_BWD, dc1, 0, aux1=sl(S["c1"], i))
            dcorr = sl(S["d_corr"], i)
            conv_fused([(dc1, 0, 256)], eng.c1.wd, None, 1, 1, CORR_PAD, EPI_BIAS, dcorr, 0)
            if lside is not None:
                lside.wait_stream(main)
            with torch.cuda.stream(lside) if lside is not None else contextlib.nullcontext():
                if otf is None:
                    R.corr_lookup_backward(st.gpyr, sl(C, i), st.radius, dcorr)
                else:
                    ch = otf[2] * 81
                    gi = R.corr_otf_backward(otf_t[0], list(otf_t[1:]), sl(C, i), otf[0], otf[1],
                                             dcorr[..., :ch].contiguous())
                    if d_otf is None:
                        d_otf = list(gi)
                    else:
                        for acc, g in zip(d_otf, gi):
                            acc.add_(g)
        if lside is not None:
            main.wait_stream(lside)
            if otf is not None:
                for g in d_otf:
                    g.record_stream(main)
        if otf is None and _EARLY_CORR_BWD:
            st.early_backward()
        if ctx.inp_dtype is None:
            d_net = R.context_act_backward(G, S["hx"][:B], S["inp"], HD).permute(0, 3, 1, 2).to(ctx.net_dtype)
            d_inp = None
        else:
            d_net = G[..., :HD].permute(0, 3, 1, 2).to(ctx.net_dtype)
            d_inp = G[..., HD:HD + 128].permute(0, 3, 1, 2).to(ctx.inp_dtype)

        grads = FusedTrainLoop._param_grads(ctx, FusedTrainLoop._wgrads, S, C, B, H, W, n, main, side)
        if otf is None:
            token_grad, otf_grads = torch.zeros((), device=dev), ()
        else:
            token_grad = None
            otf_grads = tuple(g.to(t.dtype) for g, t in zip(d_otf, otf_t))
        return (None, None, token_grad, d_net, d_inp, None, None, None, None, None, *otf_grads, *grads)

    @staticmethod
    def _param_grads(ctx, wgrads, S, C, B, H, W, n, main, side):
        eng = ctx.eng
        gbuf, dwf, dbf = eng.grad_buffers(main.device)
        if ctx.defer:
            side.wait_stream(main)
            gbuf.record_stream(side)
            wstream = torch.cuda.stream(side)
        else:
            if side is not None:
                main.wait_stream(side)
            wstream = contextlib.nullcontext()
        with wstream:
            wgrads(eng, S, C, gbuf, dwf, dbf, B, H, W, n)
            eng.__dict__.pop("_split_cache", None)
            if eng.grad_group is not None:
                eng.reduce_packed(gbuf)
            grads = [gr if gr.dtype == p.dtype else gr.to(p.dtype)
                     for gr, p in zip(eng.unpack_grads(gbuf), eng.params)]
        if ctx.defer:
            for gr in grads:
                gr.record_stream(main)
        return grads

    @staticmethod
    def _wgrads(eng, S, C, gbuf, dwf, dbf, B, H, W, n):
        inpb = S["inp"]
        hxs = S["hx"][:n]

        def wg(pc, dy, yoff, segs, bn128=0):
            _conv_wgrad(eng, pc, dy, yoff, segs, H, W, bn128)

        wg(eng.mask2, S["d_mask"], 0, [(S["head"], 256, 256)])
        wg(eng.flow, S["d_flow"], 0, [(S["head"], 0, 256)])
        wg(eng.head, S["d_head"], 0, [(S["hx"][B:], 0, HD)], 2)
        hins = [hxs, S["h1"]]
        for p in range(2):
            wg(eng.zr[p], S["d_zr"][p], 0, [(hins[p], 0, HD), (inpb, 0, 128), (hxs, HD, 128)], 4)
            wg(eng.q[p], S["d_q"][p], 0, [(S["rh"][p], 0, HD), (inpb, 0, 128), (hxs, HD, 128)])
        wg(eng.cv, S["d_conv"], 0, [(S["mot"], 0, 256)], 2)
        wg(eng.c2, S["d_c2f2"], 0, [(S["c1"], 0, 256)], 4)
        wg(eng.f2, S["d_c2f2"], 192, [(S["f1"], 0, 128)])
        wg(eng.c1, S["d_c1"], 0, [(S["corr"], 0, CORR_PAD)])
        R.flow_wgrad(C[:n], S["d_f1"], dwf, dbf)



_INTERP = {}


def _interp_matrix(n_in: int, n_out: int, dev) -> torch.Tensor:
    key = (n_in, n_out, str(dev))
    m = _INTERP.get(key)
    if m is None:
        scale = torch.tensor(float(n_in - 1), dtype=torch.float32) / (n_out - 1) if n_out > 1 else torch.tensor(0.0)
        src = scale * torch.arange(n_out, dtype=torch.float32)
        i0 = src.long()
        lam = src - i0.float()
        i1 = torch.where(i0 < n_in - 1, i0 + 1, i0)
        m = torch.zeros(n_out, n_in, dtype=torch.float32)
        rows = torch.arange(n_out)
        m[rows, i0] += 1 - lam
        m[rows, i1] += lam
        m = _INTERP[key] = m.to(dev)
    return m


def _small_forward(ctx, eng, corr_state, net, inp, coords0, coords1, iters, defer, otf=None, otf_t=()):
    B, _, H, W = coords1.shape
    dev = coords1.device
    hd = SHD
    eng.pack(dev)
    S = eng.buffers(B, H, W, iters, dev)
    sl = lambda t, i: t[i * B:(i + 1) * B]
    hv = S["hx"].view(iters + 1, B, H, W, 256)
    hv[0, ..., :hd].copy_(net.permute(0, 2, 3, 1))
    hv[..., hd:hd + 64].copy_(inp.permute(0, 2, 3, 1))
    C = S["C"]
    sl(C, 0).copy_(coords1.detach())
    c0 = coords0.detach().float().contiguous()
    if otf is not None:
        S["corr"][..., otf[2] * 49:].zero_()
    main, side = torch.cuda.current_stream(dev), eng.side_stream(dev, flow=True)
    zr, q = eng.zr[0], eng.q[0]
    for i in range(iters):
        hx, hx1 = sl(S["hx"], i), sl(S["hx"], i + 1)
        coords = sl(C, i)
        mot = sl(S["mot"], i)
        if side is not None:
            side.wait_stream(main)
        with torch.cuda.stream(side) if side is not None else contextlib.nullcontext():
            R.flow_encode(coords, eng.f1w, eng.f1b, sl(S["f1"], i), 0, hx, 240)
            conv_fused([(sl(S["f1"], i), 0, 64)], eng.f2.w, eng.f2.b, 3, 3, 32, EPI_RELU, mot, 96)
        if otf is None:
            R.corr_lookup_into(corr_state.pyr, coords, corr_state.radius, sl(S["corr"], i))
        else:
            cf = R.corr_otf(otf_t[0], list(otf_t[1:]), coords, otf[0], otf[1], True)
            sl(S["corr"], i)[..., :cf.shape[-1]].copy_(cf)
        conv_fused([(sl(S["corr"], i), 0, SCORR_PAD)], eng.c1.w, eng.c1.b, 1, 1, hd, EPI_RELU, mot, 0)
        if side is not None:
            main.wait_stream(side)
        conv_fused([(mot, 0, 128)], eng.cv.w, eng.cv.b, 3, 3, 80, EPI_RELU, hx, 160)
        z, r, qq, rh = (sl(S[k][0], i) for k in ("z", "r", "q", "rh"))
        conv_fused([(hx, 0, 256)], zr.w, zr.b, 3, 3, 2 * hd, EPI_GRU_ZR, z, 0, hd=hd, out2=rh, out3=r,
                   aux1=hx, a1off=0)
        qseg = [(rh, 0, 128), (hx, 64, 192)] if eng.spad else [(rh, 0, hd), (hx, hd, 160)]
        conv_fused(qseg, q.w, q.b, 3, 3, hd, EPI_GRU_Q, hx1, 0, out2=qq, aux1=hx, a1off=0, aux2=z)
        head = sl(S["head"], i)
        conv_fused([(hx1, 0, 128 if eng.spad else hd)], eng.head.w, eng.head.b, 3, 3, 128, EPI_RELU, head, 0)
        R.flow_head(head, 0, 128, eng.flow_w32, eng.flow.b, sl(C, i + 1), coords)
    n = iters * B
    flows = (C[B:].view(iters, B, 2, H, W) - c0).view(n, 2, H, W)
    up = 8 * torch.nn.functional.interpolate(flows, size=(8 * H, 8 * W), mode="bilinear", align_corners=True)
    ctx.eng, ctx.state, ctx.S, ctx.iters, ctx.otf = eng, corr_state, S, iters, otf
    if otf is not None:
        ctx.save_for_backward(*otf_t)
    ctx.defer = bool(defer) and eng.side_stream(dev) is not None
    ctx.c0 = c0
    ctx.net_dtype, ctx.inp_dtype = net.dtype, inp.dtype
    return up


def _small_backward(ctx, g_up):
    eng, st, S, iters = ctx.eng, ctx.state, ctx.S, ctx.iters
    hd = SHD
    B, H, W = S["inp"].shape[:3]
    dev = ctx.c0.device
    n = iters * B
    sl = lambda t, i: t[i * B:(i + 1) * B]
    main = torch.cuda.current_stream(dev)
    side = eng.side_stream(dev, 1 if ctx.defer else 0, flow=not ctx.defer)
    lside = eng.side_stream(dev, 0) if ctx.defer else None
    otf = ctx.otf
    if otf is None:
        if st.gpyr is None:
            st.gpyr = st.zero_grads()
    else:
        otf_t = ctx.saved_tensors
        d_otf = None
    G = S["G"]
    G.zero_()
    C = S["C"]
    if g_up is None:
        g_up = torch.zeros(n, 2, 8 * H, 8 * W, device=dev)
    ah, aw = _interp_matrix(H, 8 * H, dev), _interp_matrix(W, 8 * W, dev)
    dflow = torch.ops.raft_stir.upflow8_backward(g_up.float().contiguous(), ah, aw)
    S["d_flow"][..., :2].copy_(dflow.permute(0, 2, 3, 1))
    zr, q = eng.zr[0], eng.q[0]
    for i in reversed(range(iters)):
        hx, head, dh = sl(S["hx"], i), sl(S["head"], i), sl(S["d_head"], i)
        R.flow_head_dgrad(sl(dflow, i), eng.flow_w32, 128, head, 0, dh, 0)
        conv_fused([(dh, 0, 128)], eng.head.wd, None, 3, 3, hd, EPI_ACC_F32, G, 0)
        z, r, qq = sl(S["z"][0], i), sl(S["r"][0], i), sl(S["q"][0], i)
        dq, dzr = sl(S["d_q"][0], i), sl(S["d_zr"][0], i)
        R.gru_gate_bwd(G, z, qq, hx, 0, dq, dzr)
        conv_fused([(dq, 0, q.cy)], q.wd, None, 3, 3, 256, EPI_GRU_QBWD, G, 0, hd=hd, out2=dzr, o2off=hd,
                   aux1=hx, a1off=0, aux2=r)
        conv_fused([(dzr, 0, 2 * hd)], zr.wd, None, 3, 3, 256, EPI_ACC_F32, G, 0)
        dcv, dmot = sl(S["d_conv"], i), sl(S["d_mot"], i)
        R.relu_take(G, 160, 80, 96, hx, 160, dcv)
        conv_fused([(dcv, 0, eng.cv.cy)], eng.cv.wd, None, 3, 3, 128, EPI_RELU_BWD, dmot, 0, aux1=sl(S["mot"], i))
        if side is not None:
            side.wait_stream(main)
        with torch.cuda.stream(side) if side is not None else contextlib.nullcontext():
            conv_fused([(dmot, 96, 32)], eng.f2.wd, None, 3, 3, 64, EPI_RELU_BWD, sl(S["d_f1"], i), 0,
                       aux1=sl(S["f1"], i))
        dcorr = sl(S["d_corr"], i)
        conv_fused([(dmot, 0, eng.c1.cy)], eng.c1.wd, None, 1, 1, SCORR_PAD, EPI_BIAS, dcorr, 0)
        if lside is not None:
            lside.wait_stream(main)
        with torch.cuda.stream(lside) if lside is not None else contextlib.nullcontext():
            if otf is None:
                R.corr_lookup_backward(st.gpyr, sl(C, i), st.radius, dcorr)
            else:
                gi = R.corr_otf_backward(otf_t[0], list(otf_t[1:]), sl(C, i), otf[0], otf[1],
                                         dcorr[..., :otf[2] * 49].contiguous())
                if d_otf is None:
                    d_otf = list(gi)
                else:
                    for acc, g in zip(d_otf, gi):
                        acc.add_(g)
    if lside is not None:
        main.wait_stream(lside)
        if otf is not None:
            for g in d_otf:
                g.record_stream(main)
    if otf is None and _EARLY_CORR_BWD:
        st.early_backward()
    d_net = G[..., :hd].permute(0, 3, 1, 2).to(ctx.net_dtype)
    d_inp = G[..., hd:hd + 64].permute(0, 3, 1, 2).to(ctx.inp_dtype)
    grads = FusedTrainLoop._param_grads(ctx, _small_wgrads, S, C, B, H, W, n, main, side)
    if otf is None:
        token_grad, otf_grads = torch.zeros((), device=dev), ()
    else:
        token_grad = None
        otf_grads = tuple(g.to(t.dtype) for g, t in zip(d_otf, otf_t))
    return (None, None, token_grad, d_net, d_inp, None, None, None, None, None, *otf_grads, *grads)


def _small_wgrads(eng, S, C, gbuf, dwf, dbf, B, H, W, n):
    hxs = S["hx"][:n]

    def wg(pc, dy, yoff, segs, bn128=0):
        _conv_wgrad(eng, pc, dy, yoff, segs, H, W, bn128)

    wg(eng.flow, S["d_flow"], 0, [(S["head"], 0, 128)])
    wg(eng.head, S["d_head"], 0, [(S["hx"][B:], 0, 128)])
    wg(eng.zr[0], S["d_zr"][0], 0, [(hxs, 0, 256)])
    wg(eng.q[0], S["d_q"][0], 0, [(S["rh"][0], 0, 128), (hxs, 64, 192)])
    wg(eng.cv, S["d_conv"], 0, [(S["mot"], 0, 128)])
    wg(eng.f2, S["d_mot"], 96, [(S["f1"], 0, 64)])
    wg(eng.c1, S["d_mot"], 0, [(S["corr"], 0, SCORR_PAD)])
    R.flow_wgrad(C[:n], S["d_f1"], dwf, dbf)
```

raft_stir_amd/ops/conv.py:

```python
from __future__ import annotations

import os
from typing import List, Sequence, Tuple

import torch

(EPI_BIAS, EPI_RELU, EPI_SCALE, EPI_GRU_ZR, EPI_GRU_Q, EPI_FLOW,
 EPI_RELU_BWD, EPI_ACC_F32, EPI_GRU_QBWD, EPI_NORM) = range(10)

Piece = Tuple[int, int, int]
SegSpec = Tuple[int, Sequence[Piece]]


def pad_to(n: int, m: int) -> int:
    return (n + m - 1) // m * m


@torch.no_grad()
def pack_weight(weight: torch.Tensor, segs: Sequence[SegSpec], cout_pad: int,
                dtype: torch.dtype = torch.bfloat16) -> torch.Tensor:
    cout, cin, kh, kw = weight.shape
    taps = kh * kw
    wt = weight.detach().float().permute(0, 2, 3, 1).reshape(cout, taps, cin)
    ktot = sum(c for c, _ in segs)
    out = torch.zeros(cout_pad, taps, ktot, device=weight.device, dtype=torch.float32)
    kb = 0
    for c, pieces in segs:
        assert c % 32 == 0
        for w0, n, s0 in pieces:
            assert s0 + n <= c and w0 + n <= cin
            out[:cout, :, kb + s0:kb + s0 + n] = wt[:, :, w0:w0 + n]
        kb += c
    return out.to(dtype).contiguous()


@torch.no_grad()
def split_weight(packed: torch.Tensor) -> torch.Tensor:
    cp, taps, k = packed.shape
    assert k % 32 == 0
    w = packed.float().view(cp, taps, k // 32, 1, 32)
    hi = w.to(torch.bfloat16)
    lo = (w - hi.float()).to(torch.bfloat16)
    return torch.cat([hi, lo], 3).reshape(cp, taps, 2 * k).contiguous()


@torch.no_grad()
def pack_weight_split(weight: torch.Tensor, segs: Sequence[SegSpec], cout_pad: int) -> torch.Tensor:
    return split_weight(pack_weight(weight, segs, cout_pad, torch.float32))


V3_TILES = (56, 57, 61, 65, 66, 68)


@torch.no_grad()
def frag_weight(w: torch.Tensor) -> torch.Tensor:
    cp, taps, k = w.shape
    assert cp % 32 == 0 and k % 64 == 0, (cp, k)
    v = w.view(cp // 32, 32, taps, k // 64, 4, 2, 8)
    return v.permute(0, 3, 2, 4, 5, 1, 6).contiguous().view(cp, taps, k)


F32_TILES = (6, 7, 8)
V3F_TILES = (81, 82, 83, 84, 85)


@torch.no_grad()
def frag_weight_split(w_split: torch.Tensor) -> torch.Tensor:
    cp, taps, k2 = w_split.shape
    v = w_split.view(cp, taps, k2 // 64, 2, 32)
    hi = v[:, :, :, 0].reshape(cp, taps, k2 // 2)
    lo = v[:, :, :, 1].reshape(cp, taps, k2 // 2)
    return torch.cat([frag_weight(hi), frag_weight(lo)], 0)


def frag32_eligible(w_split: torch.Tensor, kh: int, kw: int) -> bool:
    return kh * kw in (5, 9) and w_split.dim() == 3 and w_split.shape[0] % 32 == 0 and w_split.shape[2] % 128 == 0


_V3F = os.environ.get("RS_V3F", "1") != "0"


def choose_tile_f32(P: int, cout: int, geo: bool = False, v3f: bool = False, taps: int = 9, ktot: int = 0) -> int:
    if v3f and _V3F and not geo:
        if P >= 16384:
            if cout <= 64:
                return 85 if ktot == 64 else 84
            return 83 if taps == 9 else 81
        return 82
    nb64 = -(-P // 64) * -(-cout // 64)
    if nb64 <= 256 and not geo:
        return 38
    if nb64 <= 768 and not geo:
        return 40
    if cout <= 64:
        return 6
    return 8 if (P >= 16384 and cout >= 256) else 7


@torch.no_grad()
def pack_bias(bias: torch.Tensor, n: int | None = None) -> torch.Tensor:
    b = bias.detach().float()
    if n is not None and n > b.numel():
        b = torch.cat([b, b.new_zeros(n - b.numel())])
    return b.contiguous()


_WIDE = 4


GEMM1_TILE = 70


def gemm1_ok(w: torch.Tensor, cout: int, chans, nscale=None) -> bool:
    return (w.dtype == torch.bfloat16 and nscale is None and all(int(c) % 64 == 0 for c in chans)
            and w.shape[0] >= pad_to(cout, 128))


def choose_tile(P: int, cout: int, seg_chans, taps: int = 9) -> int:
    if cout <= 16:
        return 5
    if all(c % 64 == 0 for c in seg_chans) and taps <= 32:
        k = taps * sum(seg_chans)
        if P >= 16384:
            if 64 < cout <= 128 and _WIDE & 1:
                return 31
            if cout > 192 and k >= 1024 and _WIDE & 2:
                return 31
            if 128 < cout <= 192 and k >= 1024 and _WIDE & 4:
                return 29
        return 16 if (P >= 16384 and cout >= 192 and k >= 384) else 17
    if -(-P // 64) * -(-cout // 64) <= 256:
        return 41
    big = cout >= 192 or (cout >= 126 and P >= 16384)
    return 4 if big else 3


_TUNED_PATH = os.environ.get("RS_CONV_TUNING_FILE") or os.path.join(
    os.path.dirname(os.path.dirname(os.path.abspath(__file__))), "conv_tuning.json")
_TUNED: dict | None = None
_RECORD: list | None = None


def tune_key(B: int, H: int, W: int, cout: int, chans, kh: int, kw: int, epi: int) -> str:
    return f"{B}x{H}x{W}|{cout}|{','.join(str(int(c)) for c in chans)}|{kh}x{kw}|{epi}"


def tuned_tiles() -> dict:
    global _TUNED
    if _TUNED is None:
        _TUNED = {}
        if os.environ.get("RS_CONV_TUNED", "1") != "0" and os.path.exists(_TUNED_PATH):
            import json
            with open(_TUNED_PATH) as f:
                _TUNED = {k: int(v) for k, v in json.load(f).get("tiles", {}).items()}
    return _TUNED


_TUNED_F32: dict | None = None


def tuned_tiles_f32() -> dict:
    global _TUNED_F32
    if _TUNED_F32 is None:
        _TUNED_F32 = {}
        if os.environ.get("RS_CONV_TUNED", "1") != "0" and os.path.exists(_TUNED_PATH):
            import json
            with open(_TUNED_PATH) as f:
                _TUNED_F32 = {k: int(v) for k, v in json.load(f).get("tiles_f32", {}).items()}
    return _TUNED_F32


def frag_eligible(w: torch.Tensor, kh: int, kw: int) -> bool:
    return kh * kw in (5, 9) and w.dim() == 3 and w.shape[0] % 32 == 0 and w.shape[2] % 64 == 0


def conv_fused(segs: List[Tuple[torch.Tensor, int, int]], w, bias, kh, kw, cout, epi, out, ooff=0,
               scale=1.0, hd=0, out2=None, o2off=0, out3=None, o3off=0, aux1=None, a1off=0,
               aux2=None, a2off=0, tile=None, nscale=None, wf=None):
    if wf is None:
        wf = getattr(w, "_rs_frag", None)
    tensors = [s[0] for s in segs]
    offs = [int(s[1]) for s in segs]
    chans = [int(s[2]) for s in segs]
    if _RECORD is not None:
        _RECORD.append(dict(segs=segs, w=w, bias=bias, kh=kh, kw=kw, cout=cout, epi=epi, out=out, ooff=ooff,
                            scale=scale, hd=hd, out2=out2, o2off=o2off, out3=out3, o3off=o3off, aux1=aux1,
                            a1off=a1off, aux2=aux2, a2off=a2off, tile=tile, nscale=nscale, wf=wf))
    if tile is None:
        t0 = tensors[0]
        key = tune_key(t0.shape[0], t0.shape[1], t0.shape[2], cout, chans, kh, kw, epi)
        P = t0.shape[0] * t0.shape[1] * t0.shape[2]
        if t0.dtype == torch.float32:
            tile = tuned_tiles_f32().get(key)
            has32 = getattr(w, "_rs_frag32", None) is not None and all(c % 64 == 0 for c in chans)
            if tile is None or (tile in V3F_TILES and not (has32 and _V3F)):
                tile = choose_tile_f32(P, cout, v3f=has32, taps=kh * kw, ktot=sum(chans))
        else:
            tile = tuned_tiles().get(key)
            if tile is None or (tile in V3_TILES and wf is None) or (tile == GEMM1_TILE and not gemm1_ok(
                    w, cout, chans, nscale)):
                tile = choose_tile(P, cout, chans, kh * kw)
    if tile in V3_TILES:
        if wf is None:
            raise ValueError("conv_fused: tiles 56-68 read the fragment-major weight: pass wf=frag_weight(w)")
        w = wf
    elif tile in V3F_TILES:
        wf32 = getattr(w, "_rs_frag32", None)
        if wf32 is None:
            raise ValueError("conv_fused: tiles 81-83 read the split fragment-major weight: tag the split "
                             "weight with _rs_frag32 = frag_weight_split(w)")
        w = wf32
    if nscale is None:
        torch.ops.raft_stir.conv_fused(tensors, offs, chans, w, bias, kh, kw, cout, epi, float(scale), hd,
                                       out, ooff, out2, o2off, out3, o3off, aux1, a1off, aux2, a2off, tile)
    else:
        torch.ops.raft_stir.conv_fused(tensors, offs, chans, w, bias, kh, kw, cout, epi, float(scale), hd,
                                       out, ooff, out2, o2off, out3, o3off, aux1, a1off, aux2, a2off, tile,
                                       nscale)
```

Before: 453.2 image-pairs/s.

## Fuse GRU gate backward and ReLU take into conv dgrad accumulate epilogues

```diff
diff --git a/raft_stir_amd/csrc/conv.hip b/raft_stir_amd/csrc/conv.hip
--- a/raft_stir_amd/csrc/conv.hip
+++ b/raft_stir_amd/csrc/conv.hip
@@ -804,9 +804,11 @@
     const float g = dh[p * dhstr + c];
     const float zv = io<T>::ld(z + p * zstr + c), qv = io<T>::ld(q + p * qstr + c);
     const float hv = io<T>::ld(h + p * hstr + hoff + c);
-    io<T>::st(dq + p * dqstr + c, g * zv * (1.f - qv * qv));
-    io<T>::st(dzr + p * dzrstr + c, g * (qv - hv) * zv * (1.f - zv));
-    dh[p * dhstr + c] = g * (1.f - zv);
+    float dqv, dzv, dhv;
+    gate_bwd_elem(g, zv, qv, hv, dqv, dzv, dhv);
+    io<T>::st(dq + p * dqstr + c, dqv);
+    io<T>::st(dzr + p * dzrstr + c, dzv);
+    dh[p * dhstr + c] = dhv;
   }
 }
 
@@ -821,7 +823,7 @@
     float v = 0.f;
     if (c < n) {
       const float g = G[p * gstr + goff + c];
-      v = io<T>::ld(act + p * astr + aoff + c) > 0.f ? g : 0.f;
+      v = relu_take_elem(g, io<T>::ld(act + p * astr + aoff + c));
     }
     io<T>::st(out + i, v);
     if (c < nz) G[p * gstr + goff + c] = 0.f;
@@ -854,6 +856,8 @@
   int Hi, Wi, SY, SX, oH, oW, OSY, OSX, OOY, OOX;
   const float* chs;
   int f32;
+  const void* aux3; int a3str, a3off;
+  int nact;
 };
 
 bool conv_launch(const ConvLaunch& L, hipStream_t stream) {
@@ -875,6 +879,8 @@
   a.out3 = L.out3; a.o3str = L.o3str; a.o3off = L.o3off;
   a.aux1 = static_cast<const bf16_t*>(L.aux1); a.a1str = L.a1str; a.a1off = L.a1off;
   a.aux2 = static_cast<const bf16_t*>(L.aux2); a.a2str = L.a2str; a.a2off = L.a2off;
+  a.aux3 = static_cast<const bf16_t*>(L.aux3); a.a3str = L.a3str; a.a3off = L.a3off;
+  a.nact = L.nact;
   for (int s = 0; s < 3; ++s) a.seg_bytes[s] = L.seg_bytes[s];
   a.w_bytes = L.w_bytes;
   a.chs = L.chs;
diff --git a/raft_stir_amd/csrc/conv_common.h b/raft_stir_amd/csrc/conv_common.h
--- a/raft_stir_amd/csrc/conv_common.h
+++ b/raft_stir_amd/csrc/conv_common.h
@@ -17,7 +17,17 @@
   EPI_ACC_F32 = 7,
   EPI_GRU_QBWD = 8,
   EPI_NORM = 9,
+  EPI_ACC_GATE = 10,
+  EPI_ACC_TAKE = 11,
 };
+
+__device__ __forceinline__ void gate_bwd_elem(float g, float zv, float qv, float hv, float& dq, float& dz,
+                                              float& dh) {
+  dq = g * zv * (1.f - qv * qv);
+  dz = g * (qv - hv) * zv * (1.f - zv);
+  dh = g * (1.f - zv);
+}
+__device__ __forceinline__ float relu_take_elem(float g, float act) { return act > 0.f ? g : 0.f; }
 
 struct Seg {
   const bf16_t* ptr;
@@ -53,6 +63,9 @@
   int oH, oW, OSY, OSX, OOY, OOX;
   const float* chs;
   int f32;
+  const bf16_t* aux3;
+  int a3str, a3off;
+  int nact;
 };
 
 typedef float f32x2v_t __attribute__((ext_vector_type(2)));
@@ -248,6 +261,86 @@
           if (cb + j < a.Cout) o[j] += v[j];
       }
     }
+  } else if constexpr (E == EPI_ACC_GATE) {
+    float* o = static_cast<float*>(a.out) + (size_t)p * a.ostr + a.ooff + cb;
+    if (cb < a.hd) {
+      const bf16_t* h = a.aux1 + (size_t)p * a.a1str + a.a1off + cb;
+      const bf16_t* z = a.aux2 + (size_t)p * a.a2str + a.a2off + cb;
+      const bf16_t* q = a.aux3 + (size_t)p * a.a3str + a.a3off + cb;
+      bf16_t* dqp = static_cast<bf16_t*>(a.out2) + (size_t)p * a.o2str + a.o2off + cb;
+      bf16_t* dzp = static_cast<bf16_t*>(a.out3) + (size_t)p * a.o3str + a.o3off + cb;
+      float gv[4], hv[4], zv[4], qv[4], dq[4], dz[4], dh[4];
+      if (vec) {
+        const float4 ov = *reinterpret_cast<const float4*>(o);
+        gv[0] = ov.x + v[0];
+        gv[1] = ov.y + v[1];
+        gv[2] = ov.z + v[2];
+        gv[3] = ov.w + v[3];
+        ld4(h, hv);
+        ld4(z, zv);
+        ld4(q, qv);
+      } else {
+#pragma unroll
+        for (int j = 0; j < 4; ++j) {
+          gv[j] = o[j] + v[j];
+          hv[j] = bf2f(h[j]);
+          zv[j] = bf2f(z[j]);
+          qv[j] = bf2f(q[j]);
+        }
+      }
+#pragma unroll
+      for (int j = 0; j < 4; ++j) gate_bwd_elem(gv[j], zv[j], qv[j], hv[j], dq[j], dz[j], dh[j]);
+      if (vec) {
+        st4(dqp, dq);
+        st4(dzp, dz);
+        *reinterpret_cast<float4*>(o) = make_float4(dh[0], dh[1], dh[2], dh[3]);
+      } else {
+#pragma unroll
+        for (int j = 0; j < 4; ++j) {
+          dqp[j] = f2bf(dq[j]);
+          dzp[j] = f2bf(dz[j]);
+          o[j] = dh[j];
+        }
+      }
+    } else {
+      if (vec && full) {
+        acc4(o, v);
+      } else {
+#pragma unroll
+        for (int j = 0; j < 4; ++j)
+          if (cb + j < a.Cout) o[j] += v[j];
+      }
+    }
+  } else if constexpr (E == EPI_ACC_TAKE) {
+    float* o = static_cast<float*>(a.out) + (size_t)p * a.ostr + a.ooff + cb;
+    if (cb < a.hd) {
+      if (vec) {
+        acc4(o, v);
+      } else {
+#pragma unroll
+        for (int j = 0; j < 4; ++j) o[j] += v[j];
+      }
+    } else {
+      const int c = cb - a.hd;
+      const bf16_t* act = a.aux1 + (size_t)p * a.a1str + a.a1off + c;
+      bf16_t* d = static_cast<bf16_t*>(a.out2) + (size_t)p * a.o2str + a.o2off + c;
+      if (vec) {
+        const float4 ov = *reinterpret_cast<const float4*>(o);
+        float av[4];
+        ld4(act, av);
+        float tv[4] = {ov.x + v[0], ov.y + v[1], ov.z + v[2], ov.w + v[3]};
+#pragma unroll
+        for (int j = 0; j < 4; ++j) tv[j] = c + j < a.nact ? relu_take_elem(tv[j], av[j]) : 0.f;
+        st4(d, tv);
+        *reinterpret_cast<float4*>(o) = make_float4(0.f, 0.f, 0.f, 0.f);
+      } else {
+#pragma unroll
+        for (int j = 0; j < 4; ++j) {
+          d[j] = f2bf(c + j < a.nact ? relu_take_elem(o[j] + v[j], bf2f(act[j])) : 0.f);
+          o[j] = 0.f;
+        }
+      }
+    }
   } else if constexpr (E == EPI_NORM) {
     if (a.hd) {
 #pragma unroll
@@ -292,8 +385,10 @@
   const int HW = a.H * a.W;
   const int cq = (lane >> 4) * 4;
   const bool vec =
-      ((a.ooff | a.ostr | a.o2off | a.o2str | a.o3off | a.o3str | a.a1off | a.a1str | a.a2off | a.a2str) & 3) == 0 &&
-      (((uintptr_t)a.out | (uintptr_t)a.out2 | (uintptr_t)a.out3 | (uintptr_t)a.aux1 | (uintptr_t)a.aux2) & 15) == 0;
+      ((a.ooff | a.ostr | a.o2off | a.o2str | a.o3off | a.o3str | a.a1off | a.a1str | a.a2off | a.a2str | a.a3off |
+        a.a3str) & 3) == 0 &&
+      (((uintptr_t)a.out | (uintptr_t)a.out2 | (uintptr_t)a.out3 | (uintptr_t)a.aux1 | (uintptr_t)a.aux2 |
+        (uintptr_t)a.aux3) & 15) == 0;
   const bool bvec = a.bias && (((uintptr_t)a.bias) & 15) == 0;
 #pragma unroll
   for (int nt = 0; nt < WN; ++nt) {
@@ -341,6 +436,8 @@
     RS_EPI(EPI_RELU);
     RS_EPI(EPI_SCALE);
     RS_EPI(EPI_NORM);
+    RS_EPI(EPI_ACC_GATE);
+    RS_EPI(EPI_ACC_TAKE);
 #undef RS_EPI
     default: epi_loop<WM, WN, EPI_BIAS>(a, acc, m0, lane, pp, pb, py, px); break;
   }
@@ -466,8 +563,10 @@
                                              const int (&pp)[WN], const int (&pb)[WN]) {
   const int cq = (lane >> 4) * 4;
   const bool vec =
-      ((a.ooff | a.ostr | a.o2off | a.o2str | a.o3off | a.o3str | a.a1off | a.a1str | a.a2off | a.a2str) & 3) == 0 &&
-      (((uintptr_t)a.out | (uintptr_t)a.out2 | (uintptr_t)a.out3 | (uintptr_t)a.aux1 | (uintptr_t)a.aux2) & 15) == 0;
+      ((a.ooff | a.ostr | a.o2off | a.o2str | a.o3off | a.o3str | a.a1off | a.a1str | a.a2off | a.a2str | a.a3off |
+        a.a3str) & 3) == 0 &&
+      (((uintptr_t)a.out | (uintptr_t)a.out2 | (uintptr_t)a.out3 | (uintptr_t)a.aux1 | (uintptr_t)a.aux2 |
+        (uintptr_t)a.aux3) & 15) == 0;
 #pragma unroll
   for (int nt = 0; nt < WN; ++nt) {
     if (pb[nt] < 0) continue;
@@ -659,10 +758,10 @@
 #pragma unroll
   for (int i = 0; i < 16; ++i) bz[i] = a.bias ? a.bias[m0 + 8 * (i >> 2) + h4 + (i & 3)] : 0.f;
   const bool lo = m0 < a.hd;
-  constexpr int NBC = NB > 3 ? 3 : NB;
+  constexpr int NBC = E == EPI_ACC_GATE ? 1 : (NB > 3 ? 3 : NB);
 #pragma unroll
   for (int n0 = 0; n0 < NB; n0 += NBC) {
-    uint2 l1[NBC][4], l2[NBC][4];
+    uint2 l1[NBC][4], l2[NBC][4], l3[NBC][4];
     float4 lf[NBC][4];
 #pragma unroll
     for (int k = 0; k < NBC; ++k) {
@@ -686,6 +785,16 @@
             l1[k][g] = *reinterpret_cast<const uint2*>(a.aux1 + p * a.a1str + a.a1off + cb);
             l2[k][g] = *reinterpret_cast<const uint2*>(a.aux2 + p * a.a2str + a.a2off + cb);
           }
+        } else if constexpr (E == EPI_ACC_GATE) {
+          lf[k][g] = *reinterpret_cast<const float4*>(static_cast<const float*>(a.out) + p * a.ostr + a.ooff + cb);
+          if (lo) {
+            l1[k][g] = *reinterpret_cast<const uint2*>(a.aux1 + p * a.a1str + a.a1off + cb);
+            l2[k][g] = *reinterpret_cast<const uint2*>(a.aux2 + p * a.a2str + a.a2off + cb);
+            l3[k][g] = *reinterpret_cast<const uint2*>(a.aux3 + p * a.a3str + a.a3off + cb);
+          }
+        } else if constexpr (E == EPI_ACC_TAKE) {
+          lf[k][g] = *reinterpret_cast<const float4*>(static_cast<const float*>(a.out) + p * a.ostr + a.ooff + cb);
+          if (!lo) l1[k][g] = *reinterpret_cast<const uint2*>(a.aux1 + p * a.a1str + a.a1off + cb - a.hd);
         }
       }
     }
@@ -757,6 +866,38 @@
           } else {
             *reinterpret_cast<float4*>(op) = make_float4(o.x + v[0], o.y + v[1], o.z + v[2], o.w + v[3]);
           }
+        } else if constexpr (E == EPI_ACC_GATE) {
+          const float4 o = lf[k][g];
+          float* op = static_cast<float*>(a.out) + p * a.ostr + a.ooff + cb;
+          const float gv[4] = {o.x + v[0], o.y + v[1], o.z + v[2], o.w + v[3]};
+          if (lo) {
+            float hv[4], zv[4], qv[4], dq[4], dz[4], dh[4];
+            unpack(l1[k][g], hv);
+            unpack(l2[k][g], zv);
+            unpack(l3[k][g], qv);
+#pragma unroll
+            for (int j = 0; j < 4; ++j) gate_bwd_elem(gv[j], zv[j], qv[j], hv[j], dq[j], dz[j], dh[j]);
+            st4(static_cast<bf16_t*>(a.out2) + p * a.o2str + a.o2off + cb, dq);
+            st4(static_cast<bf16_t*>(a.out3) + p * a.o3str + a.o3off + cb, dz);
+            *reinterpret_cast<float4*>(op) = make_float4(dh[0], dh[1], dh[2], dh[3]);
+          } else {
+            *reinterpret_cast<float4*>(op) = make_float4(gv[0], gv[1], gv[2], gv[3]);
+          }
+        } else if constexpr (E == EPI_ACC_TAKE) {
+          const float4 o = lf[k][g];
+          float* op = static_cast<float*>(a.out) + p * a.ostr + a.ooff + cb;
+          float tv[4] = {o.x + v[0], o.y + v[1], o.z + v[2], o.w + v[3]};
+          if (lo) {
+            *reinterpret_cast<float4*>(op) = make_float4(tv[0], tv[1], tv[2], tv[3]);
+          } else {
+            const int c = cb - a.hd;
+            float av[4];
+            unpack(l1[k][g], av);
+#pragma unroll
+            for (int j = 0; j < 4; ++j) tv[j] = c + j < a.nact ? relu_take_elem(tv[j], av[j]) : 0.f;
+            st4(static_cast<bf16_t*>(a.out2) + p * a.o2str + a.o2off + c, tv);
+            *reinterpret_cast<float4*>(op) = make_float4(0.f, 0.f, 0.f, 0.f);
+          }
         } else {
 #pragma unroll
           for (int j = 0; j < 4; ++j) {
@@ -775,8 +916,10 @@
                                            const int (&pp)[NB], const int (&pb)[NB], const int (&py)[NB],
                                            const int (&px)[NB]) {
   const bool vec =
-      ((a.ooff | a.ostr | a.o2off | a.o2str | a.o3off | a.o3str | a.a1off | a.a1str | a.a2off | a.a2str) & 3) == 0 &&
-      (((uintptr_t)a.out | (uintptr_t)a.out2 | (uintptr_t)a.out3 | (uintptr_t)a.aux1 | (uintptr_t)a.aux2) & 15) == 0;
+      ((a.ooff | a.ostr | a.o2off | a.o2str | a.o3off | a.o3str | a.a1off | a.a1str | a.a2off | a.a2str | a.a3off |
+        a.a3str) & 3) == 0 &&
+      (((uintptr_t)a.out | (uintptr_t)a.out2 | (uintptr_t)a.out3 | (uintptr_t)a.aux1 | (uintptr_t)a.aux2 |
+        (uintptr_t)a.aux3) & 15) == 0;
   const bool fast = vec && m0 + 32 <= a.Cout && (a.hd & 31) == 0;
   if (fast) {
     switch (a.epi) {
@@ -787,6 +930,8 @@
       RS_EB(EPI_RELU_BWD);
       RS_EB(EPI_ACC_F32);
       RS_EB(EPI_GRU_QBWD);
+      RS_EB(EPI_ACC_GATE);
+      RS_EB(EPI_ACC_TAKE);
       RS_EB(EPI_RELU);
       RS_EB(EPI_SCALE);
       RS_EB(EPI_BIAS);
@@ -806,6 +951,8 @@
     RS_E2(EPI_RELU_BWD);
     RS_E2(EPI_ACC_F32);
     RS_E2(EPI_GRU_QBWD);
+    RS_E2(EPI_ACC_GATE);
+    RS_E2(EPI_ACC_TAKE);
     RS_E2(EPI_RELU);
     RS_E2(EPI_SCALE);
 #undef RS_E2
diff --git a/raft_stir_amd/csrc/ops_conv.cpp b/raft_stir_amd/csrc/ops_conv.cpp
--- a/raft_stir_amd/csrc/ops_conv.cpp
+++ b/raft_stir_amd/csrc/ops_conv.cpp
@@ -33,6 +33,8 @@
   int Hi, Wi, SY, SX, oH, oW, OSY, OSX, OOY, OOX;
   const float* chs;
   int f32;
+  const void* aux3; int a3str, a3off;
+  int nact;
 };
 bool conv_launch(const ConvLaunch& L, hipStream_t stream);
 struct SconvLaunch {
@@ -131,7 +133,7 @@
 using at::Tensor;
 
 constexpr int EPI_GRU_ZR = 3, EPI_GRU_Q = 4, EPI_FLOW = 5, EPI_RELU_BWD = 6, EPI_ACC_F32 = 7, EPI_GRU_QBWD = 8,
-              EPI_NORM = 9;
+              EPI_NORM = 9, EPI_ACC_GATE = 10, EPI_ACC_TAKE = 11;
 
 hipStream_t stream() { return rs::current_stream(); }
 
@@ -174,7 +176,8 @@
                const c10::optional<Tensor>& out2, int64_t o2off, const c10::optional<Tensor>& out3,
                int64_t o3off, const c10::optional<Tensor>& aux1, int64_t a1off,
                const c10::optional<Tensor>& aux2, int64_t a2off, int64_t tile,
-               const NormX& nx = NormX()) {
+               const NormX& nx = NormX(), const c10::optional<Tensor>& aux3 = c10::nullopt, int64_t a3off = 0,
+               int64_t nact = 0) {
   TORCH_CHECK(!segs.empty() && segs.size() <= 3, "conv_fused: 1..3 input segments");
   TORCH_CHECK(seg_off.size() == segs.size() && seg_C.size() == segs.size(), "conv_fused: segment spec");
   const int B = segs[0].size(0), H = segs[0].size(1), W = segs[0].size(2);
@@ -187,6 +190,8 @@
     TORCH_CHECK(tile == 6 || tile == 7 || tile == 8 || (tile >= 38 && tile <= 40) || v3f,
                 "conv_fused: fp32 activations run on tiles 6, 7, 8, 38-40, 81-85 only");
     TORCH_CHECK(epi != EPI_FLOW, "conv_fused: fp32 activations: no flow epilogue (csrc/flowhead.hip serves it)");
+    TORCH_CHECK(epi != EPI_ACC_GATE && epi != EPI_ACC_TAKE,
+                "conv_fused: fp32 activations: no fused gate / take epilogue (gru_gate_bwd / relu_take serve them)");
   }
   L.f32 = f32 ? 1 : 0;
   int Ktot = 0;
@@ -291,7 +296,7 @@
       L.out2 = out2->data_ptr();
     }
   } else {
-    const bool f32out = f32 || epi == EPI_ACC_F32 || epi == EPI_GRU_QBWD;
+    const bool f32out = f32 || epi == EPI_ACC_F32 || epi == EPI_GRU_QBWD || epi == EPI_ACC_GATE || epi == EPI_ACC_TAKE;
     check_nhwc(out, B, H, W, "out", f32out ? at::kFloat : at::kBFloat16);
     const int cw = epi == EPI_GRU_ZR ? hd : Cout;
     TORCH_CHECK(ooff >= 0 && ooff + cw <= out.size(3), "conv_fused: output window out of bounds");
@@ -326,8 +331,23 @@
     opt_nhwc(out2, o2off, hd, "out2", &L.out2, &L.o2str, &L.o2off);
     opt_nhwc(aux1, a1off, hd, "aux1", &p, &L.a1str, &L.a1off); L.aux1 = p;
     opt_nhwc(aux2, a2off, hd, "aux2", &p, &L.a2str, &L.a2off); L.aux2 = p;
-  }
-  TORCH_CHECK(epi >= 0 && epi <= EPI_NORM, "conv_fused: unknown epilogue kind");
+  } else if (epi == EPI_ACC_GATE) {
+    TORCH_CHECK(hd > 0 && hd % 4 == 0 && hd <= Cout && out2 && out3 && aux1 && aux2 && aux3,
+                "conv_fused(acc_gate): needs hd % 4 == 0, out2 (dq), out3 (dz), aux1 (h), aux2 (z), aux3 (q~)");
+    opt_nhwc(out2, o2off, hd, "out2", &L.out2, &L.o2str, &L.o2off);
+    opt_nhwc(out3, o3off, hd, "out3", &L.out3, &L.o3str, &L.o3off);
+    opt_nhwc(aux1, a1off, hd, "aux1", &p, &L.a1str, &L.a1off); L.aux1 = p;
+    opt_nhwc(aux2, a2off, hd, "aux2", &p, &L.a2str, &L.a2off); L.aux2 = p;
+    opt_nhwc(aux3, a3off, hd, "aux3", &p, &L.a3str, &L.a3off); L.aux3 = p;
+  } else if (epi == EPI_ACC_TAKE) {
+    TORCH_CHECK(hd >= 0 && hd % 4 == 0 && Cout % 4 == 0 && hd < Cout && nact >= 0 && nact <= Cout - hd && out2 && aux1,
+                "conv_fused(acc_take): needs hd % 4 == 0, Cout % 4 == 0, 0 <= nact <= Cout - hd, out2 (taken "
+                "gradient), aux1 (the ReLU output)");
+    opt_nhwc(out2, o2off, Cout - hd, "out2", &L.out2, &L.o2str, &L.o2off);
+    opt_nhwc(aux1, a1off, Cout - hd, "aux1", &p, &L.a1str, &L.a1off); L.aux1 = p;
+    L.nact = nact;
+  }
+  TORCH_CHECK(epi >= 0 && epi <= EPI_ACC_TAKE, "conv_fused: unknown epilogue kind");
   if (nx.chs)
     TORCH_CHECK(!(tile >= 42 && tile <= 54) && !v3 && tile != 70 && (!(tile >= 81 && tile <= 85) || f32),
                 "conv_fused: EPI_NORM needs a tile with the shared epilogue (not 42-70)");
@@ -342,10 +362,11 @@
                 int64_t epi, double scale, int64_t hd, const Tensor& out, int64_t ooff,
                 const c10::optional<Tensor>& out2, int64_t o2off, const c10::optional<Tensor>& out3,
                 int64_t o3off, const c10::optional<Tensor>& aux1, int64_t a1off,
-                const c10::optional<Tensor>& aux2, int64_t a2off, int64_t tile, const c10::optional<Tensor>& nscale) {
+                const c10::optional<Tensor>& aux2, int64_t a2off, int64_t tile, const c10::optional<Tensor>& nscale,
+                const c10::optional<Tensor>& aux3, int64_t a3off, int64_t nact) {
   const NormX nx = norm_extras(nscale, bias, epi, Cout, "conv_fused");
   conv_impl(segs, seg_off, seg_C, w, bias, KH, KW, Cout, epi, scale, hd, out, ooff, out2, o2off, out3, o3off,
-            aux1, a1off, aux2, a2off, tile, nx);
+            aux1, a1off, aux2, a2off, tile, nx, aux3, a3off, nact);
 }
 
 void conv_geo(const std::vector<Tensor>& segs, at::IntArrayRef seg_off, at::IntArrayRef seg_C, const Tensor& w,
@@ -915,7 +936,7 @@
   m.def("conv_fused(Tensor[] segs, int[] seg_off, int[] seg_C, Tensor w, Tensor? bias, int KH, int KW, "
         "int Cout, int epi, float scale, int hd, Tensor(a!) out, int ooff, Tensor(b!)? out2, int o2off, "
         "Tensor(c!)? out3, int o3off, Tensor? aux1, int a1off, Tensor? aux2, int a2off, int tile, "
-        "Tensor? nscale=None) -> ()");
+        "Tensor? nscale=None, Tensor? aux3=None, int a3off=0, int nact=0) -> ()");
   m.def("enc_wgrad(Tensor dy, Tensor x) -> Tensor");
   m.def("sconv_wgrad(Tensor dy, Tensor x, int KH, int KW, int stride, int pad, Tensor(a!) dw) -> ()");
   m.def("sconv(Tensor x, Tensor w, Tensor? bias, int stride, int pad, bool relu, Tensor(a!) out, int yoff, "
diff --git a/raft_stir_amd/models/fused_train.py b/raft_stir_amd/models/fused_train.py
--- a/raft_stir_amd/models/fused_train.py
+++ b/raft_stir_amd/models/fused_train.py
@@ -7,9 +7,9 @@
 import torch
 
 from ..ops import _ext
-from ..ops.conv import (EPI_ACC_F32, EPI_BIAS, EPI_FLOW, EPI_GRU_Q, EPI_GRU_QBWD, EPI_GRU_ZR, EPI_RELU,
-                        EPI_RELU_BWD, EPI_SCALE, conv_fused, frag32_eligible, frag_eligible, frag_weight,
-                        frag_weight_split, pack_bias, pack_weight, pad_to)
+from ..ops.conv import (EPI_ACC_F32, EPI_ACC_GATE, EPI_ACC_TAKE, EPI_BIAS, EPI_FLOW, EPI_GRU_Q, EPI_GRU_QBWD,
+                        EPI_GRU_ZR, EPI_RELU, EPI_RELU_BWD, EPI_SCALE, conv_fused, frag32_eligible, frag_eligible,
+                        frag_weight, frag_weight_split, pack_bias, pack_weight, pad_to)
 
 R = torch.ops.raft_stir
 HD = 128
@@ -20,6 +20,8 @@
 SCORR_PAD = 256
 _SMALL_KPAD = os.environ.get("RS_SMALL_KPAD", "1") != "0"
 _EARLY_CORR_BWD = os.environ.get("RS_EARLY_CORR_BWD", "1") != "0"
+_FUSE_LOOP_BWD = os.environ.get("RS_FUSE_LOOP_BWD", "1") != "0"
+_FUSE_GATE_P1 = os.environ.get("RS_FUSE_GATE_P1", "0") != "0"
 _V3F_TRAIN = True
 
 
@@ -542,18 +544,34 @@
             dm, df, dh = sl(S["d_mask"], i), sl(S["d_flow"], i), sl(S["d_head"], i)
             conv_fused([(dm, 0, 576)], eng.mask2.wd, None, 1, 1, 256, EPI_RELU_BWD, dh, 256, aux1=head, a1off=256)
             R.flow_head_dgrad(sl(dflow, i), eng.flow_w32, 256, head, 0, dh, 0)
-            conv_fused([(dh, 0, 512)], eng.head.wd, None, 3, 3, HD, EPI_ACC_F32, G, 0)
             h_in = [(hx, 0), (sl(S["h1"], i), 0)]
+            fuse = _FUSE_LOOP_BWD and not eng.f32
+            gate1 = fuse and _FUSE_GATE_P1
+            gate = lambda p: dict(hd=HD, out2=sl(S["d_q"][p], i), out3=sl(S["d_zr"][p], i), aux1=h_in[p][0],
+                                  a1off=h_in[p][1], aux2=sl(S["z"][p], i), aux3=sl(S["q"][p], i))
+            dcv = sl(S["d_conv"], i)
+            if fuse:
+                conv_fused([(dh, 0, 512)], eng.head.wd, None, 3, 3, HD, EPI_ACC_GATE, G, 0, **gate(1))
+            else:
+                conv_fused([(dh, 0, 512)], eng.head.wd, None, 3, 3, HD, EPI_ACC_F32, G, 0)
             for p in (1, 0):
                 hb, ho = h_in[p]
                 z, r, q = sl(S["z"][p], i), sl(S["r"][p], i), sl(S["q"][p], i)
                 dq, dzr = sl(S["d_q"][p], i), sl(S["d_zr"][p], i)
-                R.gru_gate_bwd(G, z, q, hb, ho, dq, dzr)
+                if not (fuse if p == 1 else gate1):
+                    R.gru_gate_bwd(G, z, q, hb, ho, dq, dzr)
                 conv_fused([(dq, 0, HD)], eng.q[p].wd, None, eng.q[p].kh, eng.q[p].kw, 384, EPI_GRU_QBWD, G, 0,
                            hd=HD, out2=dzr, o2off=HD, aux1=hb, a1off=ho, aux2=r)
-                conv_fused([(dzr, 0, 256)], eng.zr[p].wd, None, eng.zr[p].kh, eng.zr[p].kw, 384, EPI_ACC_F32, G, 0)
-            dcv = sl(S["d_conv"], i)
-            R.relu_take(G, 256, 126, 128, hx, HD, dcv)
+                zr = eng.zr[p]
+                if p == 1 and gate1:
+                    conv_fused([(dzr, 0, 256)], zr.wd, None, zr.kh, zr.kw, 384, EPI_ACC_GATE, G, 0, **gate(0))
+                elif p == 1 or not fuse:
+                    conv_fused([(dzr, 0, 256)], zr.wd, None, zr.kh, zr.kw, 384, EPI_ACC_F32, G, 0)
+                else:
+                    conv_fused([(dzr, 0, 256)], zr.wd, None, zr.kh, zr.kw, 384, EPI_ACC_TAKE, G, 0, hd=256,
+                               out2=dcv, aux1=hx, a1off=HD, nact=126)
+            if not fuse:
+                R.relu_take(G, 256, 126, 128, hx, HD, dcv)
             dc2f2 = sl(S["d_c2f2"], i)
             conv_fused([(dcv, 0, 128)], eng.cv.wd, None, 3, 3, 256, EPI_RELU_BWD, dc2f2, 0, aux1=sl(S["mot"], i))
             dc1 = sl(S["d_c1"], i)
diff --git a/raft_stir_amd/ops/conv.py b/raft_stir_amd/ops/conv.py
--- a/raft_stir_amd/ops/conv.py
+++ b/raft_stir_amd/ops/conv.py
@@ -6,7 +6,7 @@
 import torch
 
 (EPI_BIAS, EPI_RELU, EPI_SCALE, EPI_GRU_ZR, EPI_GRU_Q, EPI_FLOW,
- EPI_RELU_BWD, EPI_ACC_F32, EPI_GRU_QBWD, EPI_NORM) = range(10)
+ EPI_RELU_BWD, EPI_ACC_F32, EPI_GRU_QBWD, EPI_NORM, EPI_ACC_GATE, EPI_ACC_TAKE) = range(12)
 
 Piece = Tuple[int, int, int]
 SegSpec = Tuple[int, Sequence[Piece]]
@@ -176,7 +176,7 @@
 
 def conv_fused(segs: List[Tuple[torch.Tensor, int, int]], w, bias, kh, kw, cout, epi, out, ooff=0,
                scale=1.0, hd=0, out2=None, o2off=0, out3=None, o3off=0, aux1=None, a1off=0,
-               aux2=None, a2off=0, tile=None, nscale=None, wf=None):
+               aux2=None, a2off=0, tile=None, nscale=None, wf=None, aux3=None, a3off=0, nact=0):
     if wf is None:
         wf = getattr(w, "_rs_frag", None)
     tensors = [s[0] for s in segs]
@@ -185,10 +185,12 @@
     if _RECORD is not None:
         _RECORD.append(dict(segs=segs, w=w, bias=bias, kh=kh, kw=kw, cout=cout, epi=epi, out=out, ooff=ooff,
                             scale=scale, hd=hd, out2=out2, o2off=o2off, out3=out3, o3off=o3off, aux1=aux1,
-                            a1off=a1off, aux2=aux2, a2off=a2off, tile=tile, nscale=nscale, wf=wf))
+                            a1off=a1off, aux2=aux2, a2off=a2off, tile=tile, nscale=nscale, wf=wf, aux3=aux3,
+                            a3off=a3off, nact=nact))
     if tile is None:
         t0 = tensors[0]
-        key = tune_key(t0.shape[0], t0.shape[1], t0.shape[2], cout, chans, kh, kw, epi)
+        kepi = EPI_ACC_F32 if epi in (EPI_ACC_GATE, EPI_ACC_TAKE) else epi
+        key = tune_key(t0.shape[0], t0.shape[1], t0.shape[2], cout, chans, kh, kw, kepi)
         P = t0.shape[0] * t0.shape[1] * t0.shape[2]
         if t0.dtype == torch.float32:
             tile = tuned_tiles_f32().get(key)
@@ -210,7 +212,11 @@
             raise ValueError("conv_fused: tiles 81-83 read the split fragment-major weight: tag the split "
                              "weight with _rs_frag32 = frag_weight_split(w)")
         w = wf32
-    if nscale is None:
+    if epi in (EPI_ACC_GATE, EPI_ACC_TAKE):
+        torch.ops.raft_stir.conv_fused(tensors, offs, chans, w, bias, kh, kw, cout, epi, float(scale), hd,
+                                       out, ooff, out2, o2off, out3, o3off, aux1, a1off, aux2, a2off, tile,
+                                       None, aux3, a3off, nact)
+    elif nscale is None:
         torch.ops.raft_stir.conv_fused(tensors, offs, chans, w, bias, kh, kw, cout, epi, float(scale), hd,
                                        out, ooff, out2, o2off, out3, o3off, aux1, a1off, aux2, a2off, tile)
     else:
```

Result: no change. 455.4 image-pairs/s (median of 6 runs) (+0.5%).
